# yangyonggit/simple-path-tracer

Hardware: AMD Instinct MI355X
Metric: Mrays/sec + Msamples/sec, default scene 1920x1080, 1/2/4/8 MI355X (higher is better)
Workload: dtype f32; 1 GPU; C2: default scene + emitter, 1920x1080, 64 spp, depth 6; scene=default_emitter, width=1920, height=1080, spp=64, max_depth=6, parallelism=tile-sharded x1 (interleaved 32x32 tiles) + RCCL gather to rank 0

## Files before the change

### include/sptr_hip.h

```cpp
#ifndef SPTR_HIP_H
#define SPTR_HIP_H

#include <stddef.h>
#include <stdint.h>

#ifdef __cplusplus
extern "C" {
#endif

#define SPTR_ABI_VERSION 9

enum sptr_status {
  SPTR_OK = 0,
  SPTR_ERR_INVALID = -1,
  SPTR_ERR_HIP = -2,
  SPTR_ERR_NO_SCENE = -3,
  SPTR_ERR_OOM = -4,
  SPTR_ERR_NO_DEVICE = -5
};

typedef struct sptr_ctx sptr_ctx;

typedef struct sptr_scene {
  const float* positions;
// ... 53 lines not shown
enum sptr_integrator { SPTR_INTEGRATOR_WAVEFRONT = 0, SPTR_INTEGRATOR_PATHTRACER = 1, SPTR_INTEGRATOR_OPTIX = 2 };

typedef struct sptr_frame {
  int32_t width, height;
  sptr_camera camera;
  uint32_t frame_begin;
  uint32_t spp;
  uint32_t max_depth;
  int32_t shard_rank, shard_count;
  uint32_t flags;
  uint32_t integrator;
  uint32_t samples_per_frame;
} sptr_frame;

typedef struct sptr_stats {
  uint64_t rays_closest;
  uint64_t rays_shadow;
  uint64_t samples;
  uint64_t waves;
  double ms_total;
  double ms_raygen, ms_trace, ms_shade, ms_shadow, ms_accum;
  uint64_t trace_launches;
  uint64_t node_visits, tri_tests, sphere_tests;
  uint64_t shadow_node_visits, shadow_prim_tests;
  double ms_trace0, ms_shade0;
  uint64_t rays_tail;
  double ms_tail;
  uint64_t traced_primary, traced_bounce;
  uint64_t node_visits_primary, tri_tests_primary, sphere_tests_primary;
  double ms_cull;
  uint64_t cull_launches;
  uint64_t shadow_launches;
  uint64_t traced_by_depth[8];
  uint64_t nodes_by_depth[8];
  uint64_t trace_visit_hist[16];
  uint64_t shadow_visit_hist[16];
  uint64_t hits_primary, hits_bounce;
  uint64_t paths_handed_off;
  uint64_t strag_visits[3];
  double ms_trace_busy;
  uint64_t traced_fused;
} sptr_stats;

int sptr_abi_version(void);
int sptr_create(int device, sptr_ctx** out);
int sptr_destroy(sptr_ctx* ctx);
const char* sptr_last_error(const sptr_ctx* ctx);
int sptr_set_debug_mode(sptr_ctx* ctx, int mode);
int sptr_set_wave_paths(sptr_ctx* ctx, uint64_t max_paths);
int sptr_set_tail_depth(sptr_ctx* ctx, uint32_t depth);
int sptr_set_bounce_chain(sptr_ctx* ctx, uint32_t mode);
int sptr_set_sky_split(sptr_ctx* ctx, uint32_t mode, uint32_t bulk_threads);
int sptr_sky_split_info(sptr_ctx* ctx, uint32_t* bulk_threads);
int sptr_set_leaf_size(sptr_ctx* ctx, uint32_t max_prims);
int sptr_set_tree_order(sptr_ctx* ctx, uint32_t mode);
typedef struct sptr_tree_order_info {
  uint32_t order, fallback, depth, num_leaves;
  double cost_sah, cost_morton;
} sptr_tree_order_info;
int sptr_tree_info(const sptr_ctx* ctx, sptr_tree_order_info* out);
int sptr_set_split_refs(sptr_ctx* ctx, uint32_t max_pieces);
int sptr_set_stragglers(sptr_ctx* ctx, uint32_t lanes);
int sptr_set_launch_mode(sptr_ctx* ctx, uint32_t mode);
int sptr_set_pixel_lanes(sptr_ctx* ctx, uint32_t lanes);
int sptr_pixel_lanes_info(const sptr_ctx* ctx, uint32_t* requested, uint32_t* active);
int sptr_graph_info(const sptr_ctx* ctx, uint32_t* valid, uint32_t* nodes, uint32_t* edges, uint32_t* depth,
                    uint32_t* captures, int32_t* capture_status);
const char* sptr_capture_error(const sptr_ctx* ctx);
int sptr_overlap_probe(sptr_ctx* ctx, double ms[3]);
int sptr_set_bvh_width(sptr_ctx* ctx, uint32_t width);

int sptr_upload_scene(sptr_ctx* ctx, const sptr_scene* scene);
int sptr_set_materials(sptr_ctx* ctx, const sptr_material* mats, uint32_t count);
int sptr_set_lights(sptr_ctx* ctx, const sptr_light* lights, uint32_t count);
int sptr_set_environment(sptr_ctx* ctx, const sptr_environment* env);
int sptr_scene_info(const sptr_ctx* ctx, uint32_t* num_prims, uint32_t* num_nodes, uint32_t* bvh_depth,
                    double* build_ms);
typedef struct sptr_scene_layout {
  uint32_t num_tris, num_spheres, num_nodes, leaf_size, bvh_depth, lds_bytes;
  uint64_t node_bytes, tri_bytes, sphere_bytes, prim_ref_bytes;
  uint32_t bvh_width;
  uint32_t num_prim_refs;
} sptr_scene_layout;
int sptr_scene_layout_info(const sptr_ctx* ctx, sptr_scene_layout* out);

int sptr_render(sptr_ctx* ctx, const sptr_frame* frame, void* stream, sptr_stats* stats);
int sptr_collect_stats(sptr_ctx* ctx, sptr_stats* stats);
int sptr_read_rgb8(sptr_ctx* ctx, uint8_t* rgb);
int sptr_read_rgb8_lagged(sptr_ctx* ctx, uint8_t* rgb, uint32_t* got);
int sptr_read_accum(sptr_ctx* ctx, float* accum);
int sptr_tiles_device(sptr_ctx* ctx, void** dptr, size_t* bytes);
int sptr_unpack_tiles(sptr_ctx* ctx, const void* gathered, int32_t shard_count, uint32_t tiles_per_rank,
                      int32_t width, int32_t height, void* rgb8_out, void* stream);

typedef struct sptr_denoise_params {
  uint32_t iterations;
  float sigma_color;
  float sigma_depth;
  float sigma_albedo;
  uint32_t normal_log2_power;
  uint32_t reserved[3];
} sptr_denoise_params;
int sptr_set_denoise(sptr_ctx* ctx, const sptr_denoise_params* params);
enum { SPTR_AOV_ALBEDO = 0, SPTR_AOV_NORMAL = 1, SPTR_AOV_DEPTH = 2, SPTR_AOV_ID = 3, SPTR_AOV_UV = 4 };
int sptr_read_aov(sptr_ctx* ctx, int kind, void* out);
int sptr_read_denoised(sptr_ctx* ctx, float* rgb);
// ... 133 lines not shown
```

### simple-path-tracer_amd/csrc/kernels_wavefront.hip

```cpp
#include <hip/hip_runtime.h>
#include <hip/hip_ext.h>

#include <algorithm>
#include <cstdlib>
#include <mutex>

#include "cull_prims.h"
#include "sky_split.h"
#include "sptr_internal.h"

#ifndef SPTR_TRACE_WAVES
#define SPTR_TRACE_WAVES 7
#endif
#ifndef SPTR_TRACE_PM_WAVES
#define SPTR_TRACE_PM_WAVES SPTR_TRACE_WAVES
#endif
#ifndef SPTR_TRACE_WP_WAVES
#define SPTR_TRACE_WP_WAVES SPTR_TRACE_WAVES
#endif
#ifndef SPTR_TRACE4_WAVES
#define SPTR_TRACE4_WAVES 7
#endif
#ifndef SPTR_SHADE_WAVES
#define SPTR_SHADE_WAVES 5
// ... 782 lines not shown
                   nt = sv.num_tris * 3u, ns = sv.num_sph;
    const uint32_t np = (sv.num_tris + sv.num_sph + 3u) / 4u;
    const float4* gn = w4 ? reinterpret_cast<const float4*>(sv.nodes4) : reinterpret_cast<const float4*>(sv.nodes);
    const float4* gp = reinterpret_cast<const float4*>(sv.prim_ref);
    for (uint32_t i = threadIdx.x; i < nn; i += blockDim.x) lds[i] = gn[i];
    for (uint32_t i = threadIdx.x; i < nt; i += blockDim.x) lds[nn + i] = sv.tris[i];
    for (uint32_t i = threadIdx.x; i < ns; i += blockDim.x) lds[nn + nt + i] = sv.sph[i];
    for (uint32_t i = threadIdx.x; i < np; i += blockDim.x) lds[nn + nt + ns + i] = gp[i];
    __syncthreads();
    s.nodes = reinterpret_cast<const BvhNode*>(lds);
    s.nodes4 = reinterpret_cast<const WideNode*>(lds);
    s.tris = lds + nn;
    s.sph = lds + nn + nt;
    s.prim_ref = reinterpret_cast<const uint32_t*>(lds + nn + nt + ns);
  }
  return s;
}

template <bool kTable>
__device__ __forceinline__ Staged stage_shaded(const SceneView& sv, const ShadeView& sh, float4* lds) {
  const bool tab = kTable && sh.pm_lds_bytes != 0u;
  float4* dst = lds + sv.lds_bytes / 16u;
  if (tab) {
    const float4* g = reinterpret_cast<const float4*>(sh.prim_mat);
    for (uint32_t i = threadIdx.x; i < sh.pm_lds_bytes / 16u; i += blockDim.x) dst[i] = g[i];
  }
  Staged s = stage_scene<true>(sv, lds);
  if (kTable) {
    s.pm = tab ? reinterpret_cast<const uint32_t*>(dst) : sh.prim_mat;
    s.pm_lds = tab;
  }
  return s;
}

__device__ __forceinline__ const uint4* stage_top(const SceneView& sv, float4* dst) {
  const uint32_t n = sv.num_top4 * (uint32_t)(sizeof(WideNode) / 16);
  const uint4* g = reinterpret_cast<const uint4*>(sv.nodes4);
  uint4* d = reinterpret_cast<uint4*>(dst);
  for (uint32_t i = threadIdx.x; i < n; i += blockDim.x) d[i] = g[i];
  return d;
}
__device__ __forceinline__ uint32_t top_lds_offset(const SceneView& sv, bool lds, bool primary, uint32_t nseg) {
  return (lds ? sv.lds_bytes / 16u : 0u) + (primary ? 0u : (4u * (nseg + 1u) + 15u) / 16u);
}

template <bool kW4, bool kAny, bool kCount, int N>
__device__ __forceinline__ bool traverse_w(const Staged& sc, const SceneView& sv, const Ray& r, float tnear, float& tfar,
                                           uint32_t& ref, Visits& vc, LdsStackN<N>& ls) {
  if (kW4) return traverse_wide<kAny, kCount>(sc.nodes4, sc.prim_ref, sc.tris, sc.sph, sv.root4, r, tnear, tfar, ref, vc, ls);
  return traverse<kAny, kCount>(sc.nodes, sc.prim_ref, sc.tris, sc.sph, sv.root, r, tnear, tfar, ref, vc, ls);
}

constexpr uint32_t kEntryFieldBits = 13, kEntryFieldMask = (1u << kEntryFieldBits) - 1u;
template <bool kW4, bool kCount, int N>
__device__ __forceinline__ bool traverse_w_from(const Staged& sc, const SceneView& sv, uint32_t root, const Ray& r,
                                                float& tfar, uint32_t& ref, Visits& vc, LdsStackN<N>& ls) {
  if constexpr (kW4) {
    return traverse_wide<false, kCount>(sc.nodes4, sc.prim_ref, sc.tris, sc.sph, sv.root4, r, 0.0f, tfar, ref, vc, ls);
  } else {
    if (root & kLeafBit) {
      if (root == sv.root) return leaf_test<false, kCount>(root, sc.prim_ref, sc.tris, sc.sph, r, 0.0f, tfar, ref, vc);
      asm volatile("" : "+v"(root));
      const float4* nd = reinterpret_cast<const float4*>(sc.nodes + ((root >> 18) & kEntryFieldMask));
      const uint32_t right = (root >> 17) & 1u;
      const float4 xy = nd[right];
      const float2 z = reinterpret_cast<const float2*>(nd + 2)[right];
      if (kCount) ++vc.nodes;
      float tent;
      if (!slab(xy.x, xy.y, xy.z, xy.w, z.x, z.y, r, 0.0f, tfar, tent)) return false;
      const uint32_t range = kLeafBit | (((root >> 4) & kEntryFieldMask) << kLeafCountBits) | (root & kLeafRangeMask);
      return leaf_test<false, kCount>(range, sc.prim_ref, sc.tris, sc.sph, r, 0.0f, tfar, ref, vc);
    }
    return traverse<false, kCount>(sc.nodes, sc.prim_ref, sc.tris, sc.sph, root, r, 0.0f, tfar, ref, vc, ls);
  }
}

template <bool kW4, bool kAny, bool kCount, int N>
__device__ __forceinline__ bool traverse_w_top(const Staged& sc, const SceneView& sv, const uint4* top, uint32_t ntop,
                                               const Ray& r, float tnear, float& tfar, uint32_t& ref, Visits& vc,
                                               LdsStackN<N>& ls) {
  if constexpr (kW4) {
    WideWalk wk;
    if (wide_start<kAny, kCount>(wk, sv.root4, sc.prim_ref, sc.tris, sc.sph, r, tnear, tfar, ref, vc)) return wk.hit;
    TravStack<N> stack;
    stack.lds = &ls.e[0][threadIdx.x];
    (void)wide_walk<kAny, kCount>(wk, stack, sc.nodes4, top, ntop, sc.prim_ref, sc.tris, sc.sph, r, tnear, tfar, ref, vc,
                                  0x7FFFFFFF);
    return wk.hit;
  }
  return traverse<kAny, kCount>(sc.nodes, sc.prim_ref, sc.tris, sc.sph, sv.root, r, tnear, tfar, ref, vc, ls);
}

__device__ __forceinline__ uint32_t stat_depth(int depth) { return depth < kStatDepths - 1 ? (uint32_t)depth : kStatDepths - 1u; }
__device__ __forceinline__ void hist_ray(uint32_t* s_hist, uint32_t visits) {
  const uint32_t b = visits ? (uint32_t)(32 - __clz(visits)) : 0u;
  atomicAdd(&s_hist[b < (uint32_t)kHistBins ? b : kHistBins - 1u], 1u);
}
__device__ __forceinline__ void hist_init(uint32_t* s_hist) {
  if (threadIdx.x < (uint32_t)kHistBins) s_hist[threadIdx.x] = 0u;
}
__device__ __forceinline__ void hist_flush(const uint32_t* s_hist, unsigned long long* tot, int base) {
  __syncthreads();
  if (threadIdx.x < (uint32_t)kHistBins && s_hist[threadIdx.x]) atomicAdd(&tot[base + threadIdx.x], (unsigned long long)s_hist[threadIdx.x]);
}
__device__ __forceinline__ void flush_depth_nodes(const Visits& vc, unsigned long long* tot, int depth) {
  unsigned long long a = vc.nodes;
  for (int off = 32; off > 0; off >>= 1) a += __shfl_xor(a, off);
  if (lane_id() == 0) atomicAdd(&tot[kTotNodesD + stat_depth(depth)], a);
}

__device__ __forceinline__ void report_stack(const Visits& vc, unsigned long long* tot) {
  if (__ballot(vc.stack_overflow != 0u) && lane_id() == 0u) tot[kTotStackOverflow] = 1ull;
}

__device__ __forceinline__ void flush_visits(const Visits& vc, unsigned long long* tot, int base) {
  unsigned long long a = vc.nodes, b = vc.tris, c = vc.sph;
  for (int off = 32; off > 0; off >>= 1) {
    a += __shfl_xor(a, off);
    b += __shfl_xor(b, off);
    c += __shfl_xor(c, off);
  }
  if (lane_id() == 0) {
    atomicAdd(&tot[base + 0], a);
    atomicAdd(&tot[base + 1], b);
    if (base == kTotNodes || base == kTotNodesP || base == kTotStragNodes) atomicAdd(&tot[base + 2], c);
  }
}
// ... 46 lines not shown
    if (d < -kCullSlack * mag) return true;
  }
  return false;
}
__device__ __forceinline__ bool pixel_frustum_misses(const SceneView& sv, const FrameView& f, int x, int y, int npx = 1) {
  if (sv.num_nodes == 0u || (sv.root & kLeafBit)) return false;
  const float u0 = (float(x) - kCullMarginPx) / float(f.W), u1 = (float(x + npx) + kCullMarginPx) / float(f.W);
  const float v0 = (float(y) - kCullMarginPx) / float(f.H), v1 = (float(y + npx) + kCullMarginPx) / float(f.H);
  auto dir = [&](float u, float v) {
    return f.cam_f + ((u - 0.5f) * 2.0f * f.half_w) * f.cam_r + (-(v - 0.5f) * 2.0f * f.half_h) * f.cam_u;
  };
  const vec3 c[4] = {dir(u0, v0), dir(u1, v0), dir(u1, v1), dir(u0, v1)};
  vec3 n[4];
#pragma unroll
  for (int k = 0; k < 4; ++k) {
    n[k] = cross(c[k], c[(k + 1) & 3]);
    if (dot(n[k], c[(k + 2) & 3]) < 0.0f) n[k] = -n[k];
  }
  struct Entry {
    uint32_t link, depth;
    Box b;
  };
  Entry st[2 * kCullDepthMax + 2];
  int sp = 0;
  {
    const BvhNode r = sv.nodes[0];
    st[sp++] = Entry{r.link.y, 1u, Box{v3(r.rxy.x, r.rxy.z, r.z.z), v3(r.rxy.y, r.rxy.w, r.z.w)}};
    st[sp++] = Entry{r.link.x, 1u, Box{v3(r.lxy.x, r.lxy.z, r.z.x), v3(r.lxy.y, r.lxy.w, r.z.y)}};
  }
  while (sp > 0) {
    const Entry e = st[--sp];
    if (box_outside(e.b, n, f.cam_pos)) continue;
    if ((e.link & kLeafBit) || e.depth >= f.cull_depth) return false;
    const BvhNode g = sv.nodes[e.link];
    st[sp++] = Entry{g.link.y, e.depth + 1u, Box{v3(g.rxy.x, g.rxy.z, g.z.z), v3(g.rxy.y, g.rxy.w, g.z.w)}};
    st[sp++] = Entry{g.link.x, e.depth + 1u, Box{v3(g.lxy.x, g.lxy.z, g.z.x), v3(g.lxy.y, g.lxy.w, g.z.y)}};
  }
  return true;
}
constexpr int kCullEntryDepth = 20;
struct CullStack {
  uint32_t st[kCullEntryDepth + 2][kBlock];
  uint16_t path[kCullEntryDepth + 1][kBlock];
};
constexpr uint32_t kCullLeaf = 1u << 17;
__device__ __forceinline__ uint32_t cull_pack(uint32_t link, uint32_t depth, uint32_t side) {
  const uint32_t l = (link & kLeafBit) ? (kCullLeaf | (((link & ~kLeafBit) >> kLeafCountBits) << 4) | (link & kLeafRangeMask)) : link;
  return l | (depth << 18) | (side << 24);
}
__device__ __forceinline__ Box child_box(const BvhNode& g, bool right) {
  return right ? Box{v3(g.rxy.x, g.rxy.z, g.z.z), v3(g.rxy.y, g.rxy.w, g.z.w)}
               : Box{v3(g.lxy.x, g.lxy.z, g.z.x), v3(g.lxy.y, g.lxy.w, g.z.y)};
}
__device__ __forceinline__ void cull_leaf(const Staged& sc, const CullPyramid& py, uint32_t link, uint32_t& lo, uint32_t& hi) {
  const uint32_t start = (link & ~kLeafBit) >> kLeafCountBits, cnt = (link & kLeafRangeMask) + 1u;
  lo = kNoHit;
  hi = 0u;
  for (uint32_t j = 0; j < cnt; ++j) {
    const uint32_t pr = sc.prim_ref[start + j];
    const uint32_t idx = pr & kIndexMask;
    bool out;
    if (pr & kSphereBit) {
      const float4 s = sc.sph[idx];
      const vec3 c = v3(s.x, s.y, s.z), v = c - py.o;
      const float rb = fabsf(s.w) + 1.1e-3f * (fabsf(v.x) + fabsf(v.y) + fabsf(v.z)) +
                       1e-5f * (py.ol + fabsf(c.x) + fabsf(c.y) + fabsf(c.z));
      out = box_outside(Box{c - v3(rb, rb, rb), c + v3(rb, rb, rb)}, py.n, py.o) || cull_sphere_outside(py, c, s.w);
    } else {
      const float4 a = sc.tris[3u * idx], b = sc.tris[3u * idx + 1u], c = sc.tris[3u * idx + 2u];
      const vec3 v0 = v3(a.x, a.y, a.z), v1 = v0 - v3(a.w, b.x, b.y), v2 = v0 + v3(b.z, b.w, c.x);
      const vec3 lo3 = v3(fminf(v0.x, fminf(v1.x, v2.x)), fminf(v0.y, fminf(v1.y, v2.y)), fminf(v0.z, fminf(v1.z, v2.z)));
      const vec3 hi3 = v3(fmaxf(v0.x, fmaxf(v1.x, v2.x)), fmaxf(v0.y, fmaxf(v1.y, v2.y)), fmaxf(v0.z, fmaxf(v1.z, v2.z)));
      const float pad = 1e-5f * (fabsf(lo3.x) + fabsf(lo3.y) + fabsf(lo3.z) + fabsf(hi3.x) + fabsf(hi3.y) + fabsf(hi3.z) + py.ol);
      out = box_outside(Box{lo3 - v3(pad, pad, pad), hi3 + v3(pad, pad, pad)}, py.n, py.o) || cull_triangle_outside(py, v0, v1, v2);
    }
    if (!out) {
      lo = min(lo, start + j);
      hi = start + j;
    }
  }
}
__device__ __forceinline__ uint32_t entry_leaf(uint32_t parent, uint32_t side, uint32_t lo, uint32_t hi) {
  if (parent >= kEntryFieldMask || hi > kEntryFieldMask) return parent;
  return kLeafBit | (parent << 18) | (side << 17) | (lo << 4) | (hi - lo);
}
__device__ __forceinline__ uint32_t cull_entry(const Staged& sc, const SceneView& sv, const FrameView& f, int x, int y, int npx,
                                               CullStack& cs) {
  if (sv.root == kNoHit) return kNoHit;
  const float u0 = (float(x) - kCullMarginPx) / float(f.W), u1 = (float(x + npx) + kCullMarginPx) / float(f.W);
  const float v0 = (float(y) - kCullMarginPx) / float(f.H), v1 = (float(y + npx) + kCullMarginPx) / float(f.H);
  auto dir = [&](float u, float v) {
    return f.cam_f + ((u - 0.5f) * 2.0f * f.half_w) * f.cam_r + (-(v - 0.5f) * 2.0f * f.half_h) * f.cam_u;
  };
  const CullPyramid py = cull_pyramid(f.cam_pos, dir(u0, v0), dir(u1, v0), dir(u1, v1), dir(u0, v1));
  uint32_t lo, hi;
  if ((sv.root & kLeafBit) || sv.num_nodes == 0u) return sv.root;
  const uint32_t limit = min(f.cull_depth, (uint32_t)kCullEntryDepth);
  uint32_t* st = &cs.st[0][threadIdx.x];
  uint16_t* path = &cs.path[0][threadIdx.x];
  int sp = 0;
  uint32_t ncand = 0u, common = kNoHit, mind = kNoHit, anc = sv.root, one_lo = 0u, one_hi = 0u, one_side = 0u;
  bool one_leaf = false;
  auto push_children = [&](uint32_t node, uint32_t depth) {
    const BvhNode g = sc.nodes[node];
    path[(depth - 1u) * kBlock] = (uint16_t)node;
    if (!box_outside(child_box(g, true), py.n, f.cam_pos)) st[sp++ * kBlock] = cull_pack(g.link.y, depth, 1u);
    if (!box_outside(child_box(g, false), py.n, f.cam_pos)) st[sp++ * kBlock] = cull_pack(g.link.x, depth, 0u);
  };
  push_children(sv.root, 1u);
  while (sp > 0) {
    const uint32_t e = st[--sp * kBlock];
    const uint32_t link = e & (kCullLeaf - 1u), depth = (e >> 18) & 63u, side = (e >> 24) & 1u;
    mind = min(mind, depth);
    if (e & kCullLeaf) {
      cull_leaf(sc, py, kLeafBit | ((link >> 4) << kLeafCountBits) | (link & kLeafRangeMask), lo, hi);
      if (lo > hi) continue;
      one_leaf = ncand++ == 0u;
      common = one_leaf ? depth : min(common, mind);
      anc = path[(common - 1u) * kBlock];
      mind = kNoHit;
      one_lo = lo;
      one_hi = hi;
      one_side = side;
    } else if (depth >= limit) {
      if (ncand++ == 0u) {
        common = depth + 1u;
        anc = link;
      } else {
        common = min(common, mind);
        anc = path[(common - 1u) * kBlock];
      }
      mind = kNoHit;
      one_leaf = false;
    } else {
      push_children(link, depth + 1u);
    }
  }
  if (ncand == 0u) return kNoHit;
  if (one_leaf) return entry_leaf(anc, one_side, one_lo, one_hi);
  return anc;
}
__device__ __forceinline__ uint32_t entry_index(uint32_t l) {
  const uint32_t w = l & 1023u;
  return ((l >> 10) << 8) | ((w >> 6) << 4) | ((w & 31u) >> 1);
}
template <bool kEntry>
__global__ void __launch_bounds__(kBlock) k_cull(SceneView sv, FrameView f, uint32_t* mask, uint32_t* plist, uint32_t* entry,
                                                 uint32_t list_culled) {
  static_assert(kTile == 32 && kBlock == 256, "16 x 16 quads per 32 x 32 tile");
  __shared__ uint32_t s_row[kTile];
  __shared__ uint32_t s_cnt[kBlock / 64u];
  __shared__ uint32_t s_base, s_base_c;
  const uint32_t t0 = blockIdx.x * kTilePixels;
  if (threadIdx.x < (uint32_t)kTile) s_row[threadIdx.x] = 0u;
  extern __shared__ float4 lds[];
  [[maybe_unused]] const Staged sc = stage_scene<kEntry>(sv, lds);
  __syncthreads();
  {
    const uint32_t qx = threadIdx.x & 15u, qy = threadIdx.x >> 4;
    int x = 0, y = 0;
    (void)local_pixel(f, t0 + 2u * qy * kTile + 2u * qx, x, y);
    bool miss;
    if constexpr (kEntry) {
      __shared__ CullStack s_cs;
      const uint32_t e = (x < f.W && y < f.H) ? cull_entry(sc, sv, f, x, y, 2, s_cs) : kNoHit;
      entry[blockIdx.x * kBlock + threadIdx.x] = e;
      miss = x < f.W && y < f.H && e == kNoHit;
    } else {
      miss = x < f.W && y < f.H && pixel_frustum_misses(sv, f, x, y, 2);
    }
    if (miss) {
      atomicOr(&s_row[2u * qy], 3u << (2u * qx));
      atomicOr(&s_row[2u * qy + 1u], 3u << (2u * qx));
    }
  }
  __syncthreads();
  const uint32_t row = threadIdx.x >> 3, col = (threadIdx.x & 7u) * 4u;
  const uint32_t bits = (s_row[row] >> col) & 0xFu;
  uint32_t keep = 0u;
#pragma unroll
  for (uint32_t j = 0; j < 4u; ++j) {
    int x, y;
    if (local_pixel(f, t0 + 4u * threadIdx.x + j, x, y) && !((bits >> j) & 1u)) keep |= 1u << j;
  }
  const uint32_t valid_bits = [&] {
    uint32_t v = 0u;
#pragma unroll
    for (uint32_t j = 0; j < 4u; ++j) {
      int x, y;
      if (local_pixel(f, t0 + 4u * threadIdx.x + j, x, y)) v |= 1u << j;
    }
    return v;
  }();
// ... 168 lines not shown
__device__ __forceinline__ void ktime_end(const WaveView& w) {
  if (!w.tslot) return;
  __syncthreads();
  if (threadIdx.x == 0)
    atomicMax(w.tslot + kTimeLineWords * (1u + (blockIdx.x & (kTimeEndLines - 1u))), (unsigned long long)wall_clock64());
}

template <bool kCount, bool kW4, bool kCube>
__global__ void __launch_bounds__(kBlock, kW4 ? SPTR_TRACE4_WAVES : SPTR_TRACE_PM_WAVES)
    k_trace_pm(SceneView sv, EnvView sh, FrameView fin, WaveView w) {
  ktime_begin(w);
  const FrameView f = frame_dyn(fin);
  __shared__ LdsStack s_stack;
  extern __shared__ float4 lds[];
  __shared__ uint32_t s_cnt;
  __shared__ uint32_t s_hist[kCount ? kHistBins : 1];
  if (threadIdx.x == 0) s_cnt = 0u;
  if (kCount) hist_init(s_hist);
  const Staged sc = stage_scene<true>(sv, lds);
  __syncthreads();
  if (blockIdx.x == 0 && threadIdx.x == 0) {
    atomicAdd(&w.tot[kTotClosest], (unsigned long long)((unsigned long long)f.valid * f.k));
    atomicAdd(&w.tot[kTotTracedP], (unsigned long long)(primary_traced(f)));
    atomicAdd(&w.tot[kTotTracedD], (unsigned long long)(primary_traced(f)));
  }
  const ImageDiv idiv = image_div(f);
  Visits vc;
  const Sched sd = block_sched(f.P);
  const uint32_t per = sd.per * f.k;
  const uint32_t seg0 = logical_block() * per;
  for (uint32_t it = 0;; ++it) {
    const uint32_t base = sd.first + it * sd.step;
    if (base >= sd.end) break;
    const uint32_t l = base + threadIdx.x;
    int x = 0, y = 0;
    const bool valid = l < f.P && local_pixel(f, l, x, y);
    const uint32_t ps = valid ? (uint32_t)(y * f.W + x) : 0u;
    const uint32_t root = valid ? primary_root<true, kW4>(sv, f, l) : kNoHit;
    vec3 a = v3(0.0f, 0.0f, 0.0f);
    if (valid && !f.reset) a = xyz(f.accum[l]);
    bool fold = true;
    uint32_t resume = f.k;
    for (uint32_t smp = 0; smp < f.k; ++smp) {
      bool hit = false;
      uint32_t ref = kNoHit;
      float tfar = __builtin_huge_valf();
      const uint32_t p = smp * f.P + l;
      if (valid) {
        Primary pr;
        primary_at(f, idiv, x, y, ps, f.acc0 + smp, pr);
        if (!(ablate(f) & 2u) && root != kNoHit) {
          const Ray r = make_ray(f.cam_pos, pr.d);
          const uint32_t v0 = vc.nodes;
          hit = traverse_w_from<kW4, kCount>(sc, sv, root, r, tfar, ref, vc, s_stack);
          if (kCount) hist_ray(s_hist, vc.nodes - v0);
        }
        if (!hit) {
          vec3 rv = v3(0.0f, 0.0f, 0.0f);
          if (sh.debug_mode != 1) {
            const vec3 e = (ablate(f) & 1u) ? pr.d : env_color<kCube>(sh, renormalized_again(pr.d));
            rv = v3(0.0f, 0.0f, 0.0f) + v3(1.0f, 1.0f, 1.0f) * e;
          }
          if (!fold) w.rad[p] = f4(rv, 0.0f);
          else if (!(ablate(f) & 4u)) a = a + rv;
        } else if (fold) {
          fold = false;
          resume = smp;
        }
      }
      const uint32_t j = block_append(&s_cnt, hit);
      if (hit) {
        if (seg0 + j < w.hrec_cap) w.hrec.put(seg0 + j, p, __float_as_uint(tfar), ref);
        else w.tot[kTotOverflow] = 1ull;
      }
    }
    if (l < f.P) f.accum[l] = make_float4(a.x, a.y, a.z, __uint_as_float(resume));
  }
  seg_publish(w.segH, &s_cnt, per);
  if (kCount && threadIdx.x == 0) atomicAdd(&w.tot[kTotHitP], (unsigned long long)s_cnt);
  report_stack(vc, w.tot);
  if (kCount) {
    flush_visits(vc, w.tot, kTotNodes);
    flush_visits(vc, w.tot, kTotNodesP);
    flush_depth_nodes(vc, w.tot, 0);
    hist_flush(s_hist, w.tot, kTotHistT);
  }
  ktime_end(w);
}

constexpr uint32_t kFoldLanes = 8;
template <bool kLds, bool kCount, bool kW4, bool kCube, bool kHiOcc = false, bool kTimed = false, bool kEntries = true,
          bool kList = false>
__global__ void __launch_bounds__(kBlock, kW4 ? SPTR_TRACE4_WAVES : (kHiOcc ? 8 : SPTR_TRACE_WP_WAVES))
    k_trace_wp(SceneView sv, EnvView sh, FrameView fin, WaveView w) {
  static_assert(!kList || (kLds && !kHiOcc && kEntries), "the item list: LDS-staged scenes at the 7-wave occupancy");
  if constexpr (kTimed) ktime_begin(w);
  const FrameView f = frame_dyn(fin);
  __shared__ KernelStack<kLds> s_stack;
  extern __shared__ float4 lds[];
  __shared__ uint32_t s_cnt;
  __shared__ uint32_t s_hist[kCount ? kHistBins : 1];
  __shared__ float4 s_fold[kBlock];
  if (threadIdx.x == 0) s_cnt = 0u;
  if (kCount) hist_init(s_hist);
  const Staged sc = stage_scene<kLds>(sv, lds);
  __syncthreads();
  if (blockIdx.x == 0 && threadIdx.x == 0) {
    atomicAdd(&w.tot[kTotClosest], (unsigned long long)((unsigned long long)f.valid * f.k));
    atomicAdd(&w.tot[kTotTracedP], (unsigned long long)(primary_traced(f)));
    atomicAdd(&w.tot[kTotTracedD], (unsigned long long)(primary_traced(f)));
  }
  const ImageDiv idiv = image_div(f);
  Visits vc;
  constexpr uint32_t kPix = kBlock / kFoldLanes;
  const uint32_t lane = lane_id(), q = lane & (kFoldLanes - 1u), g0 = lane & ~(kFoldLanes - 1u);
  const uint32_t lb = logical_block();
  const uint32_t step = gridDim.x * kPix;
  const uint32_t cap = (f.P + step - 1u) / step * kPix;
  const uint32_t per = cap * f.k;
  const uint32_t seg0 = lb * per;
  const uint32_t rounds = (f.k + kFoldLanes - 1u) / kFoldLanes;
  static_assert(kPix == kSkySplitChunk, "sky_split.h deals the items in this kernel's chunks");
  const SkySplit ss = kList ? sky_split(f.plist[f.P], f.plist[f.P + 1u], f.split_threads) : SkySplit{};
  const uint32_t work = kList ? ss.items : f.P;
  for (uint32_t it = 0;; ++it) {
    const uint32_t base = lb * kPix + it * step;
    if (base >= work) break;
    uint32_t l = base + threadIdx.x / kFoldLanes;
    if constexpr (kList) l = l < ss.items ? f.plist[sky_split_item_word(ss, f.P, l)] : f.P;
    int x = 0, y = 0;
    const bool valid = l < f.P && local_pixel(f, l, x, y);
    const uint32_t ps = valid ? (uint32_t)(y * f.W + x) : 0u;
    static_assert(kEntries || kHiOcc, "only the high-occupancy form has an instantiation without entries");
    uint32_t root = valid ? primary_root<kLds && kEntries, kW4>(sv, f, l) : kNoHit;
    vec3 a = v3(0.0f, 0.0f, 0.0f);
    if (valid && !f.reset) a = xyz(f.accum[l]);
    bool fold = true;
    uint32_t resume = f.k;
    for (uint32_t r = 0; r < rounds; ++r) {
      const uint32_t smp = r * kFoldLanes + q;
      const bool act = valid && smp < f.k;
      bool hit = false;
      uint32_t ref = kNoHit;
      float tfar = __builtin_huge_valf();
      const uint32_t p = smp * f.P + l;
      vec3 rv = v3(0.0f, 0.0f, 0.0f);
      if (act) {
        Primary pr;
        primary_at(f, idiv, x, y, ps, f.acc0 + smp, pr);
        if constexpr (kHiOcc && kEntries) {
          uint32_t lv = l;
          asm volatile("" : "+v"(lv));
          root = primary_root<kLds, kW4>(sv, f, lv);
        }
        if (root != kNoHit) {
          const Ray r = make_ray(f.cam_pos, pr.d);
          const uint32_t v0 = vc.nodes;
          if constexpr (kEntries) hit = traverse_w_from<kW4, kCount>(sc, sv, root, r, tfar, ref, vc, s_stack);
          else hit = traverse_w<kW4, false, kCount>(sc, sv, r, 0.0f, tfar, ref, vc, s_stack);
          if (kCount) hist_ray(s_hist, vc.nodes - v0);
        }
        if (!hit && sh.debug_mode != 1) rv = v3(0.0f, 0.0f, 0.0f) + v3(1.0f, 1.0f, 1.0f) * env_color<kCube>(sh, renormalized_again(pr.d));
      }
      const uint32_t hm = (uint32_t)(__ballot(hit) >> g0) & ((1u << kFoldLanes) - 1u);
      const uint32_t nact = f.k - r * kFoldLanes < kFoldLanes ? f.k - r * kFoldLanes : kFoldLanes;
      const uint32_t nfold = fold ? (hm ? (uint32_t)__builtin_ctz(hm) : nact) : 0u;
      s_fold[threadIdx.x] = make_float4(rv.x, rv.y, rv.z, 0.0f);
      __builtin_amdgcn_wave_barrier();
      if (q == 0u) {
#pragma unroll
        for (uint32_t j = 0; j < kFoldLanes; ++j) {
          if (j < nfold) {
            const float4 v = s_fold[threadIdx.x + j];
            a = v3(a.x + v.x, a.y + v.y, a.z + v.z);
          }
        }
      }
      __builtin_amdgcn_wave_barrier();
      if (fold && hm) {
        fold = false;
        resume = r * kFoldLanes + nfold;
      }
      if (act && !hit && q >= nfold) w.rad[p] = f4(rv, 0.0f);
      const uint32_t j = block_append(&s_cnt, hit);
      if (hit) {
        if (seg0 + j < w.hrec_cap) w.hrec.put(seg0 + j, p, __float_as_uint(tfar), ref);
        else w.tot[kTotOverflow] = 1ull;
      }
    }
    if (q == 0u && l < f.P) f.accum[l] = make_float4(a.x, a.y, a.z, __uint_as_float(valid ? resume : f.k));
  }
  seg_publish(w.segH, &s_cnt, per);
  if (kCount && threadIdx.x == 0) atomicAdd(&w.tot[kTotHitP], (unsigned long long)s_cnt);
  report_stack(vc, w.tot);
  if (kCount) {
    flush_visits(vc, w.tot, kTotNodes);
    flush_visits(vc, w.tot, kTotNodesP);
    flush_depth_nodes(vc, w.tot, 0);
    hist_flush(s_hist, w.tot, kTotHistT);
  }
  if constexpr (kTimed) ktime_end(w);
}
template <bool kLds, bool kCount, bool kPrimary, bool kW4, bool kCube>
__global__ void __launch_bounds__(kBlock, (kW4 && !kPrimary) ? SPTR_TRACE4_WAVES : SPTR_TRACE_WAVES)
    k_trace(SceneView sv, EnvView sh, FrameView fin, WaveView w, int depth, uint32_t nseg_in) {
  ktime_begin(w);
  const FrameView f = frame_dyn(fin);
  __shared__ KernelStack<kLds> s_stack;
  extern __shared__ float4 lds[];
  __shared__ uint32_t s_cnt;
  uint32_t* s_off = reinterpret_cast<uint32_t*>(lds + (kLds ? sv.lds_bytes / 16u : 0u));
// ... 3 lines not shown
  const Staged sc = stage_scene<kLds>(sv, lds);
  uint32_t n, per_in = 0u, nlist = 0u;
  if (kPrimary) {
    nlist = f.plist ? f.plist[f.P] : 0u;
    n = f.plist ? nlist * f.k : f.P * f.k;
    __syncthreads();
  } else {
    n = seg_scan(w.segN, nseg_in, s_off, per_in);
  }
  if (blockIdx.x == 0 && threadIdx.x == 0) {
    atomicAdd(&w.tot[kTotClosest], (unsigned long long)(kPrimary ? (unsigned long long)f.valid * f.k : n));
    const unsigned long long t = kPrimary ? primary_traced(f) : (unsigned long long)n;
    atomicAdd(&w.tot[kPrimary ? kTotTracedP : kTotTracedB], (unsigned long long)(t));
    atomicAdd(&w.tot[kTotTracedD + stat_depth(depth)], (unsigned long long)(t));
  }
  const ImageDiv idiv = image_div(f);
  const RayStream rs = w.rs[depth & 1];
  Visits vc;
  const Sched sd = block_sched(n);
  for (uint32_t base = sd.first; base < sd.end; base += sd.step) {
    const uint32_t i = base + threadIdx.x;
    bool active = i < n, hit = false, culled = false;
    uint32_t id = 0u, pid = 0u, ref = kNoHit;
    [[maybe_unused]] uint32_t root = kNoHit;
    float tfar = __builtin_huge_valf();
    vec3 o, d;
    if (active) {
      if (kPrimary) {
        Primary pr;
        uint32_t l, p = i;
        if (f.plist) p = primary_item(f, nlist, i);
        id = pid = p;
        active = primary_path(f, idiv, p, pr, l);
        if constexpr (kLds && !kW4) {
          root = active ? primary_root<kLds, kW4>(sv, f, l) : kNoHit;
          culled = root == kNoHit;
        } else {
          culled = !f.plist && pixel_culled(f, l);
        }
        o = f.cam_pos;
        d = pr.d;
      } else {
        id = seg_slot(s_off, nseg_in, per_in, i);
        const float4 o4 = rs.o[id], d4 = rs.d[id];
        o = xyz(o4);
        d = xyz(d4);
        pid = __float_as_uint(d4.w);
      }
    }
    if (active) {
      const Ray r = make_ray(o, d);
      if (!(kPrimary && ((ablate(f) & 2u) || culled))) {
        const uint32_t v0 = vc.nodes;
        if constexpr (kPrimary && kLds && !kW4) hit = traverse_w_from<kW4, kCount>(sc, sv, root, r, tfar, ref, vc, s_stack);
        else hit = traverse_w<kW4, false, kCount>(sc, sv, r, 0.0f, tfar, ref, vc, s_stack);
        if (kCount) hist_ray(s_hist, vc.nodes - v0);
      }
      if (kPrimary && !hit && (ablate(f) & 4u)) {
      } else if (!hit) {
        if (sh.debug_mode == 1) {
          w.rad[pid] = make_float4(0.0f, 0.0f, 0.0f, 0.0f);
        } else {
          const vec3 e = (ablate(f) & 1u) ? d : env_color<kCube>(sh, renormalized_again(d));
          vec3 rv;
          if (kPrimary) rv = v3(0.0f, 0.0f, 0.0f) + v3(1.0f, 1.0f, 1.0f) * e;
          else rv = xyz(w.rad[pid]) + xyz(rs.thr[id]) * e;
          w.rad[pid] = f4(rv, 0.0f);
        }
      }
    }
    const uint32_t j = block_append(&s_cnt, hit);
    if (hit) {
      if (sd.seg0 + j < w.hrec_cap) w.hrec.put(sd.seg0 + j, id, __float_as_uint(tfar), ref);
      else w.tot[kTotOverflow] = 1ull;
    }
  }
  seg_publish(w.segH, &s_cnt, sd.per);
  if (kCount && threadIdx.x == 0) atomicAdd(&w.tot[kPrimary ? kTotHitP : kTotHitB], (unsigned long long)s_cnt);
  report_stack(vc, w.tot);
  if (kCount) {
    flush_visits(vc, w.tot, kTotNodes);
    if (kPrimary) flush_visits(vc, w.tot, kTotNodesP);
    flush_depth_nodes(vc, w.tot, depth);
    hist_flush(s_hist, w.tot, kTotHistT);
  }
  ktime_end(w);
}

template <bool kAny, bool kCount, bool kW4>
__device__ __forceinline__ bool walk_start(WideWalk& wk, const Staged& sc, uint32_t root, const Ray& r, float tnear,
                                           float& tfar, uint32_t& ref, Visits& vc) {
  return wide_start<kAny, kCount>(wk, root, sc.prim_ref, sc.tris, sc.sph, r, tnear, tfar, ref, vc);
}
template <bool kAny, bool kCount, bool kW4, int kKind = kWalkU, int N>
__device__ __forceinline__ bool walk_steps(WideWalk& wk, TravStack<N>& stack, const Staged& sc, const uint4* top,
                                           uint32_t ntop, const Ray& r, float tnear, float& tfar, uint32_t& ref, Visits& vc,
                                           int steps) {
  if (kW4)
    return wide_walk<kAny, kCount, kKind>(wk, stack, sc.nodes4, top, ntop, sc.prim_ref, sc.tris, sc.sph, r, tnear, tfar, ref, vc,
                                   steps);
  return bvh2_walk<kAny, kCount>(wk.cur, wk.sp, wk.hit, stack, sc.nodes, sc.prim_ref, sc.tris, sc.sph, r, tnear, tfar, ref,
                                 vc, steps);
}

#ifndef SPTR_DYN_STEPS
#define SPTR_DYN_STEPS 8
#endif
// ... 462 lines not shown
          if (light_faces(sh.lights[li], sf)) shadow = true;
      }
    }
    vec3 so, ldir, contrib;
    float stfar = 0.0f;
    bool lit = false;
    if (kFuse) {
      if (shadow) lit = light_term(sh.lights[0], sf, -rd, thr, so, ldir, stfar, contrib);
      shadow = false;
    }
    const uint32_t js = kFuse ? 0u : block_append(&s_cnt_s, shadow);
    if (shadow && sd.seg0 + js >= w.seg_cap) {
      shadow = false;
      w.tot[kTotOverflow] = 1ull;
    }
    const bool carry = !kFuse && (uint32_t)depth == w.carry_depth;
    bool lit0 = false;
    vec3 c0 = v3(0.0f, 0.0f, 0.0f);
    if (shadow) {
      float4* task = w.stask + (size_t)(sd.seg0 + js) * L * ts;
      const vec3 view = -rd;
      for (uint32_t li = 0; li < L; ++li, task += ts) {
        vec3 so, ldir, contrib;
        float tfar;
        if (!light_term(sh.lights[li], sf, view, thr, so, ldir, tfar, contrib)) {
          task[1] = make_float4(0.0f, 0.0f, 0.0f, __uint_as_float(0u));
          continue;
        }
        task[0] = f4(so, tfar);
        if (ts > 2u) task[2] = f4(ldir, 0.0f);
        if (carry) {
          lit0 = true;
          c0 = contrib;
        } else {
          task[1] = f4(contrib, __uint_as_float(p + 1u));
        }
      }
    }
    if (active && sh.debug_mode != 1) cont = continue_path(sf, rd, (uint32_t)depth, thr, rng, no, nd) && !last;
    if (!kFuse && active && dirty) w.rad[p] = f4(radv, 0.0f);
    const uint32_t jn = block_append(&s_cnt_n, cont);
    if (cont && sd.seg0 + jn >= w.seg_cap) {
      cont = false;
      w.tot[kTotOverflow] = 1ull;
    }
    if (lit0) w.stask[(size_t)(sd.seg0 + js) * ts + 1u] = f4(c0, __uint_as_float(cont ? 0u : p + 1u));
    if (cont) {
      rout.o[sd.seg0 + jn] = f4(no, __uint_as_float(rng));
      rout.d[sd.seg0 + jn] = f4(nd, __uint_as_float(p));
      rout.thr[sd.seg0 + jn] = f4(thr, __uint_as_float(lit0 ? sd.seg0 + js + 1u : 0u));
    }
    if (kFuse) {
      if (lit) {
        const Ray r = make_ray(so, ldir);
        uint32_t ref = kNoHit;
        ++rays;
        if (!traverse_w<false, true, false>(sc, sv, r, 1e-4f, stfar, ref, vc, s_stack)) {
          if (!dirty) radv = xyz(w.rad[p]);
          dirty = true;
          radv = radv + contrib;
        }
      }
      if (active && dirty) w.rad[p] = f4(radv, 0.0f);
    }
  }
  if (kFuse) {
    for (int off = 32; off > 0; off >>= 1) rays += __shfl_xor(rays, off);
    if (lane_id() == 0u) atomicAdd(&s_rays, rays);
    report_stack(vc, w.tot);
  }
  __syncthreads();
  if (threadIdx.x == 0) {
    w.segN.cnt[logical_block()] = s_cnt_n;
    w.segS.cnt[logical_block()] = s_cnt_s;
    if (kFuse) w.bstat[blockIdx.x] += s_rays;
    if (blockIdx.x == 0) {
      *w.segN.per = sd.per;
      *w.segS.per = sd.per;
    }
  }
}

template <bool kCube, int kFrom>
__device__ __forceinline__ void bounce_ray(const Staged& sc, const SceneView& sv, const ShadeView& sh, const DevMaterial* smat,
                                           uint32_t nm, const WaveView& w, const RayStream& rin, const RayStream& rout,
                                           int depth, bool last, bool valid, uint32_t id, uint32_t seg0, uint32_t* s_cnt,
                                           Visits& vc, LdsStack& s_stack, uint32_t& rays) {
  bool cont = false, dirty = false, lit = false;
  uint32_t p = 0u, rng = 0u;
  vec3 thr, radv = v3(0.0f, 0.0f, 0.0f), no, nd, so, ldir, contrib;
  float stfar = 0.0f;
  if (valid) {
    const float4 o4 = rin.o[id], d4 = rin.d[id];
    const vec3 ro = xyz(o4), rd = xyz(d4);
    p = __float_as_uint(d4.w);
    rng = __float_as_uint(o4.w);
    thr = xyz(rin.thr[id]);
    float tfar = __builtin_huge_valf();
    uint32_t ref = kNoHit;
    if (!traverse_w<false, false, false>(sc, sv, make_ray(ro, rd), 0.0f, tfar, ref, vc, s_stack)) {
      if (sh.debug_mode == 1) {
        w.rad[p] = make_float4(0.0f, 0.0f, 0.0f, 0.0f);
      } else {
        const vec3 e = env_color<kCube>(sh.env, renormalized_again(rd));
        w.rad[p] = f4(xyz(w.rad[p]) + thr * e, 0.0f);
      }
    } else if (sh.debug_mode == 1) {
      radv = v3(1.0f, 1.0f, 1.0f);
      dirty = true;
    } else {
      const Surface sf = surface_at<kFrom>(sc, sv, sh, smat, nm, ro, rd, tfar, ref);
      const vec3 emission = v3(sf.m.emission[0], sf.m.emission[1], sf.m.emission[2]);
      if (dot(emission, emission) > 0.0f) {
        radv = xyz(w.rad[p]) + thr * emission;
        dirty = true;
      }
      if (light_faces(sh.lights[0], sf)) lit = light_term(sh.lights[0], sf, -rd, thr, so, ldir, stfar, contrib);
      cont = continue_path(sf, rd, (uint32_t)depth, thr, rng, no, nd) && !last;
    }
  }
  const uint32_t jn = block_append(s_cnt, cont);
  if (cont && seg0 + jn >= w.seg_cap) {
    cont = false;
    w.tot[kTotOverflow] = 1ull;
  }
  if (cont) {
    rout.o[seg0 + jn] = f4(no, __uint_as_float(rng));
    rout.d[seg0 + jn] = f4(nd, __uint_as_float(p));
    rout.thr[seg0 + jn] = f4(thr, 0.0f);
  }
  if (lit) {
    uint32_t ref = kNoHit;
    ++rays;
    if (!traverse_w<false, true, false>(sc, sv, make_ray(so, ldir), 1e-4f, stfar, ref, vc, s_stack)) {
      if (!dirty) radv = xyz(w.rad[p]);
      dirty = true;
      radv = radv + contrib;
    }
  }
  if (dirty) w.rad[p] = f4(radv, 0.0f);
}

template <bool kCube, bool kTimed = false>
__global__ void __launch_bounds__(kBlock, SPTR_BOUNCE_WAVES)
    k_bounce(SceneView sv, ShadeView sh, FrameView fin, WaveView w, int depth, uint32_t nseg_in) {
  if constexpr (kTimed) ktime_begin(w);
  const FrameView f = frame_dyn(fin);
  extern __shared__ float4 lds[];
  uint32_t* s_off = reinterpret_cast<uint32_t*>(lds + (sv.lds_bytes + sh.pm_lds_bytes) / 16u);
  __shared__ DevMaterial smat[32];
  __shared__ uint32_t s_cnt_n, s_rays;
  __shared__ LdsStack s_stack;
  const uint32_t nm = stage_materials(sh, smat);
  if (threadIdx.x == 0) s_cnt_n = s_rays = 0u;
  constexpr int kFrom = kShadeFused;
  const Staged sc = stage_shaded<kFrom == kShadeFused>(sv, sh, lds);
  uint32_t per_in = 0u;
  const uint32_t n = seg_scan(w.segN, nseg_in, s_off, per_in);
  if (blockIdx.x == 0 && threadIdx.x == 0) {
    atomicAdd(&w.tot[kTotClosest], (unsigned long long)(n));
    atomicAdd(&w.tot[kTotTracedF], (unsigned long long)(n));
    atomicAdd(&w.tot[kTotTracedD + stat_depth(depth)], (unsigned long long)(n));
  }
  const RayStream rin = w.rs[depth & 1], rout = w.rs[(depth + 1) & 1];
  const bool last = (uint32_t)(depth + 1) >= f.max_depth;
  Visits vc;
  uint32_t rays = 0u;
  const Sched sd = block_sched(n);
  for (uint32_t base = sd.first; base < sd.end; base += sd.step) {
    const uint32_t i = base + threadIdx.x;
    const bool valid = i < n;
    const uint32_t id = valid ? seg_slot(s_off, nseg_in, per_in, i) : 0u;
    bounce_ray<kCube, kFrom>(sc, sv, sh, smat, nm, w, rin, rout, depth, last, valid, id, sd.seg0, &s_cnt_n, vc, s_stack, rays);
  }
  for (int off = 32; off > 0; off >>= 1) rays += __shfl_xor(rays, off);
  if (lane_id() == 0u) atomicAdd(&s_rays, rays);
  report_stack(vc, w.tot);
  __syncthreads();
  if (threadIdx.x == 0) {
    w.segH.cnt[logical_block()] = s_cnt_n;
    w.bstat[blockIdx.x] += s_rays;
    if (blockIdx.x == 0) *w.segH.per = sd.per;
  }
  if constexpr (kTimed) ktime_end(w);
}

template <bool kCube, int kFrom>
__device__ __forceinline__ void bounce01_path(const Staged& sc, const SceneView& sv, const ShadeView& sh, const DevMaterial* smat,
                                              uint32_t nm, const FrameView& f, const ImageDiv& idiv, const WaveView& w,
                                              const RayStream& rout, bool last1, bool last2, bool valid, uint32_t slot,
                                              uint32_t seg0, uint32_t* s_cnt, Visits& vc, LdsStack& s_stack, uint32_t& rays,
                                              uint32_t& traced) {
  bool cont = false, active = valid;
  uint32_t p = 0u, rng = 0u;
  vec3 thr = v3(1.0f, 1.0f, 1.0f), radv = v3(0.0f, 0.0f, 0.0f), ro, rd;
  if (active) {
    uint3 h;
    w.hrec.get(slot, h.x, h.y, h.z);
    p = h.x;
    Primary pr;
    primary_path(f, idiv, p, pr);
    rng = pr.rng;
    if (sh.debug_mode == 1) {
      radv = v3(1.0f, 1.0f, 1.0f);
      active = false;
    } else {
      const Surface sf = surface_at<kFrom>(sc, sv, sh, smat, nm, f.cam_pos, pr.d, __uint_as_float(h.y), h.z);
      const vec3 emission = v3(sf.m.emission[0], sf.m.emission[1], sf.m.emission[2]);
      if (dot(emission, emission) > 0.0f) radv = radv + thr * emission;
      vec3 so, ldir, contrib;
      float stfar = 0.0f;
      const bool lit = light_faces(sh.lights[0], sf) && light_term(sh.lights[0], sf, -pr.d, thr, so, ldir, stfar, contrib);
      active = continue_path(sf, pr.d, 0u, thr, rng, ro, rd) && !last1;
      if (lit) {
        uint32_t sref = kNoHit;
        ++rays;
        if (!traverse_w<false, true, false>(sc, sv, make_ray(so, ldir), 1e-4f, stfar, sref, vc, s_stack)) radv = radv + contrib;
      }
    }
  }
  bool lit = false;
  vec3 no, nd, so, ldir, contrib;
  float stfar = 0.0f;
  if (active) {
    ++traced;
    float tfar = __builtin_huge_valf();
    uint32_t ref = kNoHit;
    if (!traverse_w<false, false, false>(sc, sv, make_ray(ro, rd), 0.0f, tfar, ref, vc, s_stack)) {
      radv = radv + thr * env_color<kCube>(sh.env, renormalized_again(rd));
    } else {
      const Surface sf = surface_at<kFrom>(sc, sv, sh, smat, nm, ro, rd, tfar, ref);
      const vec3 emission = v3(sf.m.emission[0], sf.m.emission[1], sf.m.emission[2]);
      if (dot(emission, emission) > 0.0f) radv = radv + thr * emission;
      if (light_faces(sh.lights[0], sf)) lit = light_term(sh.lights[0], sf, -rd, thr, so, ldir, stfar, contrib);
      cont = continue_path(sf, rd, 1u, thr, rng, no, nd) && !last2;
    }
  }
  const uint32_t jn = block_append(s_cnt, cont);
  if (cont && seg0 + jn >= w.seg_cap) {
    cont = false;
    w.tot[kTotOverflow] = 1ull;
  }
  if (cont) {
    rout.o[seg0 + jn] = f4(no, __uint_as_float(rng));
    rout.d[seg0 + jn] = f4(nd, __uint_as_float(p));
    rout.thr[seg0 + jn] = f4(thr, 0.0f);
  }
  if (lit) {
    uint32_t sref = kNoHit;
    ++rays;
    if (!traverse_w<false, true, false>(sc, sv, make_ray(so, ldir), 1e-4f, stfar, sref, vc, s_stack)) radv = radv + contrib;
  }
  if (valid) w.rad[p] = f4(radv, 0.0f);
}
#ifndef SPTR_BOUNCE01_WAVES
#define SPTR_BOUNCE01_WAVES 5
#endif
template <bool kCube, bool kTimed = false>
__global__ void __launch_bounds__(kBlock, SPTR_BOUNCE01_WAVES)
    k_bounce01(SceneView sv, ShadeView sh, FrameView fin, WaveView w, uint32_t nseg_in) {
  if constexpr (kTimed) ktime_begin(w);
  const FrameView f = frame_dyn(fin);
  extern __shared__ float4 lds[];
  uint32_t* s_off = reinterpret_cast<uint32_t*>(lds + (sv.lds_bytes + sh.pm_lds_bytes) / 16u);
  __shared__ DevMaterial smat[32];
  __shared__ uint32_t s_cnt_n, s_rays, s_traced;
  __shared__ LdsStack s_stack;
  const uint32_t nm = stage_materials(sh, smat);
  if (threadIdx.x == 0) s_cnt_n = s_rays = s_traced = 0u;
  constexpr int kFrom = kShadeFused;
  const Staged sc = stage_shaded<kFrom == kShadeFused>(sv, sh, lds);
  uint32_t per_in = 0u;
  const uint32_t n = seg_scan(w.segH, nseg_in, s_off, per_in);
  const RayStream rout = w.rs[0];
  const bool last1 = 1u >= f.max_depth, last2 = 2u >= f.max_depth;
  const ImageDiv idiv = image_div(f);
  Visits vc;
  uint32_t rays = 0u, traced = 0u;
  const Sched sd = block_sched(n);
  for (uint32_t base = sd.first; base < sd.end; base += sd.step) {
    const uint32_t i = base + threadIdx.x;
    const bool valid = i < n;
    const uint32_t slot = valid ? seg_slot(s_off, nseg_in, per_in, i) : 0u;
    bounce01_path<kCube, kFrom>(sc, sv, sh, smat, nm, f, idiv, w, rout, last1, last2, valid, slot, sd.seg0, &s_cnt_n, vc, s_stack, rays,
                         traced);
  }
  for (int off = 32; off > 0; off >>= 1) {
    rays += __shfl_xor(rays, off);
    traced += __shfl_xor(traced, off);
  }
  if (lane_id() == 0u) {
    atomicAdd(&s_rays, rays);
    atomicAdd(&s_traced, traced);
  }
  report_stack(vc, w.tot);
  __syncthreads();
  if (threadIdx.x == 0) {
    w.segN.cnt[logical_block()] = s_cnt_n;
    w.bstat[blockIdx.x] += s_rays;
    if (blockIdx.x == 0) *w.segN.per = sd.per;
    atomicAdd(&w.tot[kTotClosest], (unsigned long long)s_traced);
    atomicAdd(&w.tot[kTotTracedF], (unsigned long long)s_traced);
    atomicAdd(&w.tot[kTotTracedD + 1], (unsigned long long)s_traced);
  }
// ... 38 lines not shown
  for (int d = 2; d < T; ++d) {
    __syncthreads();
    const uint32_t cnt = s_cnt[(d - 1) % 3];
    if (threadIdx.x == 0) {
      s_cnt[(d + 1) % 3] = 0u;
      if (cnt) atomicAdd(&w.tot[kTotTracedD + stat_depth(d)], (unsigned long long)cnt);
      later += cnt;
    }
    const RayStream rin = w.rs[d & 1], rout = w.rs[(d + 1) & 1];
    const bool last = (uint32_t)(d + 1) >= f.max_depth;
    for (uint32_t j = 0u; j < cnt; j += kBlock) {
      const uint32_t id = sd.seg0 + j + threadIdx.x;
      const bool valid = j + threadIdx.x < cnt && id < w.seg_cap;
      bounce_ray<kCube, kFrom>(sc, sv, sh, smat, nm, w, rin, rout, d, last, valid, id, sd.seg0, &s_cnt[d % 3], vc, s_stack, rays);
    }
  }
  for (int off = 32; off > 0; off >>= 1) {
    rays += __shfl_xor(rays, off);
    traced += __shfl_xor(traced, off);
  }
  if (lane_id() == 0u) {
    atomicAdd(&s_rays, rays);
    atomicAdd(&s_traced, traced);
  }
  report_stack(vc, w.tot);
  __syncthreads();
  if (threadIdx.x == 0) {
    if ((uint32_t)T < f.max_depth) {
      w.segN.cnt[logical_block()] = s_cnt[(T - 1) % 3];
      if (blockIdx.x == 0) *w.segN.per = sd.per;
    }
    w.bstat[blockIdx.x] += s_rays;
    atomicAdd(&w.tot[kTotClosest], (unsigned long long)s_traced + later);
    atomicAdd(&w.tot[kTotTracedF], (unsigned long long)s_traced + later);
    atomicAdd(&w.tot[kTotTracedD + 1], (unsigned long long)s_traced);
  }
  if constexpr (kTimed) ktime_end(w);
}

#ifndef SPTR_ST_FIRST_WAVES
#define SPTR_ST_FIRST_WAVES 5
#endif
#ifndef SPTR_ST_WAVES
#define SPTR_ST_WAVES 6
#endif
#ifndef SPTR_ST_CLOSE_WAVES
#define SPTR_ST_CLOSE_WAVES 5
#endif
__device__ __forceinline__ void rad_add(const WaveView& w, uint32_t p, bool& dirty, vec3& radv, vec3 c) {
  if (!dirty) radv = xyz(w.rad[p]);
  dirty = true;
  radv = radv + c;
}
__device__ __forceinline__ void shadow_add(const Staged& sc, const SceneView& sv, const WaveView& w, uint32_t p, vec3 so,
                                           vec3 ldir, float stfar, vec3 contrib, bool& dirty, vec3& radv, Visits& vc,
                                           LdsStack& s_stack, uint32_t& rays) {
  uint32_t sref = kNoHit;
  ++rays;
  if (!traverse_w<false, true, false>(sc, sv, make_ray(so, ldir), 1e-4f, stfar, sref, vc, s_stack))
    rad_add(w, p, dirty, radv, contrib);
}
template <bool kCube, bool kFirst, bool kClose, int kFrom>
__device__ __forceinline__ void shade_trace(const Staged& sc, const SceneView& sv, const ShadeView& sh, const DevMaterial* smat,
                                            uint32_t nm, const FrameView& f, const ImageDiv& idiv, const WaveView& w,
                                            const RayStream& rin, const RayStream& rout, int depth, bool last, bool valid,
                                            uint32_t slot, uint32_t seg0, uint32_t* s_cnt, Visits& vc, LdsStack& s_stack,
                                            uint32_t& rays, uint32_t& traced) {
  bool active = false, dirty = kFirst && valid, lit = false;
  uint32_t p = 0u, rng = 0u;
  vec3 thr = v3(1.0f, 1.0f, 1.0f), radv = v3(0.0f, 0.0f, 0.0f), no, nd, so, ldir, contrib;
  float stfar = 0.0f;
  if (valid) {
    vec3 ro, rd;
    float t;
    uint32_t ref;
    if constexpr (kFirst) {
      uint32_t tb;
      w.hrec.get(slot, p, tb, ref);
      t = __uint_as_float(tb);
      Primary pr;
      primary_path(f, idiv, p, pr);
      ro = f.cam_pos;
      rd = pr.d;
      rng = pr.rng;
    } else {
      const float4 o4 = rin.o[slot], d4 = rin.d[slot], t4 = rin.thr[slot];
      ref = rin.ref[slot];
      ro = xyz(o4);
      rd = xyz(d4);
      thr = xyz(t4);
      t = t4.w;
      rng = __float_as_uint(o4.w);
      p = __float_as_uint(d4.w);
    }
    if (sh.debug_mode == 1) {
      radv = v3(1.0f, 1.0f, 1.0f);
      dirty = true;
    } else {
      const Surface sf = surface_at<kFrom>(sc, sv, sh, smat, nm, ro, rd, t, ref);
      const vec3 emission = v3(sf.m.emission[0], sf.m.emission[1], sf.m.emission[2]);
      if (dot(emission, emission) > 0.0f) rad_add(w, p, dirty, radv, thr * emission);
      if (light_faces(sh.lights[0], sf)) lit = light_term(sh.lights[0], sf, -rd, thr, so, ldir, stfar, contrib);
      active = continue_path(sf, rd, (uint32_t)(depth - 1), thr, rng, no, nd);
    }
  }
  if (lit) shadow_add(sc, sv, w, p, so, ldir, stfar, contrib, dirty, radv, vc, s_stack, rays);
  bool hit = false;
  float tfar = __builtin_huge_valf();
  uint32_t href = kNoHit;
  if (active) {
    ++traced;
    hit = traverse_w<false, false, false>(sc, sv, make_ray(no, nd), 0.0f, tfar, href, vc, s_stack);
    if (!hit) rad_add(w, p, dirty, radv, thr * env_color<kCube>(sh.env, renormalized_again(nd)));
  }
  if constexpr (!kClose) {
    const uint32_t jn = block_append(s_cnt, hit);
    if (hit && seg0 + jn >= w.seg_cap) {
      hit = false;
      w.tot[kTotOverflow] = 1ull;
    }
    if (hit) {
      rout.o[seg0 + jn] = f4(no, __uint_as_float(rng));
      rout.d[seg0 + jn] = f4(nd, __uint_as_float(p));
      rout.thr[seg0 + jn] = f4(thr, tfar);
      rout.ref[seg0 + jn] = href;
    }
  } else {
    bool cont = false;
    vec3 no2, nd2;
    lit = false;
    if (hit) {
      const Surface sf = surface_at<kFrom>(sc, sv, sh, smat, nm, no, nd, tfar, href);
      const vec3 emission = v3(sf.m.emission[0], sf.m.emission[1], sf.m.emission[2]);
      if (dot(emission, emission) > 0.0f) rad_add(w, p, dirty, radv, thr * emission);
      if (light_faces(sh.lights[0], sf)) lit = light_term(sh.lights[0], sf, -nd, thr, so, ldir, stfar, contrib);
      if (!last) cont = continue_path(sf, nd, (uint32_t)depth, thr, rng, no2, nd2);
    }
    const uint32_t jn = block_append(s_cnt, cont);
    if (cont && seg0 + jn >= w.seg_cap) {
      cont = false;
      w.tot[kTotOverflow] = 1ull;
    }
    if (cont) {
      rout.o[seg0 + jn] = f4(no2, __uint_as_float(rng));
      rout.d[seg0 + jn] = f4(nd2, __uint_as_float(p));
      rout.thr[seg0 + jn] = f4(thr, 0.0f);
    }
    if (lit) shadow_add(sc, sv, w, p, so, ldir, stfar, contrib, dirty, radv, vc, s_stack, rays);
  }
  if (dirty) w.rad[p] = f4(radv, 0.0f);
}

template <bool kCube, bool kFirst, bool kClose, bool kTimed = false>
__global__ void __launch_bounds__(kBlock, kClose ? SPTR_ST_CLOSE_WAVES : (kFirst ? SPTR_ST_FIRST_WAVES : SPTR_ST_WAVES))
    k_shade_trace(SceneView sv, ShadeView sh, FrameView fin, WaveView w, int depth, uint32_t nseg_in) {
  if constexpr (kTimed) ktime_begin(w);
  const FrameView f = frame_dyn(fin);
  extern __shared__ float4 lds[];
  uint32_t* s_off = reinterpret_cast<uint32_t*>(lds + (sv.lds_bytes + sh.pm_lds_bytes) / 16u);
  __shared__ DevMaterial smat[32];
  __shared__ uint32_t s_cnt_n, s_rays, s_traced;
  __shared__ LdsStack s_stack;
  const uint32_t nm = stage_materials(sh, smat);
  if (threadIdx.x == 0) s_cnt_n = s_rays = s_traced = 0u;
  constexpr int kFrom = (kTimed && kCube && !kFirst && !kClose) ? kShadeGlobal : kShadeFused;
  const Staged sc = stage_shaded<kFrom == kShadeFused>(sv, sh, lds);
  const SegTable tin = kFirst ? w.segH : w.segN, tout = kFirst ? w.segN : w.segH;
  uint32_t per_in = 0u;
  const uint32_t n = seg_scan(tin, nseg_in, s_off, per_in);
  const RayStream rin = w.rs[depth & 1], rout = w.rs[(depth + 1) & 1];
  const bool last = (uint32_t)(depth + 1) >= f.max_depth;
  const ImageDiv idiv = image_div(f);
  Visits vc;
  uint32_t rays = 0u, traced = 0u;
  const Sched sd = block_sched(n);
  for (uint32_t base = sd.first; base < sd.end; base += sd.step) {
    const uint32_t i = base + threadIdx.x;
    const bool valid = i < n;
    const uint32_t slot = valid ? seg_slot(s_off, nseg_in, per_in, i) : 0u;
    shade_trace<kCube, kFirst, kClose, kFrom>(sc, sv, sh, smat, nm, f, idiv, w, rin, rout, depth, last, valid, slot, sd.seg0, &s_cnt_n,
                                       vc, s_stack, rays, traced);
  }
  for (int off = 32; off > 0; off >>= 1) {
    rays += __shfl_xor(rays, off);
    traced += __shfl_xor(traced, off);
  }
  if (lane_id() == 0u) {
    atomicAdd(&s_rays, rays);
    atomicAdd(&s_traced, traced);
  }
  report_stack(vc, w.tot);
  __syncthreads();
  if (threadIdx.x == 0) {
    tout.cnt[logical_block()] = s_cnt_n;
    w.bstat[blockIdx.x] += s_rays;
    if (blockIdx.x == 0) *tout.per = sd.per;
    if (s_traced) {
      atomicAdd(&w.tot[kTotClosest], (unsigned long long)s_traced);
      atomicAdd(&w.tot[kTotTracedF], (unsigned long long)s_traced);
      atomicAdd(&w.tot[kTotTracedD + stat_depth(depth)], (unsigned long long)s_traced);
    }
  }
  if constexpr (kTimed) ktime_end(w);
}

template <bool kLds, bool kCount, bool kW4>
__global__ void __launch_bounds__(kBlock, kW4 ? SPTR_SHADOW4_WAVES : SPTR_SHADOW_WAVES) k_shadow(SceneView sv, ShadeView sh, WaveView w, int depth, uint32_t nseg_in) {
  ktime_begin(w);
  __shared__ KernelStack<kLds> s_stack;
  extern __shared__ float4 lds[];
  __shared__ uint32_t s_rays;
  __shared__ uint32_t s_hist[kCount ? kHistBins : 1];
  uint32_t* s_off = reinterpret_cast<uint32_t*>(lds + (kLds ? sv.lds_bytes / 16u : 0u));
  if (threadIdx.x == 0) s_rays = 0u;
  if (kCount) hist_init(s_hist);
  const Staged sc = stage_scene<kLds>(sv, lds);
  uint32_t per_in = 0u;
  const uint32_t n = seg_scan(w.segS, nseg_in, s_off, per_in);
  const uint32_t ts = w.tstride, L = w.L;
  Visits vc;
  uint32_t rays = 0u;
  const Sched sd = block_sched(n);
  for (uint32_t i = sd.first + threadIdx.x; i < sd.end; i += sd.step) {
    const float4* task = w.stask + (size_t)seg_slot(s_off, nseg_in, per_in, i) * L * ts;
    bool any = false;
    uint32_t p = 0u;
    vec3 rv = v3(0.0f, 0.0f, 0.0f);
    for (uint32_t li = 0; li < L; ++li, task += ts) {
      const float4 c = task[1];
      const uint32_t tag = __float_as_uint(c.w);
      if (tag == 0u) continue;
      p = tag - 1u;
      const float4 a = task[0];
      const vec3 dir = (ts > 2u && sh.lights[li].type != 0)
                           ? xyz(task[2])
                           : v3(sh.lights[li].v[0], sh.lights[li].v[1], sh.lights[li].v[2]);
      const Ray r = make_ray(xyz(a), dir);
      float tfar = a.w;
      uint32_t ref = kNoHit;
      ++rays;
      const uint32_t v0 = vc.nodes;
      const bool occ = traverse_w<kW4, true, kCount>(sc, sv, r, 1e-4f, tfar, ref, vc, s_stack);
      if (kCount) hist_ray(s_hist, vc.nodes - v0);
      if (!occ) {
        if (!any) rv = xyz(w.rad[p]);
        any = true;
        rv = rv + xyz(c);
      }
    }
    if (any) w.rad[p] = f4(rv, 0.0f);
  }
  for (int off = 32; off > 0; off >>= 1) rays += __shfl_xor(rays, off);
  if (lane_id() == 0u) atomicAdd(&s_rays, rays);
  __syncthreads();
  if (threadIdx.x == 0) atomicAdd(&w.bstat[blockIdx.x], (unsigned long long)s_rays);
  report_stack(vc, w.tot);
  if (kCount) {
    flush_visits(vc, w.tot, kTotShNodes);
    hist_flush(s_hist, w.tot, kTotHistS);
  }
  ktime_end(w);
}

template <bool kCount, bool kQueue>
__global__ void __launch_bounds__(kBlock, SPTR_SHADOW4_WAVES) k_shadow_dyn(SceneView sv, ShadeView sh, WaveView w, int depth,
                                                                           uint32_t nseg_in) {
  ktime_begin(w);
  __shared__ KernelStack<false> s_stack;
  extern __shared__ float4 lds[];
  __shared__ uint32_t s_rays, s_next;
  __shared__ uint32_t s_hist[kCount ? kHistBins : 1];
  uint32_t* s_off = reinterpret_cast<uint32_t*>(lds);
  if (threadIdx.x == 0) s_rays = s_next = 0u;
  if (kCount) hist_init(s_hist);
  constexpr int kKind = kQueue ? kWalkU : kWalkInline;
  const uint32_t ntop = walk_reads_top(kKind) ? sv.num_top4 : 0u;
  const uint4* top = ntop ? stage_top(sv, lds + top_lds_offset(sv, false, false, nseg_in)) : nullptr;
  uint32_t per_in = 0u;
  const uint32_t n = seg_scan(w.segS, nseg_in, s_off, per_in);
  const uint32_t ts = w.tstride;
  Visits vc;
  uint32_t rays = 0u;
  const Sched sd = block_sched(n);
  const uint32_t nb = block_items(sd, n);
  TravStack<kLdsStackG> stack;
  stack.lds = &s_stack.e[0][threadIdx.x];
  bool have = false, done = false;
  uint32_t p = 0u, ref = kNoHit;
  uint32_t v0 = 0u;
  float tfar = 0.0f;
  vec3 contrib;
  Ray r;
  WideWalk wk;
  XcdQueue xq = xcd_queue(w.work + ((uint32_t)depth % 2u) * 256u, n);
  for (;;) {
// ... 92 lines not shown
      p = __float_as_uint(d4.w);
      radv = v3(0.0f, 0.0f, 0.0f);
      loaded = false;
      depth = (uint32_t)depth0;
      have = depth < D;
    }
    if (__ballot(have) == 0ull) break;
    if (!have) continue;
    bool fin = true;
    do {
      if (cslot) {
        const float4* task = w.stask + (size_t)(cslot - 1u) * w.tstride;
        const float4 a = task[0], c = task[1];
        const vec3 sdir = (w.tstride > 2u && sh.lights[0].type != 0) ? xyz(task[2])
                                                                    : v3(sh.lights[0].v[0], sh.lights[0].v[1], sh.lights[0].v[2]);
        ++n_shadow;
        float st = a.w;
        uint32_t sref = kNoHit;
        if (!traverse_w_top<kW4, true, false>(sc, sv, top, ntop, make_ray(xyz(a), sdir), 1e-4f, st, sref, vc, s_stack)) {
          if (!loaded) {
            radv = xyz(w.rad[p]);
            loaded = true;
          }
          radv = radv + xyz(c);
        }
        cslot = 0u;
      }
      ++n_closest;
      float tfar = __builtin_huge_valf();
      uint32_t ref = kNoHit;
      const bool hit = traverse_w_top<kW4, false, false>(sc, sv, top, ntop, make_ray(ro, rd), 0.0f, tfar, ref, vc, s_stack);
      if (sh.debug_mode == 1) {
        radv = hit ? v3(1.0f, 1.0f, 1.0f) : v3(0.0f, 0.0f, 0.0f);
        loaded = true;
        break;
      }
      if (!loaded) {
        radv = xyz(w.rad[p]);
        loaded = true;
      }
      if (!hit) {
        radv = radv + thr * env_color<kCube>(sh.env, renormalized_again(rd));
        break;
      }
      const Surface sf = surface_at<kFrom>(sc, sv, sh, smat, nm, ro, rd, tfar, ref);
      const vec3 emission = v3(sf.m.emission[0], sf.m.emission[1], sf.m.emission[2]);
      if (dot(emission, emission) > 0.0f) radv = radv + thr * emission;
      const vec3 view = -rd;
      for (uint32_t li = 0; li < L; ++li) {
        vec3 so, ldir, contrib;
        float st;
        if (!light_term(sh.lights[li], sf, view, thr, so, ldir, st, contrib)) continue;
        ++n_shadow;
        uint32_t sref = kNoHit;
        if (!traverse_w_top<kW4, true, false>(sc, sv, top, ntop, make_ray(so, ldir), 1e-4f, st, sref, vc, s_stack))
          radv = radv + contrib;
      }
      vec3 no, nd;
      if (!continue_path(sf, rd, depth, thr, rng, no, nd)) break;
      ro = no;
      rd = nd;
      fin = ++depth >= D;
    } while (false);
    if (fin) {
      if (loaded) w.rad[p] = f4(radv, 0.0f);
      have = false;
    }
  }
  for (int off = 32; off > 0; off >>= 1) {
    n_closest += __shfl_xor(n_closest, off);
    n_shadow += __shfl_xor(n_shadow, off);
  }
  if (lane_id() == 0u) {
    atomicAdd(&s_rays[0], n_closest);
    atomicAdd(&s_rays[1], n_shadow);
  }
  __syncthreads();
  if (threadIdx.x == 0) {
    atomicAdd(&w.bstat_closest[blockIdx.x], (unsigned long long)s_rays[0]);
    atomicAdd(&w.bstat[blockIdx.x], (unsigned long long)s_rays[1]);
  }
  report_stack(vc, w.tot);
}

#ifndef SPTR_STRAG_WAVES
#define SPTR_STRAG_WAVES SPTR_TAIL_WAVES
#endif
template <bool kW4, bool kCube>
__global__ void __launch_bounds__(kBlock, SPTR_STRAG_WAVES) k_strag(SceneView sv, ShadeView sh, FrameView f, WaveView w,
                                                                    int depth0) {
  __shared__ KernelStack<false> s_stack;
  __shared__ DevMaterial smat[32];
  __shared__ uint32_t s_rays[2], s_next;
  const uint32_t nm = stage_materials(sh, smat);
  if (threadIdx.x < 2u) s_rays[threadIdx.x] = 0u;
  if (threadIdx.x == 0u) s_next = 0u;
  const Staged sc = stage_scene<false>(sv, nullptr);
  constexpr int kFrom = kShadeGlobal;
  extern __shared__ float4 lds[];
  const uint32_t ntop = walk_reads_top(kWalkU) ? sv.num_top4 : 0u;
  const uint4* top = ntop ? stage_top(sv, lds) : nullptr;
  __syncthreads();
  const uint32_t n = min(w.work[kWorkStrag + (uint32_t)depth0 * 32u], w.strag_cap);
  if (blockIdx.x == 0 && threadIdx.x == 0) atomicAdd(&w.tot[kTotStrag], (unsigned long long)n);
  const float4* in = w.strag + (size_t)depth0 * w.strag_cap * kStragRec;
  TravStack<kLdsStackG> stack;
  stack.lds = &s_stack.e[0][threadIdx.x];
  WideWalk wk;
  float tfar0 = 0.0f;
// ... 923 lines not shown
          }(fl);
        },
        Flags<>{}, count, W, cube);
  }
  if (!L && W) {
    const unsigned lbd = lb + (walk_reads_top(P ? kWalkPrimary : kWalkU) ? sv.num_top4 * (unsigned)sizeof(WideNode) : 0u);
    const bool queue = trace_queue_applies(sv);
    return dispatch(
        [&](auto fl) -> unsigned {
          return [&]<bool C, bool Pc, bool Cube, bool Q>(Flags<C, Pc, Cube, Q>) {
            const unsigned g = resident_grid((const void*)&k_trace_dyn<false, C, Pc, true, Cube, Q>, lbd);
            SPTR_TIMED_LAUNCH((k_trace_dyn<false, C, Pc, true, Cube, Q>), dim3(g), b, lbd, s, sv, ev, f, w, depth, nseg);
            return g;
          }(fl);
        },
        Flags<>{}, count, P, cube, queue);
  }
  return dispatch(
      [&](auto fl) -> unsigned {
        return [&]<bool Lc, bool C, bool Pc, bool Wc, bool Cube>(Flags<Lc, C, Pc, Wc, Cube>) {
          const unsigned g = resident_grid((const void*)&k_trace<Lc, C, Pc, Wc, Cube>, lb);
          SPTR_TIMED_LAUNCH((k_trace<Lc, C, Pc, Wc, Cube>), dim3(g), b, lb, s, sv, ev, f, w, depth, nseg);
          return g;
        }(fl);
      },
      Flags<>{}, L, count, P, W, cube);
}

bool shadow_overlaps(const SceneView& sv, const WaveView& w) {
  return sv.lds_bytes == 0 && sv.width == (uint32_t)kWide && w.L == 1u;
}

bool shade_fuses_shadows(const SceneView& sv, const ShadeView& sh, bool count) {
#ifdef SPTR_EXPERIMENT_KNOBS
  if (getenv("SPTR_NO_FUSE")) return false;
#endif
  return sv.lds_bytes != 0 && sv.width == 2u && sh.num_lights == 1u && !count && sh.prim_mat != nullptr;
}

unsigned launch_shade(const SceneView& sv, const ShadeView& sh, const FrameView& f, const WaveView& w, int depth,
                      uint32_t nseg, bool fuse, hipStream_t s, bool stream_rays) {
  const unsigned lb = (fuse ? sv.lds_bytes : 0u) + (4u * (nseg + 1u) + 15u) / 16u * 16u;
  return dispatch(
      [&](auto fl) -> unsigned {
        return [&]<bool Pc, bool Fc>(Flags<Pc, Fc>) {
          const unsigned g = resident_grid((const void*)&k_shade<Pc, Fc>, lb);
          hipLaunchKernelGGL((k_shade<Pc, Fc>), dim3(g), dim3(kBlock), lb, s, sv, sh, f, w, depth, nseg);
          return g;
        }(fl);
      },
      Flags<>{}, depth == 0 && !stream_rays, fuse);
}

bool cull_entries_apply(const SceneView& sv) { return sv.lds_bytes != 0u && sv.width == 2u; }
uint32_t cull_depth_for(uint32_t spp, bool exact) {
  if (exact) return (uint32_t)kCullEntryDepth;
  return spp >= 16u ? (uint32_t)kCullDepthMax : 4u;
}

void launch_cull(const SceneView& sv, const FrameView& f, uint32_t* mask, uint32_t* plist, uint32_t* entry, bool list_culled,
                 hipStream_t s) {
  if (f.P == 0u) return;
  const uint32_t lc = list_culled ? 1u : 0u;
  if (entry) hipLaunchKernelGGL(k_cull<true>, dim3(f.P / kTilePixels), dim3(kBlock), sv.lds_bytes, s, sv, f, mask, plist, entry, lc);
  else hipLaunchKernelGGL(k_cull<false>, dim3(f.P / kTilePixels), dim3(kBlock), 0, s, sv, f, mask, plist, entry, lc);
}

unsigned launch_bounce(const SceneView& sv, const ShadeView& sh, const FrameView& f, const WaveView& w_in, int depth,
                       uint32_t nseg, bool shade_first, bool close, hipStream_t s) {
  const WaveView w = with_tslot(w_in);
  const unsigned lb = sv.lds_bytes + sh.pm_lds_bytes + (4u * (nseg + 1u) + 15u) / 16u * 16u;
  if (!shade_first)
    return dispatch(
        [&](auto fl) -> unsigned {
          return [&]<bool Cube, bool T>(Flags<Cube, T>) {
            const unsigned g = resident_grid((const void*)&k_bounce<Cube, T>, lb);
            SPTR_TIMED_LAUNCH((k_bounce<Cube, T>), dim3(g), dim3(kBlock), lb, s, sv, sh, f, w, depth, nseg);
            return g;
          }(fl);
        },
        Flags<>{}, sh.env.env != nullptr, w.tslot != nullptr);
  return dispatch(
      [&](auto fl) -> unsigned {
        return [&]<bool Cube, bool Cl, bool T>(Flags<Cube, Cl, T>) {
          const unsigned g = resident_grid((const void*)&k_shade_trace<Cube, false, Cl, T>, lb);
          SPTR_TIMED_LAUNCH((k_shade_trace<Cube, false, Cl, T>), dim3(g), dim3(kBlock), lb, s, sv, sh, f, w, depth, nseg);
          return g;
        }(fl);
      },
      Flags<>{}, sh.env.env != nullptr, close, w.tslot != nullptr);
}

unsigned launch_bounce01(const SceneView& sv, const ShadeView& sh, const FrameView& f, const WaveView& w_in, uint32_t nseg,
                         bool shade_first, bool close, hipStream_t s) {
  const WaveView w = with_tslot(w_in);
  const unsigned lb = sv.lds_bytes + sh.pm_lds_bytes + (4u * (nseg + 1u) + 15u) / 16u * 16u;
  if (!shade_first)
    return dispatch(
        [&](auto fl) -> unsigned {
          return [&]<bool Cube, bool T>(Flags<Cube, T>) {
            const unsigned g = resident_grid((const void*)&k_bounce01<Cube, T>, lb);
            SPTR_TIMED_LAUNCH((k_bounce01<Cube, T>), dim3(g), dim3(kBlock), lb, s, sv, sh, f, w, nseg);
            return g;
          }(fl);
        },
        Flags<>{}, sh.env.env != nullptr, w.tslot != nullptr);
// ... 243 lines not shown
```

### simple-path-tracer_amd/csrc/sptr_api.cpp

```cpp
#include <hip/hip_runtime.h>

#include <algorithm>
#include <chrono>
#include <cmath>
#include <cstdlib>
#include <cstring>
#include <mutex>
#include <string>
#include <vector>

#include "sptr_internal.h"

#include <dlfcn.h>
#include <execinfo.h>
#include <csignal>
#include <ucontext.h>
#include <unistd.h>

struct sptr_ctx {
  sptr::Context c;
  sptr_ctx* lane = nullptr;
  bool is_lane = false;
  uint32_t lanes_req = 0;
  bool lane_scene = false;
// ... 282 lines not shown
}

FrameView frame_view(const Context& c, const sptr_frame& f) {
  FrameView v;
  v.W = f.width;
  v.H = f.height;
  v.ntx = (f.width + kTile - 1) / kTile;
  v.G = c.G;
  v.R = c.R;
  v.P = c.P;
  v.k = 1;
  v.acc0 = f.frame_begin;
  v.max_depth = f.max_depth;
  v.div_P = make_fastdiv(c.P ? c.P : 1u);
  v.div_ntx = make_fastdiv((uint32_t)v.ntx);
  v.valid = 0;
  if (c.W > 0) {
    const int ntx = (c.W + kTile - 1) / kTile;
    for (uint32_t lt = 0; lt < c.local_tiles; ++lt) {
      const uint32_t t = lt * (uint32_t)c.G + (uint32_t)c.R;
      const int x0 = (int)(t % (uint32_t)ntx) * kTile, y0 = (int)(t / (uint32_t)ntx) * kTile;
      v.valid += (uint32_t)(std::min(kTile, c.W - x0) * std::min(kTile, c.H - y0));
    }
  }
  const sptr_camera& k = f.camera;
  v.cam_pos = v3(k.pos[0], k.pos[1], k.pos[2]);
  v.cam_f = v3(k.forward[0], k.forward[1], k.forward[2]);
  v.cam_r = v3(k.right[0], k.right[1], k.right[2]);
  v.cam_u = v3(k.up[0], k.up[1], k.up[2]);
  v.half_w = k.half_width;
  v.half_h = k.half_height;
#ifdef SPTR_EXPERIMENT_KNOBS
  static const uint32_t ablate = getenv("SPTR_ABLATE") ? (uint32_t)atoi(getenv("SPTR_ABLATE")) : 0u;
  v.ablate = ablate;
#else
  v.ablate = 0u;
#endif
  v.accum = static_cast<float4*>(c.accum.p);
  v.reset = 0;
  v.pixel_major = 0;
  v.dyn = nullptr;
  v.cull = nullptr;
  v.cull_depth = 4u;
  v.sky_fold = 0u;
  v.plist = nullptr;
  v.unculled = nullptr;
  v.entry = nullptr;
  v.split_threads = 0u;
  v.integrator = f.integrator;
  v.spf = f.samples_per_frame ? f.samples_per_frame : 4u;
  return v;
}

ShadeView shade_view(const Context& cc) {
  const Context& c = shading(cc);
  ShadeView s{};
  s.mats = static_cast<const DevMaterial*>(c.mats.p);
  s.num_mats = (uint32_t)c.mats_host.size();
  s.geom_mat = static_cast<const uint32_t*>(c.geom_mat.p);
  s.tri_mat = cc.parent ? nullptr : static_cast<const uint32_t*>(c.tri_mat.p);
  const bool pm = cc.prim_mat_n != 0u && cc.prim_mat_n == prim_mat_entries(cc.num_tri_refs, cc.num_sph);
  s.prim_mat = pm ? static_cast<const uint32_t*>(cc.prim_mat.p) : nullptr;
  s.pm_lds_bytes = pm ? prim_mat_lds_bytes(scene_view(cc).lds_bytes, cc.num_tri_refs, cc.num_sph, kLdsSceneBytes) : 0u;
  s.num_lights = (uint32_t)c.lights_host.size();
  for (uint32_t i = 0; i < s.num_lights; ++i) s.lights[i] = c.lights_host[i];
  s.env.env = static_cast<const float4*>(c.env.p);
  s.env.env_size = c.env_size;
  s.env.env_intensity = c.env_intensity;
  s.env.env_clamp = c.env_clamp;
  s.env.debug_mode = c.debug_mode;
  s.debug_mode = c.debug_mode;
  return s;
}

constexpr int kStages = 10;
#ifndef SPTR_CALL_SPAN
#define SPTR_CALL_SPAN 1
#endif
struct StageTimer {
  Context& c;
  bool on;
  bool trace_only;
  hipStream_t s;
  hipError_t err = hipSuccess;
  std::string what;
  size_t open = SIZE_MAX;
  size_t call = SIZE_MAX;
  size_t alloc() {
    if (c.events_used == c.events.size()) {
      DevEvent e;
      const hipError_t r = hipEventCreate(e.put());
      if (r != hipSuccess) {
        if (err == hipSuccess) {
          err = r;
          what = "stage event create";
        }
        return SIZE_MAX;
      }
      c.events.push_back(std::move(e));
    }
    return c.events_used++;
  }
  bool capturing = false;
  size_t next() {
    const size_t i = alloc();
    if (i != SIZE_MAX && err == hipSuccess) {
      err = hipEventRecord(c.events[i], s);
      if (err != hipSuccess) what = "stage event record";
    }
// ... 484 lines not shown
        d = Tc - 1;
        continue;
      }
      if (d == 0 && fuse && !no_bounce && T >= 2 && D >= 2) {
        tm.begin(9);
        g_shade = launch_bounce01(sv, sh, fv, w, g_trace, shade_first, std::min(T, D) <= 2, s);
        tm.end();
        rays_tab = w.segN;
        spare_tab = w.segH;
        d = 1;
        continue;
      }
      tm.begin(d == 0 ? 6 : 2);
      g_shade = launch_shade(sv, sh, fv, w, d, g_trace, fuse, s);
      tm.end();
      if (!fuse && shadow_side) {
        fork_to(ss);
        tside.begin(3);
        launch_shadow(sv, sh, w, d, count, g_shade, ss);
        tside.end();
        check(hipEventRecord(ev.join, ss), "shadow join record");
        join = true;
      } else if (!fuse) {
        tm.begin(3);
        launch_shadow(sv, sh, w, d, count, g_shade, s);
        tm.end();
      }
    }
    const bool resolve = done + kk >= f.spp && !(f.flags & SPTR_FRAME_NO_RESOLVE);
    join_shadow();
    if (join_sky) check(hipStreamWaitEvent(s, ev.sky, 0), "sky join wait");
    join_sky = false;
    if (fv.split_threads && sky_split_late()) {
      tm.begin(4);
      launch_sky_list(sh, fv, s);
      tm.end();
    }
    tm.begin(4);
    if (done + kk >= f.spp) tm.last_launch();
    launch_accumulate(fv, w, static_cast<float4*>(c.accum.p), static_cast<uint32_t*>(c.tiles.p),
                      c.image_out ? c.image_out : static_cast<uint8_t*>(c.image.p), resolve, s);
    tm.end();
    done += kk;
    ++waves;
  }
  if (tside.err != hipSuccess && tm.err == hipSuccess) {
    tm.err = tside.err;
    tm.what = tside.what;
  }
  tm.end_call();
  return waves;
}

int refresh_cull(Context& c, const sptr_frame& f, hipStream_t s, bool timing) {
  if (f.flags & SPTR_FRAME_NO_CULL) return SPTR_OK;
  const SceneView sv = scene_view(c);
  const bool exact = cull_exact_for(c, sv, f);
  const uint32_t depth = cull_depth_for(f.spp, exact);
  if (f.flags & SPTR_FRAME_RECULL) {
    c.cull_epoch = 0;
    return SPTR_OK;
  }
  const bool want_list = c.sky_split_last != 0u;
  if (!(f.flags & SPTR_FRAME_RECULL) && c.cull_epoch == c.epoch && c.cull_depth == depth && c.cull_exact == exact &&
      (c.cull_listed || !want_list) && std::memcmp(&c.cull_cam, &f.camera, sizeof(sptr_camera)) == 0)
    return SPTR_OK;
  FrameView fv = frame_view(c, f);
  fv.cull_depth = depth;
  StageTimer tm{c, timing, true, s};
  tm.begin(8);
  API_HIP(hipMemsetAsync(static_cast<uint32_t*>(c.plist.p) + c.P, 0, 8, s));
  launch_cull(sv, fv, static_cast<uint32_t*>(c.cull.p), static_cast<uint32_t*>(c.plist.p),
              exact ? static_cast<uint32_t*>(c.entry.p) : nullptr, want_list, s);
  tm.end();
  API_HIP(hipGetLastError());
  if (tm.err != hipSuccess) return fail(c, SPTR_ERR_HIP, std::string("render: cull events: ") + hipGetErrorString(tm.err));
  c.cull_epoch = c.epoch;
  c.cull_cam = f.camera;
  c.cull_depth = depth;
  c.cull_exact = exact;
  c.cull_listed = want_list;
  ++c.pending_culls;
  return SPTR_OK;
}

bool same_key(const GraphKey& a, const GraphKey& b) { return std::memcmp(&a, &b, sizeof(GraphKey)) == 0; }

struct GraphShape {
  uint32_t nodes = 0, edges = 0, depth = 0;
};
constexpr size_t kMaxGraphNodes = 4096;
bool check_graph(hipGraph_t g, GraphShape& out, std::string& why) {
  size_t n = 0, ne = 0;
  if (hipGraphGetNodes(g, nullptr, &n) != hipSuccess || hipGraphGetEdges(g, nullptr, nullptr, &ne) != hipSuccess) {
    why = "hipGraphGetNodes/Edges failed";
    return false;
  }
  if (n == 0 || n > kMaxGraphNodes) {
    why = std::to_string(n) + " nodes";
    return false;
  }
  std::vector<hipGraphNode_t> nodes(n), from(ne), to(ne);
  if (hipGraphGetNodes(g, nodes.data(), &n) != hipSuccess ||
      (ne && hipGraphGetEdges(g, from.data(), to.data(), &ne) != hipSuccess)) {
    why = "hipGraphGetNodes/Edges failed";
    return false;
// ... 320 lines not shown
  x->c.debug_mode = mode;
  ++x->c.epoch;
  return SPTR_OK;
}

static int set_leaf_size_one(sptr_ctx* x, uint32_t n) {
  if (!x) return SPTR_ERR_INVALID;
  if (n > kMaxLeafSize) return fail(x->c, SPTR_ERR_INVALID, "leaf size must be 0 (automatic) or 1..16");
  x->c.leaf_size = n;
  ++x->c.epoch;
  return SPTR_OK;
}

static int set_tree_order_one(sptr_ctx* x, uint32_t mode) {
  if (!x) return SPTR_ERR_INVALID;
  if (mode > 1u) return fail(x->c, SPTR_ERR_INVALID, "tree order must be 0 (automatic) or 1 (Morton)");
  x->c.tree_order = mode;
  ++x->c.epoch;
  return SPTR_OK;
}

static int set_bvh_width_one(sptr_ctx* x, uint32_t width) {
  if (!x) return SPTR_ERR_INVALID;
  if (width != 0 && width != 2 && width != (uint32_t)kWide)
    return fail(x->c, SPTR_ERR_INVALID, "bvh width must be 0 (auto), 2 or " + std::to_string(kWide));
  x->c.bvh_width = width;
  ++x->c.epoch;
  return build_prim_materials(x->c);
}

static int set_tail_depth_one(sptr_ctx* x, uint32_t depth) {
  if (!x) return SPTR_ERR_INVALID;
  if (depth > (uint32_t)kMaxDepth) return fail(x->c, SPTR_ERR_INVALID, "tail depth must be 0 (automatic) or 1..32");
  x->c.tail_depth = depth;
  ++x->c.epoch;
  return SPTR_OK;
}

static int set_bounce_chain_one(sptr_ctx* x, uint32_t mode) {
  if (!x) return SPTR_ERR_INVALID;
  if (mode > 2u) return fail(x->c, SPTR_ERR_INVALID, "bounce chain must be 0 (automatic), 1 (off) or 2 (on)");
  x->c.bounce_chain = mode;
  return SPTR_OK;
}

static int set_sky_split_one(sptr_ctx* x, uint32_t mode, uint32_t bulk_threads) {
  if (!x) return SPTR_ERR_INVALID;
  if (mode > 2u) return fail(x->c, SPTR_ERR_INVALID, "sky split must be 0 (automatic), 1 (off) or 2 (on)");
  x->c.sky_split = mode;
  x->c.sky_split_threads = bulk_threads;
  return SPTR_OK;
}

static int set_split_refs_one(sptr_ctx* x, uint32_t max_pieces) {
  if (!x) return SPTR_ERR_INVALID;
  if (max_pieces == 0u) max_pieces = 1u;
  if (max_pieces > 32u || (max_pieces & (max_pieces - 1u)))
    return fail(x->c, SPTR_ERR_INVALID, "split references: 0 (default: 1, none) or a power of two up to 32");
  x->c.split_pieces = max_pieces;
  ++x->c.epoch;
  return SPTR_OK;
}

static int set_stragglers_one(sptr_ctx* x, uint32_t lanes) {
  if (!x) return SPTR_ERR_INVALID;
  if (lanes > 64u) return fail(x->c, SPTR_ERR_INVALID, "straggler lanes: 0 (no hand-off) to 64");
  x->c.strag_lanes = lanes;
  ++x->c.epoch;
  return SPTR_OK;
}

static int set_wave_paths_one(sptr_ctx* x, uint64_t max_paths) {
  if (!x) return SPTR_ERR_INVALID;
  if (max_paths > (1ull << 30)) return fail(x->c, SPTR_ERR_INVALID, "wave paths above 2^30");
  x->c.wave_paths = max_paths;
  ++x->c.epoch;
  return SPTR_OK;
}

static int upload_scene_one(sptr_ctx* x, const sptr_scene* s) {
  if (!x || !s) return SPTR_ERR_INVALID;
  Context& c = x->c;
  if (sync_pending(c) != SPTR_OK) return SPTR_ERR_HIP;
  API_HIP(hipSetDevice(c.device));
  if ((s->num_tris && (!s->indices || !s->positions || !s->tri_geom_first)) || (s->num_spheres && !s->spheres) ||
      ((s->num_tri_geoms + s->num_spheres) && !s->geom_material))
    return fail(c, SPTR_ERR_INVALID, "scene: null array with nonzero count");
  if ((uint64_t)s->num_tris + s->num_spheres >= (1ull << (31 - kLeafCountBits)))
    return fail(c, SPTR_ERR_INVALID, "scene too large (at most 2^26 primitives)");
  if (s->num_tri_geoms && s->tri_geom_first[s->num_tri_geoms] != s->num_tris)
    return fail(c, SPTR_ERR_INVALID, "scene: tri_geom_first must end at num_tris");
  for (uint64_t i = 0; i < (uint64_t)s->num_tris * 3; ++i)
    if (s->indices[i] >= s->num_verts) return fail(c, SPTR_ERR_INVALID, "scene: vertex index out of range");
  std::vector<uint32_t> tg(s->num_tris);
  for (uint32_t g = 0; g < s->num_tri_geoms; ++g) {
    if (s->tri_geom_first[g] > s->tri_geom_first[g + 1]) return fail(c, SPTR_ERR_INVALID, "scene: geom offsets");
    for (uint32_t i = s->tri_geom_first[g]; i < s->tri_geom_first[g + 1]; ++i) tg[i] = g;
  }
  c.have_scene = false;
  c.prim_mat_n = 0u;
  c.num_tri_geoms = s->num_tri_geoms;
  c.geom_first.assign(s->tri_geom_first, s->tri_geom_first + (s->num_tri_geoms ? s->num_tri_geoms + 1 : 0));
  c.geom_material.assign(s->geom_material, s->geom_material + s->num_tri_geoms + s->num_spheres);
  const int rc = build_lbvh(c, s->positions, s->num_verts, s->indices, s->num_tris, s->spheres, s->num_spheres, tg.data(),
                            s->num_tri_geoms);
  if (rc != SPTR_OK) return rc;
  c.have_scene = true;
  ++c.epoch;
  return resolve_geom_materials(c);
}

int sptr_scene_info(const sptr_ctx* x, uint32_t* num_prims, uint32_t* num_nodes, uint32_t* depth, double* build_ms) {
  if (!x) return SPTR_ERR_INVALID;
  const Context& c = x->c;
  if (num_prims) *num_prims = c.num_tris + c.num_sph;
  if (num_nodes) *num_nodes = c.num_nodes;
  if (depth) *depth = c.bvh_depth;
  if (build_ms) *build_ms = c.build_ms;
  return SPTR_OK;
}

int sptr_scene_layout_info(const sptr_ctx* x, sptr_scene_layout* out) {
  if (!x || !out) return SPTR_ERR_INVALID;
  const Context& c = x->c;
  const SceneView sv = scene_view(c);
  out->num_tris = c.num_tris;
  out->num_spheres = c.num_sph;
  out->num_nodes = c.num_nodes;
  out->leaf_size = c.leaf_used;
  out->bvh_depth = c.bvh_depth;
  out->lds_bytes = sv.lds_bytes;
  out->bvh_width = sv.width;
  out->num_nodes = sv.width == (uint32_t)kWide ? c.num_nodes4 : c.num_nodes;
  out->node_bytes = sv.width == (uint32_t)kWide ? (uint64_t)c.num_nodes4 * sizeof(WideNode) : (uint64_t)c.num_nodes * sizeof(BvhNode);
  out->tri_bytes = (uint64_t)c.num_tri_refs * 48u;
  out->sphere_bytes = (uint64_t)c.num_sph * 16u;
  out->prim_ref_bytes = ((uint64_t)c.num_tri_refs + c.num_sph) * 4u;
  out->num_prim_refs = c.num_tri_refs + c.num_sph;
  return SPTR_OK;
}

static int set_materials_one(sptr_ctx* x, const sptr_material* m, uint32_t n) {
  if (!x || (n && !m)) return SPTR_ERR_INVALID;
  Context& c = x->c;
  if (sync_pending(c) != SPTR_OK) return SPTR_ERR_HIP;
  if (n == 0) return fail(c, SPTR_ERR_INVALID, "at least one material is required");
  API_HIP(hipSetDevice(c.device));
  c.mats_host.resize(n);
  std::memcpy(c.mats_host.data(), m, sizeof(DevMaterial) * n);
  API_HIP(c.mats.ensure(sizeof(DevMaterial) * n));
  API_HIP(hipMemcpy(c.mats.p, c.mats_host.data(), sizeof(DevMaterial) * n, hipMemcpyHostToDevice));
  ++c.epoch;
  return resolve_geom_materials(c);
}

static int set_lights_one(sptr_ctx* x, const sptr_light* l, uint32_t n) {
  if (!x || (n && !l)) return SPTR_ERR_INVALID;
  Context& c = x->c;
  if (n > (uint32_t)kMaxLights) return fail(c, SPTR_ERR_INVALID, "too many lights");
  c.lights_host.resize(n);
  ++c.epoch;
// ... 81 lines not shown
    if (f->integrator != SPTR_INTEGRATOR_WAVEFRONT)
      return fail(c, SPTR_ERR_INVALID, "render: a seed offset applies to SPTR_INTEGRATOR_WAVEFRONT only (sptr_set_seed_offset)");
    if ((uint64_t)c.seed_offset + f->frame_begin + f->spp - 1 > 0xFFFFFFFFull)
      return fail(c, SPTR_ERR_INVALID, "render: seed offset + frame_begin + spp - 1 overflows 32 bits");
  }
  GraphKey key{};
  key.epoch = c.epoch;
  key.frame = *f;
  key.frame.frame_begin = 0;
  key.frame.flags &= (SPTR_FRAME_TIMING | SPTR_FRAME_TIMING_TRACE | SPTR_FRAME_COUNT_VISITS | SPTR_FRAME_NO_RESOLVE |
                      SPTR_FRAME_NO_CULL | SPTR_FRAME_RECULL);
  uint32_t waves = 0;
  uint64_t samples = 0;
  if (f->integrator != SPTR_INTEGRATOR_WAVEFRONT) {
    if (c.pending == 0) API_HIP(hipMemsetAsync(c.w_tot.p, 0, kTotWords * 8, s));
    const uint32_t spf = f->integrator == SPTR_INTEGRATOR_PATHTRACER ? (f->samples_per_frame ? f->samples_per_frame : 4u) : 1u;
    rc = run_call(c, key, f->frame_begin, reset ? 1u : 0u, total, (uint64_t)frame_view(c, *f).valid * f->spp, nullptr,
                  timing || trace_timing, false, s,
                  [&](hipStream_t cs, StageTimer& tm) { return enqueue_path_per_thread(c, *f, cs, tm); }, waves);
    if (rc != SPTR_OK) return rc;
    samples = (uint64_t)frame_view(c, *f).valid * f->spp * spf;
  } else {
    uint64_t wave_paths = c.wave_paths;
    if (!wave_paths) {
      wave_paths = kDefaultWavePaths;
      if (c.wb.cap < std::min<uint64_t>(wave_paths, (uint64_t)f->spp * c.P)) {
        size_t free_b = 0, total_b = 0;
        if (hipMemGetInfo(&free_b, &total_b) == hipSuccess && free_b) {
          const uint32_t hm = hrec_mult(scene_view(c));
          const uint64_t held = c.wb.cap ? c.wb.cap * wave_path_bytes(c.wb.L, c.wb.ts, hm) : 0ull;
          const uint32_t L = std::max<uint32_t>(1u, (uint32_t)shading(c).lights_host.size());
          const double budget = ((double)free_b + (double)held) * kWaveMemFraction -
                                (double)wave_slack_bytes(L, task_stride(c), std::min<uint32_t>(f->spp, 1024u), hm);
          const uint64_t fit = budget > 0.0 ? (uint64_t)budget / wave_path_bytes(L, task_stride(c), hm) : 0ull;
          wave_paths = std::max<uint64_t>(1ull << 24, std::min<uint64_t>(wave_paths, fit));
        }
      }
    }
    uint32_t k = (uint32_t)std::max<uint64_t>(1, wave_paths / c.P);
    k = std::min<uint32_t>(k, f->spp);
    {
      FrameView probe = frame_view(c, *f);
      probe.k = k;
      bool pm = bounce0_pixel_major(scene_view(c), probe) != 0u;
      if (f->spp % k) {
        probe.k = f->spp % k;
        pm = pm || bounce0_pixel_major(scene_view(c), probe) != 0u;
      }
      rc = ensure_wave(c, (uint64_t)k * c.P, (uint32_t)shading(c).lights_host.size(), task_stride(c), pm ? k : 1u,
                       hrec_mult(scene_view(c)));
      if (rc != SPTR_OK) return rc;
    }
    const int T = std::max(1, (int)(c.tail_depth ? c.tail_depth : auto_tail_depth((uint64_t)k * c.P, scene_view(c))));
    key.epoch = c.epoch;
    key.k = k;
    key.tail = (uint32_t)T;
    key.chain = c.bounce_chain;
    key.sky_split = c.sky_split;
    key.sky_split_threads = c.sky_split_threads;
    {
      FrameView probe = frame_view(c, *f);
      probe.k = k;
      probe.pixel_major = bounce0_pixel_major(scene_view(c), probe);
      if (!(f->flags & SPTR_FRAME_NO_CULL)) probe.cull = static_cast<const uint32_t*>(c.cull.p);
      c.sky_split_last = sky_split_threads(c, scene_view(c), shade_view(c), probe);
    }
    if (c.pending == 0) API_HIP(hipMemsetAsync(c.w_tot.p, 0, kTotWords * 8, s));
    rc = refresh_cull(c, *f, s, timing || trace_timing);
    if (rc != SPTR_OK) return rc;
    uint32_t* clear = ((f->flags & SPTR_FRAME_RECULL) && !(f->flags & SPTR_FRAME_NO_CULL))
                          ? static_cast<uint32_t*>(c.plist.p) + c.P : nullptr;
    rc = run_call(c, key, f->frame_begin + c.seed_offset, reset ? 1u : 0u, total, (uint64_t)frame_view(c, *f).valid * f->spp, clear,
                  timing || trace_timing, !timing, s,
                  [&](hipStream_t cs, StageTimer& tm) { return enqueue_wavefront(c, *f, k, T, cs, tm); }, waves);
    if (rc != SPTR_OK) return rc;
    if (clear) {
      c.cull_epoch = c.epoch;
      c.cull_cam = f->camera;
      c.cull_exact = cull_exact_for(c, scene_view(c), *f);
      c.cull_listed = c.sky_split_last != 0u;
      c.cull_depth = cull_depth_for(f->spp, c.cull_exact);
      ++c.pending_culls;
    }
    samples = (uint64_t)frame_view(c, *f).valid * f->spp;
  }
  c.last_samples = total;
  ++c.pending;
  c.pending_stream = s;
  c.pending_samples += samples;
  c.pending_waves += waves;
  if (f->flags & SPTR_FRAME_ASYNC) {
    if (stats) std::memset(stats, 0, sizeof(*stats));
    return SPTR_OK;
  }
  return collect_pending(c, stats);
}

const char* sptr_capture_error(const sptr_ctx* x) { return x ? x->c.capture_error.c_str() : "null context"; }

int sptr_graph_info(const sptr_ctx* x, uint32_t* valid, uint32_t* nodes, uint32_t* edges, uint32_t* depth,
                    uint32_t* captures, int32_t* capture_status) {
  if (!x) return SPTR_ERR_INVALID;
  const GraphCache& g = x->c.graph;
  if (captures) *captures = x->c.captures;
  if (capture_status) *capture_status = x->c.capture_status;
  if (valid) *valid = g.valid ? 1u : 0u;
// ... 1082 lines not shown
  uint32_t *di = nullptr, *dout = nullptr;
  char* tmp = nullptr;
  size_t tb = 0;
  API_HIP(scan_u32(nullptr, tb, nullptr, nullptr, n, c.stream));
  API_HIP(d.alloc(&di, n));
  API_HIP(d.alloc(&dout, n));
  API_HIP(d.alloc(&tmp, tb));
  if (n) API_HIP(hipMemcpy(di, in, (size_t)n * 4, hipMemcpyHostToDevice));
  API_HIP(scan_u32(tmp, tb, di, dout, n, c.stream));
  API_HIP(hipStreamSynchronize(c.stream));
  if (n) API_HIP(hipMemcpy(out, dout, (size_t)n * 4, hipMemcpyDeviceToHost));
  return SPTR_OK;
}


static int lane_forward(sptr_ctx* x, int rc_lane) {
  if (!x || !x->lane || rc_lane == SPTR_OK) return SPTR_OK;
  return fail(x->c, rc_lane, std::string("pixel lane: ") + x->lane->c.err);
}

int sptr_upload_scene(sptr_ctx* x, const sptr_scene* s) {
  const int rc = upload_scene_one(x, s);
  if (rc != SPTR_OK) return rc;
  x->geom_first_valid = false;
  x->dn.snap_valid = false;
  if (x->split) x->c.W = 0;
  x->split = false;
  x->lane_scene = false;
  if (x->lane && scene_view(x->c).lds_bytes != 0) {
    Context& cy = x->lane->c;
    if (!cy.stream && hipStreamCreateWithPriority(cy.stream.put(), hipStreamNonBlocking, x->c.prio_lo) != hipSuccess)
      return fail(x->c, SPTR_ERR_HIP, "pixel lane: stream creation failed");
    const int r1 = upload_scene_one(x->lane, s);
    if (r1 != SPTR_OK) return lane_forward(x, r1);
    x->lane_scene = true;
    const int r2 = build_prim_materials(cy);
    if (r2 != SPTR_OK) return lane_forward(x, r2);
  }
  return SPTR_OK;
}

int sptr_set_dynamic(sptr_ctx* x, uint32_t on) {
  if (!x) return SPTR_ERR_INVALID;
  x->c.dynamic = on != 0u;
  x->c.dynamic_xf = (on & SPTR_DYNAMIC_TRANSFORMS) != 0u;
  if (x->lane) x->lane->c.dynamic = x->c.dynamic;
  return SPTR_OK;
}

static int refit_one(Context& c, const float* d_pos, const float* d_sph, const float* d_xf) {
  if (sync_pending(c) != SPTR_OK) return SPTR_ERR_HIP;
  const int rc = refit_lbvh(c, d_pos, reinterpret_cast<const float4*>(d_sph), d_xf);
  ++c.epoch;
  return rc;
}

static int refit_scene(sptr_ctx* x, const char* who, const float* d_pos, const float* d_sph, const float* d_xf,
                       std::chrono::steady_clock::time_point t0) {
  Context& c = x->c;
  auto& d = x->dn;
  if (d.motion_on && d.last.valid && d.last.gen == d.geom_gen) {
    const int rs = refit_snapshot(c);
    if (rs != SPTR_OK) return rs;
    d.snap_gen = d.geom_gen;
    d.snap_valid = true;
  }
  const uint64_t epoch_before = c.epoch;
  const int rc = refit_one(c, d_pos, d_sph, d_xf);
  ++d.geom_gen;
  if (rc != SPTR_OK) return rc;
  if (d.motion_on)
    for (sptr_ctx::Denoise::Pass* p : {&d.last, &d.carry})
      if (p->valid && p->epoch == epoch_before) p->epoch = c.epoch;
  if (x->lane && x->lane_scene) {
    Context& cy = x->lane->c;
    if (!cy.rf.valid) return fail(c, SPTR_ERR_INVALID, std::string(who) + ": the pixel lane's scene is not dynamic");
    const int r1 = refit_one(cy, d_pos, d_sph, d_xf);
    if (r1 != SPTR_OK) return lane_forward(x, r1);
  }
  c.rf.ms_wall = std::chrono::duration<double, std::milli>(std::chrono::steady_clock::now() - t0).count();
  return SPTR_OK;
}

int sptr_update_geometry(sptr_ctx* x, const float* positions, uint32_t num_verts, const float* spheres,
                         uint32_t num_spheres, uint32_t flags) {
  if (!x) return SPTR_ERR_INVALID;
  Context& c = x->c;
  if (x->is_lane) return fail(c, SPTR_ERR_INVALID, "update_geometry: not on a lane context");
  if (!c.have_scene) return fail(c, SPTR_ERR_NO_SCENE, "update_geometry: no scene uploaded");
  if (c.rf.split)
    return fail(c, SPTR_ERR_INVALID, "update_geometry: the scene was built with split references (sptr_set_split_refs)");
  if (!c.rf.valid) return fail(c, SPTR_ERR_INVALID, "update_geometry: the scene was not uploaded with sptr_set_dynamic(1)");
  if (!positions && !spheres) return fail(c, SPTR_ERR_INVALID, "update_geometry: no coordinates given");
  if ((positions && num_verts != c.rf.num_verts) || (spheres && num_spheres != c.num_sph))
    return fail(c, SPTR_ERR_INVALID, "update_geometry: counts differ from the uploaded scene's");
  if (flags & ~(uint32_t)SPTR_UPDATE_DEVICE_PTRS) return fail(c, SPTR_ERR_INVALID, "update_geometry: unknown flags");
  const auto t0 = std::chrono::steady_clock::now();
  API_HIP(hipSetDevice(c.device));
  if (sync_pending(c) != SPTR_OK) return SPTR_ERR_HIP;
  const float *d_pos = positions, *d_sph = spheres;
  if (!(flags & SPTR_UPDATE_DEVICE_PTRS)) {
    if (positions) {
      API_HIP(c.rf.in_pos.ensure((size_t)num_verts * 12));
      API_HIP(hipMemcpyAsync(c.rf.in_pos.p, positions, (size_t)num_verts * 12, hipMemcpyHostToDevice, c.stream));
      d_pos = static_cast<const float*>(c.rf.in_pos.p);
    }
// ... 682 lines not shown
  return rc;
}

int sptr_set_debug_mode(sptr_ctx* x, int mode) { return lane_shading_changed(x, set_debug_mode_one(x, mode)); }

int sptr_set_leaf_size(sptr_ctx* x, uint32_t n) {
  const int rc = set_leaf_size_one(x, n);
  return rc == SPTR_OK ? lane_forward(x, set_leaf_size_one(x ? x->lane : nullptr, n)) : rc;
}

int sptr_set_tree_order(sptr_ctx* x, uint32_t mode) {
  const int rc = set_tree_order_one(x, mode);
  return rc == SPTR_OK ? lane_forward(x, set_tree_order_one(x ? x->lane : nullptr, mode)) : rc;
}

int sptr_tree_info(const sptr_ctx* x, sptr_tree_order_info* out) {
  if (!x || !out) return SPTR_ERR_INVALID;
  const Context::TreeInfo& t = x->c.tree_info;
  out->order = t.order;
  out->fallback = t.fallback;
  out->depth = t.depth;
  out->num_leaves = t.leaves;
  out->cost_sah = t.cost_sah;
  out->cost_morton = t.cost_morton;
  return SPTR_OK;
}

int sptr_set_bvh_width(sptr_ctx* x, uint32_t width) {
  const int rc = set_bvh_width_one(x, width);
  return rc == SPTR_OK ? lane_forward(x, set_bvh_width_one(x ? x->lane : nullptr, width)) : rc;
}

int sptr_set_tail_depth(sptr_ctx* x, uint32_t depth) {
  const int rc = set_tail_depth_one(x, depth);
  return rc == SPTR_OK ? lane_forward(x, set_tail_depth_one(x ? x->lane : nullptr, depth)) : rc;
}

int sptr_set_bounce_chain(sptr_ctx* x, uint32_t mode) {
  const int rc = set_bounce_chain_one(x, mode);
  return rc == SPTR_OK ? lane_forward(x, set_bounce_chain_one(x ? x->lane : nullptr, mode)) : rc;
}

int sptr_set_sky_split(sptr_ctx* x, uint32_t mode, uint32_t bulk_threads) {
  const int rc = set_sky_split_one(x, mode, bulk_threads);
  return rc == SPTR_OK ? lane_forward(x, set_sky_split_one(x ? x->lane : nullptr, mode, bulk_threads)) : rc;
}

int sptr_sky_split_info(sptr_ctx* x, uint32_t* bulk_threads) {
  if (!x || !bulk_threads) return SPTR_ERR_INVALID;
  *bulk_threads = x->c.sky_split_last;
  return SPTR_OK;
}

int sptr_set_split_refs(sptr_ctx* x, uint32_t max_pieces) {
  const int rc = set_split_refs_one(x, max_pieces);
  return rc == SPTR_OK ? lane_forward(x, set_split_refs_one(x ? x->lane : nullptr, max_pieces)) : rc;
}

int sptr_set_stragglers(sptr_ctx* x, uint32_t lanes) {
  const int rc = set_stragglers_one(x, lanes);
  return rc == SPTR_OK ? lane_forward(x, set_stragglers_one(x ? x->lane : nullptr, lanes)) : rc;
}

int sptr_set_wave_paths(sptr_ctx* x, uint64_t max_paths) {
  const int rc = set_wave_paths_one(x, max_paths);
  return rc == SPTR_OK ? lane_forward(x, set_wave_paths_one(x ? x->lane : nullptr, max_paths)) : rc;
}

int sptr_set_materials(sptr_ctx* x, const sptr_material* m, uint32_t n) {
  const int rs = lane_shading_sync(x);
  if (rs != SPTR_OK) return rs;
  const int rc = lane_shading_changed(x, set_materials_one(x, m, n));
  if (rc != SPTR_OK || !x->lane) return rc;
  if (!x->lane_scene) {
    x->lane->c.prim_mat_n = 0u;
    return rc;
  }
  return lane_forward(x, build_prim_materials(x->lane->c));
}

int sptr_set_lights(sptr_ctx* x, const sptr_light* l, uint32_t n) {
  return lane_shading_changed(x, set_lights_one(x, l, n));
}

int sptr_set_environment(sptr_ctx* x, const sptr_environment* e) {
  const int rs = lane_shading_sync(x);
  if (rs != SPTR_OK) return rs;
  return lane_shading_changed(x, set_environment_one(x, e));
}

int sptr_set_launch_mode(sptr_ctx* x, uint32_t mode) {
  const int rc = set_launch_mode_one(x, mode);
  return rc == SPTR_OK ? lane_forward(x, set_launch_mode_one(x->lane, mode)) : rc;
}

}
```

### simple-path-tracer_amd/csrc/sptr_internal.h

```cpp
#pragma once
#include <hip/hip_runtime.h>

#include <string>
#include <utility>
#include <vector>

#include "adaptive_rule.h"
#include "dev_owned.h"
#include "hit_list.h"
#include "prim_mat_table.h"
#include "ray_batch.h"
#include "sptr_hip.h"
#include "sptr_math.h"
#include "tile_map.h"

namespace sptr {

constexpr uint32_t kLeafBit = 0x80000000u;
constexpr uint32_t kSphereBit = 0x40000000u;
constexpr uint32_t kIndexMask = 0x3FFFFFFFu;
constexpr uint32_t kLeafCountBits = 5;
constexpr uint32_t kLeafRangeMask = 0xFu;
constexpr uint32_t kLeafDirect = 0x10u;
constexpr uint32_t kLeafDirectSphere = 0x08u;
constexpr uint32_t kLeafCountMask = (1u << kLeafCountBits) - 1u;
constexpr uint32_t kMaxLeafSize = kLeafRangeMask + 1u;
constexpr uint32_t kNoHit = 0xFFFFFFFFu;
constexpr int kTile = 32;
constexpr int kTilePixels = kTile * kTile;
constexpr int kMaxLights = 8;
constexpr int kWide = 4;
constexpr int kWideLevels = 2;
constexpr int kQWords = 1;
constexpr int kTopLevels = 3;
constexpr int kMaxDepth = 32;
constexpr int kStack = 96;
constexpr int kBlock = 256;
#ifndef SPTR_TREELET_PASSES
#define SPTR_TREELET_PASSES 3
#endif
constexpr uint32_t kLdsSceneBytes = 48 * 1024;

struct BvhNode {
  float4 lxy;
  float4 rxy;
  float4 z;
  uint4 link;
};
static_assert(sizeof(BvhNode) == 64, "node size");

struct alignas(16) WideNode {
  float ox, oy, oz;
  uint32_t ex;
  uint32_t link[kWide];
  uint32_t q[6][kQWords];
  uint32_t parent;
  uint32_t pad[1];
};
static_assert(sizeof(WideNode) == 64, "node size");

struct DevMaterial {
  float albedo[3];
  float metallic;
  float roughness;
  float emission[3];
  float ior;
  int32_t type;
  float pad[2];
};
static_assert(sizeof(DevMaterial) == 48, "material size");

struct DevLight {
  int32_t type;
  float v[3];
  float radiance[3];
  float pad;
};

struct SceneView {
  const BvhNode* nodes;
  const WideNode* nodes4;
  const uint32_t* prim_ref;
  const float4* tris;
  const float4* sph;
  const uint32_t* tri_geom;
  const uint32_t* sph_geom;
  uint32_t num_nodes, num_tris, num_sph, root;
  uint32_t num_nodes4, root4;
  uint32_t num_top4;
  uint32_t width;
  uint32_t lds_bytes;
  uint64_t scene_bytes;
};

struct EnvView {
  const float4* env;
  int32_t env_size;
  float env_intensity, env_clamp;
  int32_t debug_mode;
};

struct ShadeView {
  const DevMaterial* mats;
  uint32_t num_mats;
  const uint32_t* geom_mat;
  const uint32_t* tri_mat;
  uint32_t num_lights;
  DevLight lights[kMaxLights];
  EnvView env;
  int32_t debug_mode;
  const uint32_t* prim_mat;
  uint32_t pm_lds_bytes;
};

struct FrameView {
  int32_t W, H, ntx, G, R;
  FastDiv div_P, div_ntx;
  uint32_t P;
  uint32_t k;
  uint32_t acc0;
  uint32_t max_depth;
  uint32_t valid;
  vec3 cam_pos, cam_f, cam_r, cam_u;
  float half_w, half_h;
  uint32_t ablate;
  float4* accum;
  uint32_t reset;
  uint32_t split_threads;
  const uint32_t* dyn;
  uint32_t pixel_major;
  uint32_t integrator;
  uint32_t spf;
  vec3 ox_u, ox_v, ox_w;
  vec3 ox_light_dir, ox_light_rad;
  uint32_t ox_has_light;
  const uint32_t* cull;
  uint32_t sky_fold;
  uint32_t cull_depth;
  const uint32_t* plist;
  const uint32_t* unculled;
  const uint32_t* entry;
};
static_assert(sizeof(FrameView) == 272, "FrameView: split_threads sits in padding, the kernels' arguments keep their layout");
constexpr size_t kDynBytes = 2048;

enum : uint32_t { kFoldNone = 0, kFoldThread = 1, kFoldWave = 2 };

constexpr uint32_t kWorkTraceQueue = 512;
constexpr uint32_t kWorkStrag = 768;
constexpr uint32_t kStragBounces = 4;
constexpr uint32_t kWorkWords = kWorkStrag + 32u * kStragBounces;
constexpr uint32_t kStragCap = 1u << 17;
constexpr uint32_t kStragRec = 4u + (uint32_t)kStack / 4u;
static_assert(kStragRec * 4u - 16u >= (uint32_t)kStack, "a straggler record holds the whole traversal stack");
constexpr uint32_t kStragLanesDefault = 12;
#ifndef SPTR_STRAG_MAXD
#define SPTR_STRAG_MAXD 1
#endif
constexpr uint32_t kStragHandoffBounces = SPTR_STRAG_MAXD;
constexpr uint32_t kMaxSegs = 2048;

enum : int {
  kTotClosest = 0,
  kTotShadow,
  kTotNodes, kTotTris, kTotSph,
// ... 241 lines not shown
  bool have_bad_key = false;
  std::string err;
  int debug_mode = 0;
  uint64_t wave_paths = 0;
  uint32_t tail_depth = 0;
  uint32_t bounce_chain = 0;
  uint32_t sky_split = 0;
  uint32_t sky_split_threads = 0;
  bool cull_listed = false;
  uint32_t sky_split_last = 0;
  DevBuf nodes, prim_ref, tris, sph, tri_geom, sph_geom, tri_orig, sph_orig, geom_mat;
  DevBuf tri_mat;
  DevBuf prim_mat;
  uint32_t prim_mat_n = 0;
  uint32_t leaf_size = 0;
  uint32_t bvh_width = 0;
  uint32_t leaf_used = 0;
  uint32_t treelet_passes = SPTR_TREELET_PASSES;
  uint32_t tree_order = 0;
  struct TreeInfo {
    uint32_t order = 1, fallback = 2, depth = 0, leaves = 0;
    double cost_sah = 0.0, cost_morton = 0.0;
  } tree_info;
  uint32_t num_nodes = 0, num_tris = 0, num_sph = 0, root = 0, bvh_depth = 0;
  uint32_t num_tri_refs = 0;
  uint32_t split_pieces = 1;
  uint32_t num_nodes4 = 0, root4 = 0;
  uint32_t excluded_prims = 0;
  uint32_t num_top4 = 0;
  uint32_t stack_need2 = 0, stack_need4 = 0;
  DevBuf nodes4;
  uint32_t num_tri_geoms = 0;
  std::vector<uint32_t> geom_first;
  std::vector<uint32_t> geom_material;
  bool have_scene = false;
  double build_ms = 0.0;
  bool dynamic = false;
  bool dynamic_xf = false;
  RefitState rf;
  std::vector<DevMaterial> mats_host;
  DevBuf mats;
  std::vector<DevLight> lights_host;
  DevBuf env;
  int32_t env_size = 0;
  float env_intensity = 0.8f, env_clamp = 5.0f;
  WaveBufs wb;
  DevBuf w_tot;
  int32_t W = 0, H = 0, G = 1, R = 0;
  uint32_t P = 0, local_tiles = 0;
  DevBuf accum, tiles, image;
  DevBuf cull;
  DevBuf plist;
  DevBuf entry;
  uint64_t cull_epoch = 0;
  sptr_camera cull_cam{};
  uint32_t cull_depth = 0;
  bool cull_exact = false;
  uint32_t last_samples = 0;
  uint32_t seed_offset = 0;
  DevBuf qbuf;
  std::vector<DevEvent> events;
  std::vector<StageMark> marks;
  size_t events_used = 0;
  uint32_t pending = 0;
  hipStream_t pending_stream = nullptr;
  uint64_t pending_samples = 0, pending_waves = 0, pending_culls = 0;
};

int build_lbvh(Context& c, const float* h_pos, uint32_t nverts, const uint32_t* h_idx, uint32_t ntris,
               const float* h_sph, uint32_t nsph, const uint32_t* h_tri_geom, uint32_t sph_geom_base);

int refit_retain_slots(Context& c, const float* d_pos, const uint32_t* d_idx, const float4* d_sph);
void launch_wide_sources(uint32_t ncur, const uint2* cur, uint32_t base, const BvhNode* nodes, uint32_t* wsrc, hipStream_t s);
int refit_lbvh(Context& c, const float* d_pos, const float4* d_sph, const float* d_xf = nullptr);
int refit_tree_cost(Context& c, double* cost, double* root_area);
int refit_snapshot(Context& c);
void refit_release(Context& c);

hipError_t scan_u32(void* temp, size_t& temp_bytes, const uint32_t* in, uint32_t* out, uint32_t n, hipStream_t s);
hipError_t radix_sort_pairs_u64(void* temp, size_t& temp_bytes, const uint64_t* keys_in, uint64_t* keys_out,
                                const uint32_t* vals_in, uint32_t* vals_out, uint32_t n, hipStream_t s);

SceneView scene_view(const Context& c);
unsigned launch_trace(const SceneView& sv, const ShadeView& sh, const FrameView& f, const WaveView& w, int depth, bool count,
                  uint32_t nseg_in, hipStream_t s, bool stream_rays = false);
bool shade_fuses_shadows(const SceneView& sv, const ShadeView& sh, bool count);
bool shadow_overlaps(const SceneView& sv, const WaveView& w);
unsigned launch_shade(const SceneView& sv, const ShadeView& sh, const FrameView& f, const WaveView& w, int depth,
                      uint32_t nseg, bool fuse, hipStream_t s, bool stream_rays = false);
unsigned launch_bounce01(const SceneView& sv, const ShadeView& sh, const FrameView& f, const WaveView& w, uint32_t nseg,
                         bool shade_first, bool close, hipStream_t s);
unsigned launch_bounce(const SceneView& sv, const ShadeView& sh, const FrameView& f, const WaveView& w, int depth,
                       uint32_t nseg, bool shade_first, bool close, hipStream_t s);
unsigned launch_bounce_chain(const SceneView& sv, const ShadeView& sh, const FrameView& f, const WaveView& w, int T,
                             uint32_t nseg, hipStream_t s);
unsigned launch_tail(const SceneView& sv, const ShadeView& sh, const FrameView& f, const WaveView& w, int depth0,
                     uint32_t nseg_in, hipStream_t s);
unsigned launch_shadow(const SceneView& sv, const ShadeView& sh, const WaveView& w, int depth, bool count, uint32_t nseg_in,
                   hipStream_t s);
void launch_strag(const SceneView& sv, const ShadeView& sh, const FrameView& f, const WaveView& w, int depth,
                  hipStream_t s);
bool trace_queue_applies(const SceneView& sv);
uint32_t hrec_mult(const SceneView& sv);
bool strag_applies(const SceneView& sv);
uint32_t bounce0_pixel_major(const SceneView& sv, const FrameView& f);
void launch_accumulate(const FrameView& f, const WaveView& w, float4* accum, uint32_t* tiles, uint8_t* image,
                       bool resolve, hipStream_t s);
uint32_t cull_depth_for(uint32_t spp, bool exact);
bool cull_entries_apply(const SceneView& sv);
void launch_cull(const SceneView& sv, const FrameView& f, uint32_t* mask, uint32_t* plist, uint32_t* entry, bool list_culled,
                 hipStream_t s);
void launch_sky(const ShadeView& sh, const FrameView& f, bool capped, hipStream_t s);
void launch_sky_list(const ShadeView& sh, const FrameView& f, hipStream_t s);
uint32_t sky_list_resident_threads(const ShadeView& sh);
void launch_interleave_tiles(const uint32_t* a, uint32_t na, const uint32_t* b, uint32_t nb, uint32_t* dst,
                             uint32_t n, hipStream_t s);
void launch_resolve(const FrameView& f, const float4* accum, uint32_t n, uint32_t* tiles, uint8_t* image,
                    hipStream_t s);
void launch_frame_dyn(uint32_t* dyn, uint32_t frame_begin, uint32_t reset, uint32_t total, uint32_t* clear,
                      unsigned long long* t0, hipStream_t s);
const void* frame_dyn_kernel();
void launch_pathtracer(const SceneView& sv, const ShadeView& sh, const FrameView& f, const WaveView& w, hipStream_t s);
void launch_optix(const SceneView& sv, const ShadeView& sh, const FrameView& f, const WaveView& w, hipStream_t s);
void launch_unpack(const uint32_t* gathered, int G, uint32_t tiles_per_rank, int W, int H, uint8_t* rgb,
                   hipStream_t s);
void launch_tri_materials(const uint32_t* tri_geom, const uint32_t* geom_mat, uint32_t n, uint32_t* tri_mat, hipStream_t s);
void launch_prim_materials(const uint32_t* tri_geom, const uint32_t* sph_geom, const uint32_t* geom_mat, uint32_t num_tris,
                           uint32_t num_sph, uint32_t* prim_mat, hipStream_t s);
void launch_query(const SceneView& sv, const uint32_t* tri_orig, const uint32_t* sph_orig, const float* rays, uint32_t n,
                  bool anyhit, uint32_t* ref, float* t, float* ng, uint8_t* occ, uint32_t* stack_overflow, hipStream_t s);
void launch_primary(const FrameView& f, float* dirs, uint32_t* rng, hipStream_t s);
void launch_eval_math(int fn, const float* x, uint32_t n, float* out, hipStream_t s);
void launch_aov(const SceneView& sv, const FrameView& f, const AovView& a, hipStream_t s);
void launch_dn_mean(const DenoiseView& v, const float4* accum0, const float4* accum1, int G, float4* out, hipStream_t s);
void launch_atrous(const DenoiseView& v, const float4* cin, float4* cout, int step, float S2, hipStream_t s);
void launch_dn_resolve(const DenoiseView& v, const float4* c, uint8_t* image, hipStream_t s);
void launch_dn_reproject(const DenoiseView& v, const FrameView& f, const ReprojView& r, hipStream_t s);
void launch_dn_reproject_motion(const DenoiseView& v, const FrameView& f, const ReprojView& r, hipStream_t s);
void launch_atrous_history(const DenoiseView& v, const float4* cin, float4* cout, int step, float Si, hipStream_t s);
void launch_rayquery(const SceneView& sv, const RayQueryView& q, bool anyhit, hipStream_t s);
void launch_rayquery_multi(const SceneView& sv, const RayMultiView& q, hipStream_t s, uint32_t* list_capacity, uint32_t* lds_bytes);
void launch_ray_keys(const SceneView& sv, const float4* rays, uint32_t n, uint64_t* keys, uint32_t* index, hipStream_t s);
unsigned launch_rays_inject(const RayBatchView& b, const RayChunk& ck, const WaveView& w, hipStream_t s);
void launch_rays_gather(const RayBatchView& b, const RayChunk& ck, const WaveView& w, hipStream_t s);
struct AdaptiveBufs {
  uint32_t* base;
  float4* E;
  uint32_t* n;
  uint32_t* list;
  uint32_t* bstat;
  uint32_t* result;
  uint32_t guard_off[4];
};
constexpr uint32_t kAdaptiveGuardWords = 16;
constexpr uint32_t kAdaptiveGuardValue = 0xA5C3F00Du;
constexpr uint32_t kAdaptiveStatWords = 8;
enum : uint32_t { kAdaptiveResGroup = 0, kAdaptiveResActive, kAdaptiveResKeyBelow, kAdaptiveResKeyAbove, kAdaptiveResMinN,
                  kAdaptiveResMaxN, kAdaptiveResGuardBad, kAdaptiveResWords = 8 };
void launch_adapt_select(const AdaptiveBufs& b, const AdaptiveRule& rule, uint32_t key, const FrameView& f, hipStream_t s);
unsigned launch_adapt_inject(const AdaptiveBufs& b, const RayChunk& ck, uint32_t seed_offset, const FrameView& f,
                             const WaveView& w, hipStream_t s);
void launch_adapt_gather(const AdaptiveBufs& b, const RayChunk& ck, const FrameView& f, const WaveView& w, hipStream_t s);
void launch_adapt_resolve(const AdaptiveBufs& b, const FrameView& f, uint32_t* tiles, uint8_t* image, hipStream_t s);
void launch_spin(uint64_t ticks, hipStream_t s);
// ... 3 lines not shown
```

### simple-path-tracer_amd/sptr.py

```python
from __future__ import annotations

import ctypes as C
import os
from dataclasses import dataclass

import numpy as np

HERE = os.path.dirname(os.path.abspath(__file__))
LIB_PATH = os.environ.get("SPTR_LIB") or os.path.join(HERE, "libsptr_hip.so")

SPTR_ABI_VERSION = 9
SPTR_FRAME_TIMING = 1
SPTR_FRAME_NO_RESOLVE = 2
SPTR_FRAME_COUNT_VISITS = 4
SPTR_FRAME_ASYNC = 8
SPTR_FRAME_TIMING_TRACE = 16
SPTR_FRAME_NO_CULL = 32
SPTR_FRAME_RECULL = 64
SPTR_UPDATE_DEVICE_PTRS = 1
SPTR_DYNAMIC_REFIT = 1
SPTR_DYNAMIC_TRANSFORMS = 2
SPTR_QUERY_ANY_HIT = 1
SPTR_QUERY_DEVICE_PTRS = 2
SPTR_QUERY_SORT = 4
# ... 33 lines not shown


class Camera(C.Structure):
    _fields_ = [("pos", C.c_float * 3), ("forward", C.c_float * 3), ("right", C.c_float * 3),
                ("up", C.c_float * 3), ("half_width", C.c_float), ("half_height", C.c_float)]

    def as_array(self) -> np.ndarray:
        return np.array(list(self.pos) + list(self.forward) + list(self.right) + list(self.up)
                        + [self.half_width, self.half_height], dtype=np.float32)


class Frame(C.Structure):
    _fields_ = [("width", C.c_int32), ("height", C.c_int32), ("camera", Camera), ("frame_begin", C.c_uint32),
                ("spp", C.c_uint32), ("max_depth", C.c_uint32), ("shard_rank", C.c_int32),
                ("shard_count", C.c_int32), ("flags", C.c_uint32), ("integrator", C.c_uint32),
                ("samples_per_frame", C.c_uint32)]


class Stats(C.Structure):
    _fields_ = [("rays_closest", C.c_uint64), ("rays_shadow", C.c_uint64), ("samples", C.c_uint64),
                ("waves", C.c_uint64), ("ms_total", C.c_double), ("ms_raygen", C.c_double),
                ("ms_trace", C.c_double), ("ms_shade", C.c_double), ("ms_shadow", C.c_double),
                ("ms_accum", C.c_double), ("trace_launches", C.c_uint64), ("node_visits", C.c_uint64),
                ("tri_tests", C.c_uint64), ("sphere_tests", C.c_uint64), ("shadow_node_visits", C.c_uint64),
                ("shadow_prim_tests", C.c_uint64), ("ms_trace0", C.c_double), ("ms_shade0", C.c_double),
                ("rays_tail", C.c_uint64), ("ms_tail", C.c_double), ("traced_primary", C.c_uint64),
                ("traced_bounce", C.c_uint64), ("node_visits_primary", C.c_uint64),
                ("tri_tests_primary", C.c_uint64), ("sphere_tests_primary", C.c_uint64), ("ms_cull", C.c_double),
                ("cull_launches", C.c_uint64), ("shadow_launches", C.c_uint64),
                ("traced_by_depth", C.c_uint64 * 8), ("nodes_by_depth", C.c_uint64 * 8),
                ("trace_visit_hist", C.c_uint64 * 16), ("shadow_visit_hist", C.c_uint64 * 16),
                ("hits_primary", C.c_uint64), ("hits_bounce", C.c_uint64), ("paths_handed_off", C.c_uint64), ("strag_visits", C.c_uint64 * 3),
                ("ms_trace_busy", C.c_double), ("traced_fused", C.c_uint64)]

    def as_dict(self) -> dict:
        return {k: (list(v) if isinstance(v, C.Array) else v) for k, v in ((k, getattr(self, k)) for k, _ in self._fields_)}


class SceneLayout(C.Structure):
    _fields_ = [("num_tris", C.c_uint32), ("num_spheres", C.c_uint32), ("num_nodes", C.c_uint32),
                ("leaf_size", C.c_uint32), ("bvh_depth", C.c_uint32), ("lds_bytes", C.c_uint32),
                ("node_bytes", C.c_uint64), ("tri_bytes", C.c_uint64), ("sphere_bytes", C.c_uint64),
                ("prim_ref_bytes", C.c_uint64), ("bvh_width", C.c_uint32), ("num_prim_refs", C.c_uint32)]

    def as_dict(self) -> dict:
        return {k: getattr(self, k) for k, _ in self._fields_}


class TreeOrderInfo(C.Structure):
    _fields_ = [("order", C.c_uint32), ("fallback", C.c_uint32), ("depth", C.c_uint32), ("num_leaves", C.c_uint32),
                ("cost_sah", C.c_double), ("cost_morton", C.c_double)]


class DenoiseParams(C.Structure):
    _fields_ = [("iterations", C.c_uint32), ("sigma_color", C.c_float), ("sigma_depth", C.c_float),
                ("sigma_albedo", C.c_float), ("normal_log2_power", C.c_uint32), ("reserved", C.c_uint32 * 3)]


class HistoryParams(C.Structure):
    _fields_ = [("max_history", C.c_uint32), ("reserved", C.c_uint32 * 3)]


class RayQuery(C.Structure):
    _fields_ = [("rays", C.c_void_p), ("n", C.c_uint32), ("flags", C.c_uint32), ("geom", C.c_void_p),
                ("prim", C.c_void_p), ("t", C.c_void_p), ("ng", C.c_void_p), ("uv", C.c_void_p),
                ("occluded", C.c_void_p), ("reserved", C.c_uint64 * 4)]


class MultiHitQuery(C.Structure):
    _fields_ = [("rays", C.c_void_p), ("n", C.c_uint32), ("flags", C.c_uint32), ("max_hits", C.c_uint32),
                ("pad", C.c_uint32), ("count", C.c_void_p), ("geom", C.c_void_p), ("prim", C.c_void_p),
                ("t", C.c_void_p), ("ng", C.c_void_p), ("uv", C.c_void_p), ("reserved", C.c_uint64 * 4)]


SPTR_MULTI_HIT_MAX = 16


class RayRender(C.Structure):
    _fields_ = [("rays", C.c_void_p), ("seeds", C.c_void_p), ("n", C.c_uint32), ("samples", C.c_uint32),
                ("frame_index", C.c_uint32), ("max_depth", C.c_uint32), ("flags", C.c_uint32),
                ("radiance", C.c_void_p), ("reserved", C.c_uint32 * 4)]


class AdaptiveParams(C.Structure):
    _fields_ = [("threshold", C.c_float), ("min_samples", C.c_uint32), ("max_samples", C.c_uint32),
                ("step", C.c_uint32), ("flags", C.c_uint32), ("reserved", C.c_uint32 * 3)]


class AdaptiveInfo(C.Structure):
    _fields_ = [("samples", C.c_uint64), ("rays_closest", C.c_uint64), ("rays_shadow", C.c_uint64),
                ("passes", C.c_uint32), ("chunks", C.c_uint32), ("active_first", C.c_uint32),
                ("active_last", C.c_uint32), ("min_count", C.c_uint32), ("max_count", C.c_uint32),
                ("ms", C.c_double), ("reserved", C.c_uint32 * 4)]


SPTR_RAYS_DEVICE_PTRS, SPTR_RAYS_ACCUMULATE, SPTR_RAYS_NORMALIZE = 1, 2, 4
SPTR_ADAPTIVE_CONTINUE = 1
SPTR_AOV_ALBEDO, SPTR_AOV_NORMAL, SPTR_AOV_DEPTH, SPTR_AOV_ID, SPTR_AOV_UV = 0, 1, 2, 3, 4
DEFAULT_MAX_HISTORY = 4

_lib = None

EXPORTS = [
    "sptr_abi_version", "sptr_create", "sptr_destroy", "sptr_last_error", "sptr_set_debug_mode",
    "sptr_set_wave_paths", "sptr_set_launch_mode", "sptr_set_pixel_lanes", "sptr_pixel_lanes_info", "sptr_graph_info", "sptr_capture_error", "sptr_overlap_probe", "sptr_set_tail_depth", "sptr_set_bounce_chain", "sptr_set_sky_split", "sptr_sky_split_info", "sptr_set_leaf_size", "sptr_set_tree_order", "sptr_tree_info", "sptr_set_split_refs", "sptr_set_stragglers", "sptr_set_bvh_width", "sptr_upload_scene", "sptr_set_materials", "sptr_set_lights",
    "sptr_set_environment", "sptr_scene_info", "sptr_scene_layout_info", "sptr_render", "sptr_collect_stats",
    "sptr_read_rgb8", "sptr_read_rgb8_lagged",
    "sptr_read_accum",
    "sptr_tiles_device", "sptr_unpack_tiles", "sptr_intersect", "sptr_occluded", "sptr_primary_rays",
    "sptr_sort_pairs_u64", "sptr_scan_u32", "sptr_eval_math",
    "sptr_set_denoise", "sptr_read_aov", "sptr_read_denoised", "sptr_denoise_info",
    "sptr_set_seed_offset", "sptr_set_denoise_history", "sptr_read_history", "sptr_history_info",
    "sptr_set_history_motion", "sptr_read_motion", "sptr_motion_info",
    "sptr_set_dynamic", "sptr_update_geometry", "sptr_refit_info",
    "sptr_set_rest_positions", "sptr_update_transforms", "sptr_tree_cost",
    "sptr_query_rays", "sptr_query_info", "sptr_query_multi_hit", "sptr_multi_hit_info", "sptr_render_rays", "sptr_ray_render_info",
    "sptr_render_adaptive", "sptr_read_sample_counts",
    "sptr_host_builtin_scene", "sptr_host_scene_view", "sptr_host_scene_free", "sptr_host_camera_lookat",
    "sptr_host_preset_materials", "sptr_host_default_lights", "sptr_host_equirect_to_faces",
    "sptr_host_pack_tiles", "sptr_host_unpack_tiles", "sptr_host_load_hdr", "sptr_host_free",
]


def lib() -> C.CDLL:
    global _lib
    if _lib is not None:
        return _lib
    if not os.path.exists(LIB_PATH):
        raise SptrError(f"{LIB_PATH} not built (run make in simple-path-tracer_amd/)")
    L = C.CDLL(LIB_PATH)
    vp, i32, u32, u64 = C.c_void_p, C.c_int32, C.c_uint32, C.c_uint64
    fp, up, bp = C.POINTER(C.c_float), C.POINTER(C.c_uint32), C.POINTER(C.c_uint8)
    sig = {
        "sptr_abi_version": (C.c_int, []),
        "sptr_create": (C.c_int, [C.c_int, C.POINTER(vp)]),
        "sptr_destroy": (C.c_int, [vp]),
        "sptr_last_error": (C.c_char_p, [vp]),
        "sptr_set_debug_mode": (C.c_int, [vp, C.c_int]),
        "sptr_set_wave_paths": (C.c_int, [vp, u64]),
        "sptr_set_launch_mode": (C.c_int, [vp, u32]),
        "sptr_set_pixel_lanes": (C.c_int, [vp, u32]),
        "sptr_pixel_lanes_info": (C.c_int, [vp, C.POINTER(u32), C.POINTER(u32)]),
        "sptr_graph_info": (C.c_int, [vp, up, up, up, up, up, C.POINTER(C.c_int32)]),
        "sptr_capture_error": (C.c_char_p, [vp]),
        "sptr_overlap_probe": (C.c_int, [vp, C.POINTER(C.c_double)]),
        "sptr_set_tail_depth": (C.c_int, [vp, u32]),
        "sptr_set_bounce_chain": (C.c_int, [vp, u32]),
        "sptr_set_sky_split": (C.c_int, [vp, u32, u32]),
        "sptr_sky_split_info": (C.c_int, [vp, C.POINTER(u32)]),
        "sptr_set_leaf_size": (C.c_int, [vp, u32]),
        "sptr_set_tree_order": (C.c_int, [vp, u32]),
        "sptr_tree_info": (C.c_int, [vp, C.POINTER(TreeOrderInfo)]),
        "sptr_set_split_refs": (C.c_int, [vp, u32]),
        "sptr_set_stragglers": (C.c_int, [vp, u32]),
        "sptr_set_bvh_width": (C.c_int, [vp, u32]),
        "sptr_upload_scene": (C.c_int, [vp, C.POINTER(Scene)]),
        "sptr_set_materials": (C.c_int, [vp, C.POINTER(Material), u32]),
        "sptr_set_lights": (C.c_int, [vp, C.POINTER(Light), u32]),
        "sptr_set_environment": (C.c_int, [vp, C.POINTER(Environment)]),
        "sptr_scene_info": (C.c_int, [vp, up, up, up, C.POINTER(C.c_double)]),
        "sptr_scene_layout_info": (C.c_int, [vp, C.POINTER(SceneLayout)]),
        "sptr_render": (C.c_int, [vp, C.POINTER(Frame), vp, C.POINTER(Stats)]),
        "sptr_collect_stats": (C.c_int, [vp, C.POINTER(Stats)]),
        "sptr_read_rgb8": (C.c_int, [vp, bp]),
        "sptr_read_rgb8_lagged": (C.c_int, [vp, bp, C.POINTER(u32)]),
        "sptr_read_accum": (C.c_int, [vp, fp]),
        "sptr_tiles_device": (C.c_int, [vp, C.POINTER(vp), C.POINTER(C.c_size_t)]),
        "sptr_unpack_tiles": (C.c_int, [vp, vp, i32, u32, i32, i32, vp, vp]),
        "sptr_intersect": (C.c_int, [vp, fp, u32, up, up, fp, fp]),
        "sptr_occluded": (C.c_int, [vp, fp, u32, bp]),
        "sptr_primary_rays": (C.c_int, [vp, C.POINTER(Camera), i32, i32, u32, fp, up]),
        "sptr_sort_pairs_u64": (C.c_int, [vp, C.POINTER(C.c_uint64), up, u32, C.POINTER(C.c_uint64), up]),
        "sptr_scan_u32": (C.c_int, [vp, up, u32, up]),
        "sptr_eval_math": (C.c_int, [vp, C.c_int, fp, u32, fp]),
        "sptr_set_denoise": (C.c_int, [vp, C.POINTER(DenoiseParams)]),
        "sptr_read_aov": (C.c_int, [vp, C.c_int, vp]),
        "sptr_read_denoised": (C.c_int, [vp, fp]),
        "sptr_denoise_info": (C.c_int, [vp, C.POINTER(C.c_double), C.POINTER(C.c_double), up]),
        "sptr_set_seed_offset": (C.c_int, [vp, u32]),
        "sptr_set_denoise_history": (C.c_int, [vp, C.POINTER(HistoryParams)]),
        "sptr_read_history": (C.c_int, [vp, fp]),
        "sptr_history_info": (C.c_int, [vp, up, C.POINTER(C.c_double), up]),
        "sptr_set_history_motion": (C.c_int, [vp, u32]),
        "sptr_read_motion": (C.c_int, [vp, fp]),
        "sptr_motion_info": (C.c_int, [vp, up, C.POINTER(C.c_double), up]),
        "sptr_set_dynamic": (C.c_int, [vp, u32]),
        "sptr_update_geometry": (C.c_int, [vp, vp, u32, vp, u32, u32]),
        "sptr_refit_info": (C.c_int, [vp, up, C.POINTER(C.c_double), C.POINTER(C.c_double), up]),
        "sptr_set_rest_positions": (C.c_int, [vp, vp, u32, u32]),
        "sptr_update_transforms": (C.c_int, [vp, vp, u32, vp, u32, u32]),
        "sptr_tree_cost": (C.c_int, [vp] + [C.POINTER(C.c_double)] * 4),
        "sptr_query_rays": (C.c_int, [vp, C.POINTER(RayQuery), vp]),
        "sptr_query_info": (C.c_int, [vp, C.POINTER(C.c_double), C.POINTER(C.c_double), up, up]),
        "sptr_query_multi_hit": (C.c_int, [vp, C.POINTER(MultiHitQuery), vp]),
        "sptr_multi_hit_info": (C.c_int, [vp, C.POINTER(C.c_double), C.POINTER(C.c_double), up, up, up, up]),
        "sptr_render_rays": (C.c_int, [vp, C.POINTER(RayRender), vp]),
        "sptr_ray_render_info": (C.c_int, [vp, C.POINTER(C.c_double), C.POINTER(u64), C.POINTER(u64), up]),
        "sptr_render_adaptive": (C.c_int, [vp, C.POINTER(Frame), C.POINTER(AdaptiveParams), C.POINTER(AdaptiveInfo)]),
        "sptr_read_sample_counts": (C.c_int, [vp, up]),
        "sptr_host_builtin_scene": (C.c_int, [C.c_char_p, u32, u32, C.POINTER(vp)]),
        "sptr_host_scene_view": (C.c_int, [vp, C.POINTER(Scene)]),
        "sptr_host_scene_free": (None, [vp]),
# ... 262 lines not shown
        self._check(self._L.sptr_set_lights(self._h, arr, len(lights)), "set_lights")

    def set_environment(self, faces: np.ndarray | None = None, intensity: float = 0.8, max_clamp: float = 5.0):
        e = Environment()
        if faces is not None:
            self._env_keep = np.ascontiguousarray(faces, np.float32)
            e.faces = _f(self._env_keep)
            e.size = self._env_keep.shape[1]
        e.intensity = intensity
        e.max_clamp = max_clamp
        self._check(self._L.sptr_set_environment(self._h, C.byref(e)), "set_environment")

    def set_wave_paths(self, n: int):
        self._check(self._L.sptr_set_wave_paths(self._h, n), "set_wave_paths")

    def graph_info(self) -> dict:
        v = [C.c_uint32() for _ in range(5)] + [C.c_int32()]
        self._check(self._L.sptr_graph_info(self._h, *[C.byref(x) for x in v]), "graph_info")
        d = dict(zip(("valid", "nodes", "edges", "depth", "captures", "capture_status"), (int(x.value) for x in v)))
        d["capture_error"] = self._L.sptr_capture_error(self._h).decode()
        return d

    def overlap_probe(self) -> dict:
        ms = (C.c_double * 3)()
        self._check(self._L.sptr_overlap_probe(self._h, ms), "overlap_probe")
        return {"serial_ms": round(ms[0], 4), "side_ms": round(ms[1], 4), "sky_side_ms": round(ms[2], 4),
                "side_has_own_queue": bool(ms[1] < 0.75 * ms[0]), "sky_side_has_own_queue": bool(ms[2] < 0.75 * ms[0])}

    def set_launch_mode(self, mode: int):
        self._check(self._L.sptr_set_launch_mode(self._h, mode), "set_launch_mode")

    def set_pixel_lanes(self, lanes: int):
        self._check(self._L.sptr_set_pixel_lanes(self._h, lanes), "set_pixel_lanes")

    def pixel_lanes_info(self) -> dict:
        r, a = C.c_uint32(), C.c_uint32()
        self._check(self._L.sptr_pixel_lanes_info(self._h, C.byref(r), C.byref(a)), "pixel_lanes_info")
        return {"requested": r.value, "active": bool(a.value)}

    def set_tail_depth(self, n: int):
        self._check(self._L.sptr_set_tail_depth(self._h, n), "set_tail_depth")

    def set_bounce_chain(self, mode: int):
        self._check(self._L.sptr_set_bounce_chain(self._h, mode), "set_bounce_chain")

    def set_sky_split(self, mode: int, bulk_threads: int = 0):
        self._check(self._L.sptr_set_sky_split(self._h, mode, bulk_threads), "set_sky_split")

    def sky_split_info(self) -> dict:
        t = C.c_uint32()
        self._check(self._L.sptr_sky_split_info(self._h, C.byref(t)), "sky_split_info")
        return {"bulk_threads": t.value}

    def set_leaf_size(self, n: int):
        self._check(self._L.sptr_set_leaf_size(self._h, n), "set_leaf_size")

    def set_tree_order(self, mode: int):
        self._check(self._L.sptr_set_tree_order(self._h, mode), "set_tree_order")

    def tree_info(self) -> dict:
        t = TreeOrderInfo()
        self._check(self._L.sptr_tree_info(self._h, C.byref(t)), "tree_info")
        return {k: getattr(t, k) for k, _ in TreeOrderInfo._fields_}

    def set_split_refs(self, max_pieces: int):
        self._check(self._L.sptr_set_split_refs(self._h, max_pieces), "set_split_refs")

    def set_stragglers(self, lanes: int):
        self._check(self._L.sptr_set_stragglers(self._h, lanes), "set_stragglers")

    def set_bvh_width(self, n: int):
        self._check(self._L.sptr_set_bvh_width(self._h, n), "set_bvh_width")

    def set_debug_mode(self, m: int):
        self._check(self._L.sptr_set_debug_mode(self._h, m), "set_debug_mode")

    def render(self, cam: Camera, width: int, height: int, spp: int = 1, frame_begin: int = 1,
               max_depth: int = 6, shard_rank: int = 0, shard_count: int = 1, flags: int = 0,
               stream: int | None = None, integrator: int = SPTR_INTEGRATOR_WAVEFRONT,
               samples_per_frame: int = 0) -> Stats:
        f = Frame(width, height, cam, frame_begin, spp, max_depth, shard_rank, shard_count, flags, integrator,
                  samples_per_frame)
        st = Stats()
        self._check(self._L.sptr_render(self._h, C.byref(f), C.c_void_p(stream) if stream else None, C.byref(st)),
                    "render")
        self.width, self.height = width, height
        return st

    def collect_stats(self) -> Stats:
        st = Stats()
        self._check(self._L.sptr_collect_stats(self._h, C.byref(st)), "collect_stats")
        return st

    def read_rgb8(self) -> np.ndarray:
        out = np.zeros((self.height, self.width, 3), np.uint8)
        self._check(self._L.sptr_read_rgb8(self._h, _b(out)), "read_rgb8")
        return out

    def read_rgb8_lagged(self, out: np.ndarray) -> bool:
        assert out.dtype == np.uint8 and out.flags.c_contiguous and out.size == self.width * self.height * 3
        got = C.c_uint32()
        self._check(self._L.sptr_read_rgb8_lagged(self._h, _b(out), C.byref(got)), "read_rgb8_lagged")
        return bool(got.value)

    def read_accum(self) -> np.ndarray:
        out = np.zeros((self.height, self.width, 3), np.float32)
# ... 343 lines not shown
```

Measured before the change: 96350 Mrays/s.

## Add light-space shadow entry table to start shadow rays below the BVH root

Builds a per-light grid (128x128 cells over the scene bounds projected along the light) in which each cell stores the deepest BVH node or leaf range that can occlude shadow rays from that cell, found with a prism-culling descent. It reuses the frustum-cull descent through a templated Region abstraction. Shadow rays then look up their cell and start any-hit traversal from that entry, or skip traversal entirely when no geometry can occlude. The aim is to cut BVH node visits for shadow rays. In exchange it adds a table build when geometry or the light changes, gated by a minimum sample count, plus a host sync to read the root node.

```diff
diff --git a/include/sptr_hip.h b/include/sptr_hip.h
--- a/include/sptr_hip.h
+++ b/include/sptr_hip.h
@@ -129,6 +129,12 @@
 int sptr_set_bounce_chain(sptr_ctx* ctx, uint32_t mode);
 int sptr_set_sky_split(sptr_ctx* ctx, uint32_t mode, uint32_t bulk_threads);
 int sptr_sky_split_info(sptr_ctx* ctx, uint32_t* bulk_threads);
+typedef struct sptr_shadow_entries_info_t {
+  uint32_t mode, cells, bytes, builds;
+  float cells_below_root, cells_unoccluded;
+} sptr_shadow_entries_info_t;
+int sptr_set_shadow_entries(sptr_ctx* ctx, uint32_t mode);
+int sptr_shadow_entries_info(sptr_ctx* ctx, sptr_shadow_entries_info_t* out);
 int sptr_set_leaf_size(sptr_ctx* ctx, uint32_t max_prims);
 int sptr_set_tree_order(sptr_ctx* ctx, uint32_t mode);
 typedef struct sptr_tree_order_info {
diff --git a/simple-path-tracer_amd/csrc/kernels_wavefront.hip b/simple-path-tracer_amd/csrc/kernels_wavefront.hip
--- a/simple-path-tracer_amd/csrc/kernels_wavefront.hip
+++ b/simple-path-tracer_amd/csrc/kernels_wavefront.hip
@@ -858,14 +858,14 @@
 }
 
 constexpr uint32_t kEntryFieldBits = 13, kEntryFieldMask = (1u << kEntryFieldBits) - 1u;
-template <bool kW4, bool kCount, int N>
-__device__ __forceinline__ bool traverse_w_from(const Staged& sc, const SceneView& sv, uint32_t root, const Ray& r,
+template <bool kW4, bool kAny, bool kCount, int N>
+__device__ __forceinline__ bool traverse_w_from(const Staged& sc, const SceneView& sv, uint32_t root, const Ray& r, float tnear,
                                                 float& tfar, uint32_t& ref, Visits& vc, LdsStackN<N>& ls) {
   if constexpr (kW4) {
-    return traverse_wide<false, kCount>(sc.nodes4, sc.prim_ref, sc.tris, sc.sph, sv.root4, r, 0.0f, tfar, ref, vc, ls);
+    return traverse_wide<kAny, kCount>(sc.nodes4, sc.prim_ref, sc.tris, sc.sph, sv.root4, r, tnear, tfar, ref, vc, ls);
   } else {
     if (root & kLeafBit) {
-      if (root == sv.root) return leaf_test<false, kCount>(root, sc.prim_ref, sc.tris, sc.sph, r, 0.0f, tfar, ref, vc);
+      if (root == sv.root) return leaf_test<kAny, kCount>(root, sc.prim_ref, sc.tris, sc.sph, r, tnear, tfar, ref, vc);
       asm volatile("" : "+v"(root));
       const float4* nd = reinterpret_cast<const float4*>(sc.nodes + ((root >> 18) & kEntryFieldMask));
       const uint32_t right = (root >> 17) & 1u;
@@ -873,12 +873,33 @@
       const float2 z = reinterpret_cast<const float2*>(nd + 2)[right];
       if (kCount) ++vc.nodes;
       float tent;
-      if (!slab(xy.x, xy.y, xy.z, xy.w, z.x, z.y, r, 0.0f, tfar, tent)) return false;
+      if (!slab(xy.x, xy.y, xy.z, xy.w, z.x, z.y, r, tnear, tfar, tent)) return false;
       const uint32_t range = kLeafBit | (((root >> 4) & kEntryFieldMask) << kLeafCountBits) | (root & kLeafRangeMask);
-      return leaf_test<false, kCount>(range, sc.prim_ref, sc.tris, sc.sph, r, 0.0f, tfar, ref, vc);
-    }
-    return traverse<false, kCount>(sc.nodes, sc.prim_ref, sc.tris, sc.sph, root, r, 0.0f, tfar, ref, vc, ls);
-  }
+      return leaf_test<kAny, kCount>(range, sc.prim_ref, sc.tris, sc.sph, r, tnear, tfar, ref, vc);
+    }
+    return traverse<kAny, kCount>(sc.nodes, sc.prim_ref, sc.tris, sc.sph, root, r, tnear, tfar, ref, vc, ls);
+  }
+}
+
+__device__ __forceinline__ uint32_t shadow_root(const SceneView& sv, const ShadeView& sh, vec3 so) {
+  uint32_t root = sv.root;
+  if (sh.shadow_entry) {
+    uint32_t i, j;
+    if (shadow_cell(sh.shadow_frame, so, i, j)) root = sh.shadow_entry[j * sh.shadow_frame.R + i];
+  }
+  return root;
+}
+template <bool kCount, int N>
+__device__ __forceinline__ bool shadow_occluded_from(const Staged& sc, const SceneView& sv, uint32_t root, vec3 so, vec3 ldir,
+                                                     float stfar, Visits& vc, LdsStackN<N>& ls) {
+  if (root == kNoHit) return false;
+  uint32_t ref = kNoHit;
+  return traverse_w_from<false, true, kCount>(sc, sv, root, make_ray(so, ldir), 1e-4f, stfar, ref, vc, ls);
+}
+template <bool kCount, int N>
+__device__ __forceinline__ bool shadow_occluded(const Staged& sc, const SceneView& sv, const ShadeView& sh, vec3 so, vec3 ldir,
+                                                float stfar, Visits& vc, LdsStackN<N>& ls) {
+  return shadow_occluded_from<kCount>(sc, sv, shadow_root(sv, sh, so), so, ldir, stfar, vc, ls);
 }
 
 template <bool kW4, bool kAny, bool kCount, int N>
@@ -1031,7 +1052,30 @@
   return right ? Box{v3(g.rxy.x, g.rxy.z, g.z.z), v3(g.rxy.y, g.rxy.w, g.z.w)}
                : Box{v3(g.lxy.x, g.lxy.z, g.z.x), v3(g.lxy.y, g.lxy.w, g.z.y)};
 }
-__device__ __forceinline__ void cull_leaf(const Staged& sc, const CullPyramid& py, uint32_t link, uint32_t& lo, uint32_t& hi) {
+struct PyramidRegion {
+  CullPyramid py;
+  __device__ __forceinline__ bool box_out(const Box& b) const { return box_outside(b, py.n, py.o); }
+  __device__ __forceinline__ bool sphere_out(float4 s) const {
+    const vec3 c = v3(s.x, s.y, s.z), v = c - py.o;
+    const float rb = fabsf(s.w) + 1.1e-3f * (fabsf(v.x) + fabsf(v.y) + fabsf(v.z)) +
+                     1e-5f * (py.ol + fabsf(c.x) + fabsf(c.y) + fabsf(c.z));
+    return box_outside(Box{c - v3(rb, rb, rb), c + v3(rb, rb, rb)}, py.n, py.o) || cull_sphere_outside(py, c, s.w);
+  }
+  __device__ __forceinline__ bool tri_out(vec3 v0, vec3 v1, vec3 v2) const {
+    const vec3 lo3 = v3(fminf(v0.x, fminf(v1.x, v2.x)), fminf(v0.y, fminf(v1.y, v2.y)), fminf(v0.z, fminf(v1.z, v2.z)));
+    const vec3 hi3 = v3(fmaxf(v0.x, fmaxf(v1.x, v2.x)), fmaxf(v0.y, fmaxf(v1.y, v2.y)), fmaxf(v0.z, fmaxf(v1.z, v2.z)));
+    const float pad = 1e-5f * (fabsf(lo3.x) + fabsf(lo3.y) + fabsf(lo3.z) + fabsf(hi3.x) + fabsf(hi3.y) + fabsf(hi3.z) + py.ol);
+    return box_outside(Box{lo3 - v3(pad, pad, pad), hi3 + v3(pad, pad, pad)}, py.n, py.o) || cull_triangle_outside(py, v0, v1, v2);
+  }
+};
+struct PrismRegion {
+  ShadowPrism p;
+  __device__ __forceinline__ bool box_out(const Box& b) const { return shadow_box_outside(p, b.lo, b.hi); }
+  __device__ __forceinline__ bool sphere_out(float4 s) const { return shadow_sphere_outside(p, v3(s.x, s.y, s.z), s.w); }
+  __device__ __forceinline__ bool tri_out(vec3 v0, vec3 v1, vec3 v2) const { return shadow_triangle_outside(p, v0, v1, v2); }
+};
+template <class Region>
+__device__ __forceinline__ void cull_leaf(const Staged& sc, const Region& rg, uint32_t link, uint32_t& lo, uint32_t& hi) {
   const uint32_t start = (link & ~kLeafBit) >> kLeafCountBits, cnt = (link & kLeafRangeMask) + 1u;
   lo = kNoHit;
   hi = 0u;
@@ -1040,18 +1084,11 @@
     const uint32_t idx = pr & kIndexMask;
     bool out;
     if (pr & kSphereBit) {
-      const float4 s = sc.sph[idx];
-      const vec3 c = v3(s.x, s.y, s.z), v = c - py.o;
-      const float rb = fabsf(s.w) + 1.1e-3f * (fabsf(v.x) + fabsf(v.y) + fabsf(v.z)) +
-                       1e-5f * (py.ol + fabsf(c.x) + fabsf(c.y) + fabsf(c.z));
-      out = box_outside(Box{c - v3(rb, rb, rb), c + v3(rb, rb, rb)}, py.n, py.o) || cull_sphere_outside(py, c, s.w);
+      out = rg.sphere_out(sc.sph[idx]);
     } else {
       const float4 a = sc.tris[3u * idx], b = sc.tris[3u * idx + 1u], c = sc.tris[3u * idx + 2u];
       const vec3 v0 = v3(a.x, a.y, a.z), v1 = v0 - v3(a.w, b.x, b.y), v2 = v0 + v3(b.z, b.w, c.x);
-      const vec3 lo3 = v3(fminf(v0.x, fminf(v1.x, v2.x)), fminf(v0.y, fminf(v1.y, v2.y)), fminf(v0.z, fminf(v1.z, v2.z)));
-      const vec3 hi3 = v3(fmaxf(v0.x, fmaxf(v1.x, v2.x)), fmaxf(v0.y, fmaxf(v1.y, v2.y)), fmaxf(v0.z, fmaxf(v1.z, v2.z)));
-      const float pad = 1e-5f * (fabsf(lo3.x) + fabsf(lo3.y) + fabsf(lo3.z) + fabsf(hi3.x) + fabsf(hi3.y) + fabsf(hi3.z) + py.ol);
-      out = box_outside(Box{lo3 - v3(pad, pad, pad), hi3 + v3(pad, pad, pad)}, py.n, py.o) || cull_triangle_outside(py, v0, v1, v2);
+      out = rg.tri_out(v0, v1, v2);
     }
     if (!out) {
       lo = min(lo, start + j);
@@ -1063,18 +1100,10 @@
   if (parent >= kEntryFieldMask || hi > kEntryFieldMask) return parent;
   return kLeafBit | (parent << 18) | (side << 17) | (lo << 4) | (hi - lo);
 }
-__device__ __forceinline__ uint32_t cull_entry(const Staged& sc, const SceneView& sv, const FrameView& f, int x, int y, int npx,
-                                               CullStack& cs) {
-  if (sv.root == kNoHit) return kNoHit;
-  const float u0 = (float(x) - kCullMarginPx) / float(f.W), u1 = (float(x + npx) + kCullMarginPx) / float(f.W);
-  const float v0 = (float(y) - kCullMarginPx) / float(f.H), v1 = (float(y + npx) + kCullMarginPx) / float(f.H);
-  auto dir = [&](float u, float v) {
-    return f.cam_f + ((u - 0.5f) * 2.0f * f.half_w) * f.cam_r + (-(v - 0.5f) * 2.0f * f.half_h) * f.cam_u;
-  };
-  const CullPyramid py = cull_pyramid(f.cam_pos, dir(u0, v0), dir(u1, v0), dir(u1, v1), dir(u0, v1));
+template <class Region>
+__device__ __forceinline__ uint32_t cull_descend(const Staged& sc, const SceneView& sv, const Region& rg, uint32_t limit,
+                                                 CullStack& cs) {
   uint32_t lo, hi;
-  if ((sv.root & kLeafBit) || sv.num_nodes == 0u) return sv.root;
-  const uint32_t limit = min(f.cull_depth, (uint32_t)kCullEntryDepth);
   uint32_t* st = &cs.st[0][threadIdx.x];
   uint16_t* path = &cs.path[0][threadIdx.x];
   int sp = 0;
@@ -1083,8 +1112,8 @@
   auto push_children = [&](uint32_t node, uint32_t depth) {
     const BvhNode g = sc.nodes[node];
     path[(depth - 1u) * kBlock] = (uint16_t)node;
-    if (!box_outside(child_box(g, true), py.n, f.cam_pos)) st[sp++ * kBlock] = cull_pack(g.link.y, depth, 1u);
-    if (!box_outside(child_box(g, false), py.n, f.cam_pos)) st[sp++ * kBlock] = cull_pack(g.link.x, depth, 0u);
+    if (!rg.box_out(child_box(g, true))) st[sp++ * kBlock] = cull_pack(g.link.y, depth, 1u);
+    if (!rg.box_out(child_box(g, false))) st[sp++ * kBlock] = cull_pack(g.link.x, depth, 0u);
   };
   push_children(sv.root, 1u);
   while (sp > 0) {
@@ -1092,7 +1121,7 @@
     const uint32_t link = e & (kCullLeaf - 1u), depth = (e >> 18) & 63u, side = (e >> 24) & 1u;
     mind = min(mind, depth);
     if (e & kCullLeaf) {
-      cull_leaf(sc, py, kLeafBit | ((link >> 4) << kLeafCountBits) | (link & kLeafRangeMask), lo, hi);
+      cull_leaf(sc, rg, kLeafBit | ((link >> 4) << kLeafCountBits) | (link & kLeafRangeMask), lo, hi);
       if (lo > hi) continue;
       one_leaf = ncand++ == 0u;
       common = one_leaf ? depth : min(common, mind);
@@ -1118,6 +1147,18 @@
   if (ncand == 0u) return kNoHit;
   if (one_leaf) return entry_leaf(anc, one_side, one_lo, one_hi);
   return anc;
+}
+__device__ __forceinline__ uint32_t cull_entry(const Staged& sc, const SceneView& sv, const FrameView& f, int x, int y, int npx,
+                                               CullStack& cs) {
+  if (sv.root == kNoHit) return kNoHit;
+  const float u0 = (float(x) - kCullMarginPx) / float(f.W), u1 = (float(x + npx) + kCullMarginPx) / float(f.W);
+  const float v0 = (float(y) - kCullMarginPx) / float(f.H), v1 = (float(y + npx) + kCullMarginPx) / float(f.H);
+  auto dir = [&](float u, float v) {
+    return f.cam_f + ((u - 0.5f) * 2.0f * f.half_w) * f.cam_r + (-(v - 0.5f) * 2.0f * f.half_h) * f.cam_u;
+  };
+  const PyramidRegion rg{cull_pyramid(f.cam_pos, dir(u0, v0), dir(u1, v0), dir(u1, v1), dir(u0, v1))};
+  if ((sv.root & kLeafBit) || sv.num_nodes == 0u) return sv.root;
+  return cull_descend(sc, sv, rg, min(f.cull_depth, (uint32_t)kCullEntryDepth), cs);
 }
 __device__ __forceinline__ uint32_t entry_index(uint32_t l) {
   const uint32_t w = l & 1023u;
@@ -1392,7 +1433,7 @@
         if (!(ablate(f) & 2u) && root != kNoHit) {
           const Ray r = make_ray(f.cam_pos, pr.d);
           const uint32_t v0 = vc.nodes;
-          hit = traverse_w_from<kW4, kCount>(sc, sv, root, r, tfar, ref, vc, s_stack);
+          hit = traverse_w_from<kW4, false, kCount>(sc, sv, root, r, 0.0f, tfar, ref, vc, s_stack);
           if (kCount) hist_ray(s_hist, vc.nodes - v0);
         }
         if (!hit) {
@@ -1496,7 +1537,7 @@
         if (root != kNoHit) {
           const Ray r = make_ray(f.cam_pos, pr.d);
           const uint32_t v0 = vc.nodes;
-          if constexpr (kEntries) hit = traverse_w_from<kW4, kCount>(sc, sv, root, r, tfar, ref, vc, s_stack);
+          if constexpr (kEntries) hit = traverse_w_from<kW4, false, kCount>(sc, sv, root, r, 0.0f, tfar, ref, vc, s_stack);
           else hit = traverse_w<kW4, false, kCount>(sc, sv, r, 0.0f, tfar, ref, vc, s_stack);
           if (kCount) hist_ray(s_hist, vc.nodes - v0);
         }
@@ -1606,7 +1647,7 @@
       const Ray r = make_ray(o, d);
       if (!(kPrimary && ((ablate(f) & 2u) || culled))) {
         const uint32_t v0 = vc.nodes;
-        if constexpr (kPrimary && kLds && !kW4) hit = traverse_w_from<kW4, kCount>(sc, sv, root, r, tfar, ref, vc, s_stack);
+        if constexpr (kPrimary && kLds && !kW4) hit = traverse_w_from<kW4, false, kCount>(sc, sv, root, r, 0.0f, tfar, ref, vc, s_stack);
         else hit = traverse_w<kW4, false, kCount>(sc, sv, r, 0.0f, tfar, ref, vc, s_stack);
         if (kCount) hist_ray(s_hist, vc.nodes - v0);
       }
@@ -2175,10 +2216,8 @@
     }
     if (kFuse) {
       if (lit) {
-        const Ray r = make_ray(so, ldir);
-        uint32_t ref = kNoHit;
         ++rays;
-        if (!traverse_w<false, true, false>(sc, sv, r, 1e-4f, stfar, ref, vc, s_stack)) {
+        if (!shadow_occluded<false>(sc, sv, sh, so, ldir, stfar, vc, s_stack)) {
           if (!dirty) radv = xyz(w.rad[p]);
           dirty = true;
           radv = radv + contrib;
@@ -2253,9 +2292,8 @@
     rout.thr[seg0 + jn] = f4(thr, 0.0f);
   }
   if (lit) {
-    uint32_t ref = kNoHit;
     ++rays;
-    if (!traverse_w<false, true, false>(sc, sv, make_ray(so, ldir), 1e-4f, stfar, ref, vc, s_stack)) {
+    if (!shadow_occluded<false>(sc, sv, sh, so, ldir, stfar, vc, s_stack)) {
       if (!dirty) radv = xyz(w.rad[p]);
       dirty = true;
       radv = radv + contrib;
@@ -2336,9 +2374,8 @@
       const bool lit = light_faces(sh.lights[0], sf) && light_term(sh.lights[0], sf, -pr.d, thr, so, ldir, stfar, contrib);
       active = continue_path(sf, pr.d, 0u, thr, rng, ro, rd) && !last1;
       if (lit) {
-        uint32_t sref = kNoHit;
         ++rays;
-        if (!traverse_w<false, true, false>(sc, sv, make_ray(so, ldir), 1e-4f, stfar, sref, vc, s_stack)) radv = radv + contrib;
+        if (!shadow_occluded<false>(sc, sv, sh, so, ldir, stfar, vc, s_stack)) radv = radv + contrib;
       }
     }
   }
@@ -2370,9 +2407,8 @@
     rout.thr[seg0 + jn] = f4(thr, 0.0f);
   }
   if (lit) {
-    uint32_t sref = kNoHit;
     ++rays;
-    if (!traverse_w<false, true, false>(sc, sv, make_ray(so, ldir), 1e-4f, stfar, sref, vc, s_stack)) radv = radv + contrib;
+    if (!shadow_occluded<false>(sc, sv, sh, so, ldir, stfar, vc, s_stack)) radv = radv + contrib;
   }
   if (valid) w.rad[p] = f4(radv, 0.0f);
 }
@@ -2517,12 +2553,11 @@
   dirty = true;
   radv = radv + c;
 }
-__device__ __forceinline__ void shadow_add(const Staged& sc, const SceneView& sv, const WaveView& w, uint32_t p, vec3 so,
-                                           vec3 ldir, float stfar, vec3 contrib, bool& dirty, vec3& radv, Visits& vc,
-                                           LdsStack& s_stack, uint32_t& rays) {
-  uint32_t sref = kNoHit;
+__device__ __forceinline__ void shadow_add(const Staged& sc, const SceneView& sv, const ShadeView& sh, const FrameView& f,
+                                           const WaveView& w, uint32_t p, uint32_t sroot, vec3 so, vec3 ldir, float stfar,
+                                           vec3 contrib, bool& dirty, vec3& radv, Visits& vc, LdsStack& s_stack, uint32_t& rays) {
   ++rays;
-  if (!traverse_w<false, true, false>(sc, sv, make_ray(so, ldir), 1e-4f, stfar, sref, vc, s_stack))
+  if ((ablate(f) & 8u) || !shadow_occluded_from<false>(sc, sv, sroot, so, ldir, stfar, vc, s_stack))
     rad_add(w, p, dirty, radv, contrib);
 }
 template <bool kCube, bool kFirst, bool kClose, int kFrom>
@@ -2532,7 +2567,7 @@
                                             uint32_t slot, uint32_t seg0, uint32_t* s_cnt, Visits& vc, LdsStack& s_stack,
                                             uint32_t& rays, uint32_t& traced) {
   bool active = false, dirty = kFirst && valid, lit = false;
-  uint32_t p = 0u, rng = 0u;
+  uint32_t p = 0u, rng = 0u, sroot = kNoHit;
   vec3 thr = v3(1.0f, 1.0f, 1.0f), radv = v3(0.0f, 0.0f, 0.0f), no, nd, so, ldir, contrib;
   float stfar = 0.0f;
   if (valid) {
@@ -2566,10 +2601,11 @@
       const vec3 emission = v3(sf.m.emission[0], sf.m.emission[1], sf.m.emission[2]);
       if (dot(emission, emission) > 0.0f) rad_add(w, p, dirty, radv, thr * emission);
       if (light_faces(sh.lights[0], sf)) lit = light_term(sh.lights[0], sf, -rd, thr, so, ldir, stfar, contrib);
+      if (lit) sroot = shadow_root(sv, sh, so);
       active = continue_path(sf, rd, (uint32_t)(depth - 1), thr, rng, no, nd);
     }
   }
-  if (lit) shadow_add(sc, sv, w, p, so, ldir, stfar, contrib, dirty, radv, vc, s_stack, rays);
+  if (lit) shadow_add(sc, sv, sh, f, w, p, sroot, so, ldir, stfar, contrib, dirty, radv, vc, s_stack, rays);
   bool hit = false;
   float tfar = __builtin_huge_valf();
   uint32_t href = kNoHit;
@@ -2599,6 +2635,7 @@
       const vec3 emission = v3(sf.m.emission[0], sf.m.emission[1], sf.m.emission[2]);
       if (dot(emission, emission) > 0.0f) rad_add(w, p, dirty, radv, thr * emission);
       if (light_faces(sh.lights[0], sf)) lit = light_term(sh.lights[0], sf, -nd, thr, so, ldir, stfar, contrib);
+      if (lit) sroot = shadow_root(sv, sh, so);
       if (!last) cont = continue_path(sf, nd, (uint32_t)depth, thr, rng, no2, nd2);
     }
     const uint32_t jn = block_append(s_cnt, cont);
@@ -2611,7 +2648,7 @@
       rout.d[seg0 + jn] = f4(nd2, __uint_as_float(p));
       rout.thr[seg0 + jn] = f4(thr, 0.0f);
     }
-    if (lit) shadow_add(sc, sv, w, p, so, ldir, stfar, contrib, dirty, radv, vc, s_stack, rays);
+    if (lit) shadow_add(sc, sv, sh, f, w, p, sroot, so, ldir, stfar, contrib, dirty, radv, vc, s_stack, rays);
   }
   if (dirty) w.rad[p] = f4(radv, 0.0f);
 }
@@ -2700,12 +2737,16 @@
       const vec3 dir = (ts > 2u && sh.lights[li].type != 0)
                            ? xyz(task[2])
                            : v3(sh.lights[li].v[0], sh.lights[li].v[1], sh.lights[li].v[2]);
-      const Ray r = make_ray(xyz(a), dir);
       float tfar = a.w;
-      uint32_t ref = kNoHit;
       ++rays;
       const uint32_t v0 = vc.nodes;
-      const bool occ = traverse_w<kW4, true, kCount>(sc, sv, r, 1e-4f, tfar, ref, vc, s_stack);
+      bool occ;
+      if (kLds && !kW4 && li == 0u) {
+        occ = shadow_occluded<kCount>(sc, sv, sh, xyz(a), dir, tfar, vc, s_stack);
+      } else {
+        uint32_t ref = kNoHit;
+        occ = traverse_w<kW4, true, kCount>(sc, sv, make_ray(xyz(a), dir), 1e-4f, tfar, ref, vc, s_stack);
+      }
       if (kCount) hist_ray(s_hist, vc.nodes - v0);
       if (!occ) {
         if (!any) rv = xyz(w.rad[p]);
@@ -2904,9 +2945,14 @@
         float st;
         if (!light_term(sh.lights[li], sf, view, thr, so, ldir, st, contrib)) continue;
         ++n_shadow;
-        uint32_t sref = kNoHit;
-        if (!traverse_w_top<kW4, true, false>(sc, sv, top, ntop, make_ray(so, ldir), 1e-4f, st, sref, vc, s_stack))
-          radv = radv + contrib;
+        bool occ;
+        if (kLds && !kW4 && li == 0u) {
+          occ = shadow_occluded<false>(sc, sv, sh, so, ldir, st, vc, s_stack);
+        } else {
+          uint32_t sref = kNoHit;
+          occ = traverse_w_top<kW4, true, false>(sc, sv, top, ntop, make_ray(so, ldir), 1e-4f, st, sref, vc, s_stack);
+        }
+        if (!occ) radv = radv + contrib;
       }
       vec3 no, nd;
       if (!continue_path(sf, rd, depth, thr, rng, no, nd)) break;
@@ -3936,6 +3982,22 @@
       Flags<>{}, depth == 0 && !stream_rays, fuse);
 }
 
+__global__ void __launch_bounds__(kBlock) k_shadow_entries(SceneView sv, ShadowFrame fr, uint32_t* table) {
+  extern __shared__ float4 lds[];
+  __shared__ CullStack s_cs;
+  const Staged sc = stage_scene<true>(sv, lds);
+  __syncthreads();
+  const uint32_t cell = blockIdx.x * kBlock + threadIdx.x;
+  if (cell >= fr.R * fr.R) return;
+  const uint32_t j = cell / fr.R, i = cell - j * fr.R;
+  const PrismRegion rg{shadow_prism(fr, i, j)};
+  table[cell] = cull_descend(sc, sv, rg, (uint32_t)kCullEntryDepth, s_cs);
+}
+void launch_shadow_entries(const SceneView& sv, const ShadowFrame& fr, uint32_t* table, hipStream_t s) {
+  const uint32_t cells = fr.R * fr.R;
+  hipLaunchKernelGGL(k_shadow_entries, dim3((cells + kBlock - 1u) / kBlock), dim3(kBlock), sv.lds_bytes, s, sv, fr, table);
+}
+
 bool cull_entries_apply(const SceneView& sv) { return sv.lds_bytes != 0u && sv.width == 2u; }
 uint32_t cull_depth_for(uint32_t spp, bool exact) {
   if (exact) return (uint32_t)kCullEntryDepth;
diff --git a/simple-path-tracer_amd/csrc/shadow_entry.h b/simple-path-tracer_amd/csrc/shadow_entry.h
--- /dev/null
+++ b/simple-path-tracer_amd/csrc/shadow_entry.h
@@ -0,0 +1,152 @@
+#pragma once
+#include "cull_prims.h"
+
+namespace sptr {
+
+struct ShadowFrame {
+  vec3 eu, ev;
+  float u0, v0;
+  float cell;
+  float inv_cell;
+  float mag;
+  float diag;
+  uint32_t R;
+};
+
+struct ShadowPrism {
+  float a0, a1, b0, b1;
+  float mag, diag;
+  vec3 eu, ev;
+};
+
+inline void shadow_frame_axes(vec3 w, vec3& eu, vec3& ev) {
+  const float ax = cull_abs(w.x), ay = cull_abs(w.y), az = cull_abs(w.z);
+  const vec3 a = (ax <= ay && ax <= az) ? v3(1.0f, 0.0f, 0.0f) : (ay <= az ? v3(0.0f, 1.0f, 0.0f) : v3(0.0f, 0.0f, 1.0f));
+  const vec3 c = cross(a, w);
+  eu = c * (1.0f / cull_len(c));
+  const vec3 d = cross(w, eu);
+  ev = d * (1.0f / cull_len(d));
+}
+
+inline bool shadow_frame(vec3 w, vec3 lo, vec3 hi, uint32_t R, ShadowFrame& f) {
+  const float wl = cull_len(w);
+  if (!(wl > 0.5f && wl < 2.0f) || R == 0u) return false;
+  if (!(lo.x <= hi.x && lo.y <= hi.y && lo.z <= hi.z)) return false;
+  shadow_frame_axes(w * (1.0f / wl), f.eu, f.ev);
+  float umin = 3.0e38f, umax = -3.0e38f, vmin = 3.0e38f, vmax = -3.0e38f;
+  for (int k = 0; k < 8; ++k) {
+    const vec3 p = v3((k & 1) ? hi.x : lo.x, (k & 2) ? hi.y : lo.y, (k & 4) ? hi.z : lo.z);
+    const float u = dot(p, f.eu), v = dot(p, f.ev);
+    umin = u < umin ? u : umin;
+    umax = u > umax ? u : umax;
+    vmin = v < vmin ? v : vmin;
+    vmax = v > vmax ? v : vmax;
+  }
+  auto amax = [](float a, float b) { return cull_abs(a) > cull_abs(b) ? cull_abs(a) : cull_abs(b); };
+  f.mag = amax(lo.x, hi.x) + amax(lo.y, hi.y) + amax(lo.z, hi.z);
+  f.diag = cull_len(hi - lo);
+  const float ext = (umax - umin) > (vmax - vmin) ? (umax - umin) : (vmax - vmin);
+  const float pad = 0.01f * ext + 1e-4f * f.mag + 1e-6f;
+  const float side = ext + 2.0f * pad;
+  f.R = R;
+  f.cell = side / float(R);
+  f.inv_cell = float(R) / side;
+  f.u0 = 0.5f * (umin + umax) - 0.5f * side;
+  f.v0 = 0.5f * (vmin + vmax) - 0.5f * side;
+  return f.mag < 1.0e30f && side > 0.0f && side < 1.0e30f;
+}
+
+SPTR_HD bool shadow_cell(const ShadowFrame& f, vec3 o, uint32_t& i, uint32_t& j) {
+  const float fi = (dot(o, f.eu) - f.u0) * f.inv_cell, fj = (dot(o, f.ev) - f.v0) * f.inv_cell;
+  const float r = float(f.R);
+  if (!(fi >= 0.0f && fi < r && fj >= 0.0f && fj < r)) return false;
+  i = (uint32_t)fi;
+  j = (uint32_t)fj;
+  return true;
+}
+
+SPTR_HD float shadow_cell_margin(const ShadowFrame& f) { return 1e-5f * f.mag + kCullPrimSlack * f.cell; }
+
+SPTR_HD ShadowPrism shadow_prism(const ShadowFrame& f, uint32_t i, uint32_t j) {
+  const float m = shadow_cell_margin(f);
+  ShadowPrism p;
+  p.a0 = f.u0 + float(i) * f.cell - m;
+  p.a1 = f.u0 + float(i + 1u) * f.cell + m;
+  p.b0 = f.v0 + float(j) * f.cell - m;
+  p.b1 = f.v0 + float(j + 1u) * f.cell + m;
+  p.mag = f.mag;
+  p.diag = f.diag;
+  p.eu = f.eu;
+  p.ev = f.ev;
+  return p;
+}
+
+SPTR_HD bool shadow_box_outside(const ShadowPrism& p, vec3 lo, vec3 hi) {
+  const vec3 e[2] = {p.eu, p.ev};
+  const float c0[2] = {p.a0, p.b0}, c1[2] = {p.a1, p.b1};
+  for (int k = 0; k < 2; ++k) {
+    const vec3 n = e[k];
+    const vec3 pmin = v3(n.x >= 0.0f ? lo.x : hi.x, n.y >= 0.0f ? lo.y : hi.y, n.z >= 0.0f ? lo.z : hi.z);
+    const vec3 pmax = v3(n.x >= 0.0f ? hi.x : lo.x, n.y >= 0.0f ? hi.y : lo.y, n.z >= 0.0f ? hi.z : lo.z);
+    const float bmin = dot(pmin, n), bmax = dot(pmax, n);
+    const float slack = kCullPrimSlack * (cull_mag(pmin, n) + cull_mag(pmax, n)) + kCullPrimRound * p.mag;
+    if (bmin > c1[k] + slack) return true;
+    if (bmax < c0[k] - slack) return true;
+  }
+  return false;
+}
+
+SPTR_HD bool shadow_sphere_outside(const ShadowPrism& p, vec3 C, float R) {
+  const float cu = dot(C, p.eu), cv = dot(C, p.ev);
+  const float round = kCullPrimRound * (p.mag + cull_mag(C, p.eu) + cull_mag(C, p.ev));
+  const float Re = sq_root(R * R + 1e-6f * p.diag * p.diag) + round;
+  float du = 0.0f, dv = 0.0f;
+  if (cu < p.a0) du = p.a0 - cu;
+  if (cu > p.a1) du = cu - p.a1;
+  if (cv < p.b0) dv = p.b0 - cv;
+  if (cv > p.b1) dv = cv - p.b1;
+  const float lim = Re + kCullPrimSlack * (Re + du + dv) + round;
+  return du * du + dv * dv > lim * lim;
+}
+
+SPTR_HD bool shadow_triangle_outside(const ShadowPrism& p, vec3 v0, vec3 v1, vec3 v2) {
+  const vec3 q[3] = {v0, v1, v2};
+  float u[3], v[3];
+  for (int k = 0; k < 3; ++k) {
+    u[k] = dot(q[k], p.eu);
+    v[k] = dot(q[k], p.ev);
+  }
+  const float round = kCullPrimRound * p.mag;
+  {
+    const float umin = fmin_g(u[0], fmin_g(u[1], u[2])), umax = fmax_g(u[0], fmax_g(u[1], u[2]));
+    const float vmin = fmin_g(v[0], fmin_g(v[1], v[2])), vmax = fmax_g(v[0], fmax_g(v[1], v[2]));
+    const float su = kCullPrimSlack * (cull_abs(umin) + cull_abs(umax)) + round;
+    const float sv = kCullPrimSlack * (cull_abs(vmin) + cull_abs(vmax)) + round;
+    if (umin > p.a1 + su || umax < p.a0 - su || vmin > p.b1 + sv || vmax < p.b0 - sv) return true;
+  }
+  const float cu[4] = {p.a0, p.a1, p.a1, p.a0}, cv[4] = {p.b0, p.b0, p.b1, p.b1};
+  for (int i = 0; i < 3; ++i) {
+    const int i1 = (i + 1) % 3, i2 = (i + 2) % 3;
+    const float nu = -(v[i1] - v[i]), nv = u[i1] - u[i];
+    const float nl = cull_abs(nu) + cull_abs(nv);
+    const float st = nu * (u[i2] - u[i]) + nv * (v[i2] - v[i]);
+    float mag = cull_abs(nu * (u[i2] - u[i])) + cull_abs(nv * (v[i2] - v[i]));
+    float cmin = 3.0e38f, cmax = -3.0e38f;
+    bool nan = false;
+    for (int k = 0; k < 4; ++k) {
+      const float a = nu * (cu[k] - u[i]), b = nv * (cv[k] - v[i]);
+      const float s = a + b;
+      nan = nan || !(s == s);
+      cmin = s < cmin ? s : cmin;
+      cmax = s > cmax ? s : cmax;
+      mag = fmax_g(mag, cull_abs(a) + cull_abs(b));
+    }
+    if (nan || !(st == st)) continue;
+    const float tmin = st < 0.0f ? st : 0.0f, tmax = st > 0.0f ? st : 0.0f;
+    const float slack = kCullPrimSlack * mag + 4.0f * round * nl;
+    if (cmin > tmax + slack || cmax < tmin - slack) return true;
+  }
+  return false;
+}
+
+}
diff --git a/simple-path-tracer_amd/csrc/sptr_api.cpp b/simple-path-tracer_amd/csrc/sptr_api.cpp
--- a/simple-path-tracer_amd/csrc/sptr_api.cpp
+++ b/simple-path-tracer_amd/csrc/sptr_api.cpp
@@ -358,9 +358,20 @@
   return v;
 }
 
+static bool shadow_entries_current(const Context& cc) {
+  const Context& c = shading(cc);
+  if (!cc.se.valid || cc.se.geom_rev != cc.geom_rev || c.lights_host.size() != 1u) return false;
+  const DevLight& l = c.lights_host[0];
+  return l.type == 0 && cc.se.light.type == 0 && std::memcmp(l.v, cc.se.light.v, sizeof(l.v)) == 0;
+}
+
 ShadeView shade_view(const Context& cc) {
   const Context& c = shading(cc);
   ShadeView s{};
+  if (cc.shadow_mode != 0u && shadow_entries_current(cc) && cull_entries_apply(scene_view(cc))) {
+    s.shadow_entry = static_cast<const uint32_t*>(cc.se.table.p);
+    s.shadow_frame = cc.se.frame;
+  }
   s.mats = static_cast<const DevMaterial*>(c.mats.p);
   s.num_mats = (uint32_t)c.mats_host.size();
   s.geom_mat = static_cast<const uint32_t*>(c.geom_mat.p);
@@ -951,6 +962,43 @@
   return waves;
 }
 
+constexpr uint64_t kShadowEntryMinSamples = 1ull << 23;
+constexpr uint64_t kShadowEntryRebuildMinSamples = 1ull << 27;
+int refresh_shadow_entries(Context& c, const sptr_frame& f, hipStream_t s) {
+  if (c.shadow_mode == 0u) return SPTR_OK;
+  const SceneView sv = scene_view(c);
+  const ShadeView sh = shade_view(c);
+  if (sh.shadow_entry) return SPTR_OK;
+  if (!cull_entries_apply(sv) || !shade_fuses_shadows(sv, sh, false) || sh.lights[0].type != 0) return SPTR_OK;
+  if (sv.root == kNoHit || (sv.root & kLeafBit) || sv.num_nodes == 0u) return SPTR_OK;
+  const DevLight& l = sh.lights[0];
+  if (c.se.no_frame && c.se.geom_rev == c.geom_rev && std::memcmp(l.v, c.se.light.v, sizeof(l.v)) == 0) return SPTR_OK;
+  if (c.shadow_mode == 1u) {
+    const bool first = c.se.upload_rev != c.upload_rev;
+    if ((uint64_t)c.P * f.spp < (first ? kShadowEntryMinSamples : kShadowEntryRebuildMinSamples)) return SPTR_OK;
+  }
+  BvhNode root;
+  API_HIP(hipMemcpyAsync(&root, sv.nodes + sv.root, sizeof(BvhNode), hipMemcpyDeviceToHost, s));
+  API_HIP(hipStreamSynchronize(s));
+  const vec3 lo = v3(std::min(root.lxy.x, root.rxy.x), std::min(root.lxy.z, root.rxy.z), std::min(root.z.x, root.z.z));
+  const vec3 hi = v3(std::max(root.lxy.y, root.rxy.y), std::max(root.lxy.w, root.rxy.w), std::max(root.z.y, root.z.w));
+  ShadowFrame fr;
+  c.se.valid = false;
+  c.se.geom_rev = c.geom_rev;
+  c.se.light = l;
+  c.se.upload_rev = c.upload_rev;
+  c.se.no_frame = !shadow_frame(v3(l.v[0], l.v[1], l.v[2]), lo, hi, kShadowEntryCells, fr);
+  if (c.se.no_frame) return SPTR_OK;
+  API_HIP(c.se.table.ensure((size_t)fr.R * fr.R * 4));
+  launch_shadow_entries(sv, fr, static_cast<uint32_t*>(c.se.table.p), s);
+  API_HIP(hipGetLastError());
+  c.se.valid = true;
+  c.se.frame = fr;
+  ++c.se.builds;
+  ++c.epoch;
+  return SPTR_OK;
+}
+
 int refresh_cull(Context& c, const sptr_frame& f, hipStream_t s, bool timing) {
   if (f.flags & SPTR_FRAME_NO_CULL) return SPTR_OK;
   const SceneView sv = scene_view(c);
@@ -1377,6 +1425,14 @@
   return SPTR_OK;
 }
 
+static int set_shadow_entries_one(sptr_ctx* x, uint32_t mode) {
+  if (!x) return SPTR_ERR_INVALID;
+  if (mode > 2u) return fail(x->c, SPTR_ERR_INVALID, "shadow entries must be 0 (off), 1 (automatic) or 2 (always)");
+  if (x->c.shadow_mode != mode) ++x->c.epoch;
+  x->c.shadow_mode = mode;
+  return SPTR_OK;
+}
+
 static int set_split_refs_one(sptr_ctx* x, uint32_t max_pieces) {
   if (!x) return SPTR_ERR_INVALID;
   if (max_pieces == 0u) max_pieces = 1u;
@@ -1432,6 +1488,8 @@
   if (rc != SPTR_OK) return rc;
   c.have_scene = true;
   ++c.epoch;
+  ++c.geom_rev;
+  ++c.upload_rev;
   return resolve_geom_materials(c);
 }
 
@@ -1619,6 +1677,8 @@
       if (rc != SPTR_OK) return rc;
     }
     const int T = std::max(1, (int)(c.tail_depth ? c.tail_depth : auto_tail_depth((uint64_t)k * c.P, scene_view(c))));
+    rc = refresh_shadow_entries(c, *f, s);
+    if (rc != SPTR_OK) return rc;
     key.epoch = c.epoch;
     key.k = k;
     key.tail = (uint32_t)T;
@@ -2807,6 +2867,7 @@
   if (sync_pending(c) != SPTR_OK) return SPTR_ERR_HIP;
   const int rc = refit_lbvh(c, d_pos, reinterpret_cast<const float4*>(d_sph), d_xf);
   ++c.epoch;
+  ++c.geom_rev;
   return rc;
 }
 
@@ -3595,6 +3656,35 @@
   return SPTR_OK;
 }
 
+int sptr_set_shadow_entries(sptr_ctx* x, uint32_t mode) {
+  const int rc = set_shadow_entries_one(x, mode);
+  return rc == SPTR_OK ? lane_forward(x, set_shadow_entries_one(x ? x->lane : nullptr, mode)) : rc;
+}
+
+int sptr_shadow_entries_info(sptr_ctx* x, sptr_shadow_entries_info_t* out) {
+  if (!x || !out) return SPTR_ERR_INVALID;
+  Context& c = x->c;
+  std::memset(out, 0, sizeof(*out));
+  out->mode = c.shadow_mode;
+  out->builds = c.se.builds;
+  if (!shade_view(c).shadow_entry) return SPTR_OK;
+  const uint32_t R = c.se.frame.R, n = R * R;
+  std::vector<uint32_t> words(n);
+  API_HIP(hipSetDevice(c.device));
+  API_HIP(hipDeviceSynchronize());
+  API_HIP(hipMemcpy(words.data(), c.se.table.p, (size_t)n * 4, hipMemcpyDeviceToHost));
+  uint32_t below = 0u, none = 0u;
+  for (uint32_t w : words) {
+    below += w != c.root ? 1u : 0u;
+    none += w == kNoHit ? 1u : 0u;
+  }
+  out->cells = R;
+  out->bytes = n * 4u;
+  out->cells_below_root = (float)below / (float)n;
+  out->cells_unoccluded = (float)none / (float)n;
+  return SPTR_OK;
+}
+
 int sptr_set_split_refs(sptr_ctx* x, uint32_t max_pieces) {
   const int rc = set_split_refs_one(x, max_pieces);
   return rc == SPTR_OK ? lane_forward(x, set_split_refs_one(x ? x->lane : nullptr, max_pieces)) : rc;
diff --git a/simple-path-tracer_amd/csrc/sptr_internal.h b/simple-path-tracer_amd/csrc/sptr_internal.h
--- a/simple-path-tracer_amd/csrc/sptr_internal.h
+++ b/simple-path-tracer_amd/csrc/sptr_internal.h
@@ -10,6 +10,7 @@
 #include "hit_list.h"
 #include "prim_mat_table.h"
 #include "ray_batch.h"
+#include "shadow_entry.h"
 #include "sptr_hip.h"
 #include "sptr_math.h"
 #include "tile_map.h"
@@ -111,6 +112,8 @@
   int32_t debug_mode;
   const uint32_t* prim_mat;
   uint32_t pm_lds_bytes;
+  const uint32_t* shadow_entry;
+  ShadowFrame shadow_frame;
 };
 
 struct FrameView {
@@ -458,6 +461,19 @@
   DevBuf cull;
   DevBuf plist;
   DevBuf entry;
+  uint64_t geom_rev = 1;
+  uint64_t upload_rev = 1;
+  uint32_t shadow_mode = 1;
+  struct ShadowEntries {
+    DevBuf table;
+    bool valid = false;
+    uint64_t geom_rev = 0;
+    DevLight light{};
+    uint64_t upload_rev = 0;
+    bool no_frame = false;
+    ShadowFrame frame{};
+    uint32_t builds = 0;
+  } se;
   uint64_t cull_epoch = 0;
   sptr_camera cull_cam{};
   uint32_t cull_depth = 0;
@@ -516,6 +532,8 @@
 bool cull_entries_apply(const SceneView& sv);
 void launch_cull(const SceneView& sv, const FrameView& f, uint32_t* mask, uint32_t* plist, uint32_t* entry, bool list_culled,
                  hipStream_t s);
+constexpr uint32_t kShadowEntryCells = 128;
+void launch_shadow_entries(const SceneView& sv, const ShadowFrame& fr, uint32_t* table, hipStream_t s);
 void launch_sky(const ShadeView& sh, const FrameView& f, bool capped, hipStream_t s);
 void launch_sky_list(const ShadeView& sh, const FrameView& f, hipStream_t s);
 uint32_t sky_list_resident_threads(const ShadeView& sh);
diff --git a/simple-path-tracer_amd/sptr.py b/simple-path-tracer_amd/sptr.py
--- a/simple-path-tracer_amd/sptr.py
+++ b/simple-path-tracer_amd/sptr.py
@@ -109,6 +109,11 @@
                 ("cost_sah", C.c_double), ("cost_morton", C.c_double)]
 
 
+class ShadowEntriesInfo(C.Structure):
+    _fields_ = [("mode", C.c_uint32), ("cells", C.c_uint32), ("bytes", C.c_uint32), ("builds", C.c_uint32),
+                ("cells_below_root", C.c_float), ("cells_unoccluded", C.c_float)]
+
+
 class DenoiseParams(C.Structure):
     _fields_ = [("iterations", C.c_uint32), ("sigma_color", C.c_float), ("sigma_depth", C.c_float),
                 ("sigma_albedo", C.c_float), ("normal_log2_power", C.c_uint32), ("reserved", C.c_uint32 * 3)]
@@ -160,7 +165,7 @@
 
 EXPORTS = [
     "sptr_abi_version", "sptr_create", "sptr_destroy", "sptr_last_error", "sptr_set_debug_mode",
-    "sptr_set_wave_paths", "sptr_set_launch_mode", "sptr_set_pixel_lanes", "sptr_pixel_lanes_info", "sptr_graph_info", "sptr_capture_error", "sptr_overlap_probe", "sptr_set_tail_depth", "sptr_set_bounce_chain", "sptr_set_sky_split", "sptr_sky_split_info", "sptr_set_leaf_size", "sptr_set_tree_order", "sptr_tree_info", "sptr_set_split_refs", "sptr_set_stragglers", "sptr_set_bvh_width", "sptr_upload_scene", "sptr_set_materials", "sptr_set_lights",
+    "sptr_set_wave_paths", "sptr_set_launch_mode", "sptr_set_pixel_lanes", "sptr_pixel_lanes_info", "sptr_graph_info", "sptr_capture_error", "sptr_overlap_probe", "sptr_set_tail_depth", "sptr_set_bounce_chain", "sptr_set_sky_split", "sptr_sky_split_info", "sptr_set_shadow_entries", "sptr_shadow_entries_info", "sptr_set_leaf_size", "sptr_set_tree_order", "sptr_tree_info", "sptr_set_split_refs", "sptr_set_stragglers", "sptr_set_bvh_width", "sptr_upload_scene", "sptr_set_materials", "sptr_set_lights",
     "sptr_set_environment", "sptr_scene_info", "sptr_scene_layout_info", "sptr_render", "sptr_collect_stats",
     "sptr_read_rgb8", "sptr_read_rgb8_lagged",
     "sptr_read_accum",
@@ -205,6 +210,8 @@
         "sptr_set_bounce_chain": (C.c_int, [vp, u32]),
         "sptr_set_sky_split": (C.c_int, [vp, u32, u32]),
         "sptr_sky_split_info": (C.c_int, [vp, C.POINTER(u32)]),
+        "sptr_set_shadow_entries": (C.c_int, [vp, u32]),
+        "sptr_shadow_entries_info": (C.c_int, [vp, C.POINTER(ShadowEntriesInfo)]),
         "sptr_set_leaf_size": (C.c_int, [vp, u32]),
         "sptr_set_tree_order": (C.c_int, [vp, u32]),
         "sptr_tree_info": (C.c_int, [vp, C.POINTER(TreeOrderInfo)]),
@@ -573,6 +580,14 @@
         self._check(self._L.sptr_sky_split_info(self._h, C.byref(t)), "sky_split_info")
         return {"bulk_threads": t.value}
 
+    def set_shadow_entries(self, mode: int):
+        self._check(self._L.sptr_set_shadow_entries(self._h, mode), "set_shadow_entries")
+
+    def shadow_entries_info(self) -> dict:
+        i = ShadowEntriesInfo()
+        self._check(self._L.sptr_shadow_entries_info(self._h, C.byref(i)), "shadow_entries_info")
+        return {k: getattr(i, k) for k, _ in ShadowEntriesInfo._fields_}
+
     def set_leaf_size(self, n: int):
         self._check(self._L.sptr_set_leaf_size(self._h, n), "set_leaf_size")
 
```

New measurement: 99190 Mrays/s (median of 6 runs). 2.9% higher.
